# mit-acl/clipper

Hardware: AMD Instinct MI355X
Metric: affinity+solve ms and GEMV HBM GB/s, n=10k assoc, 95% outliers, 1/8 GPU (lower is better)
Workload: dtype f64 (M stored f32)

## Files before the change

clipper_amd/_abi.py:

```python
from __future__ import annotations

import ctypes as C
import os
from dataclasses import dataclass, field

import numpy as np

_HERE = os.path.dirname(os.path.abspath(__file__))
LIB_PATH = os.environ.get("CLIPPER_HIP_LIB") or os.path.join(_HERE, "lib", "libclipper_hip.so")

STORE_F32, STORE_F64, STORE_F32_CSC, STORE_F64_CSC = 0, 1, 2, 3
ROUNDING_NONZERO, ROUNDING_DSD, ROUNDING_DSD_HEU = 0, 1, 2
MC_EXACT, MC_HEU, MC_KCORE = 0, 1, 2
MC_SEED_ONLY = 3
SDP_MAX_N = 128
SDP_WIDE_MAX_N = 1024
SDP_ROUTE_WORKGROUP, SDP_ROUTE_AUTO, SDP_ROUTE_WIDE = 0, 1, 2
INVARIANT_MAX_D, INVARIANT_MAX_PARAMS = 32, 16

EXPORTED_SYMBOLS = [
    "clipper_hip_device_count", "clipper_hip_create", "clipper_hip_create_group",
    "clipper_hip_create_rank", "clipper_hip_comm_unique_id", "clipper_hip_comm_init",
    "clipper_hip_destroy", "clipper_hip_last_error", "clipper_hip_affinity_euclidean",
    "clipper_hip_affinity_pointnormal", "clipper_hip_num_associations",
    "clipper_hip_get_associations", "clipper_hip_set_matrix", "clipper_hip_set_sparse",
    "clipper_hip_get_matrix", "clipper_hip_solve", "clipper_hip_get_nodes",
    "clipper_hip_get_selected_associations", "clipper_hip_matvec", "clipper_hip_set_profiling",
    "clipper_hip_set_window", "clipper_hip_window", "clipper_hip_densest_subgraph",
    "clipper_hip_set_resident", "clipper_hip_last_solver",
    "clipper_hip_set_row_view", "clipper_hip_get_view_stats", "clipper_hip_view_matvec", "clipper_hip_set_subproblem",
    "clipper_hip_storage_in_use", "clipper_hip_knn", "clipper_hip_distance_based_correspondences",
    "clipper_hip_get_timings", "clipper_hip_bench_matvec", "clipper_hip_device_info",
    "clipper_hip_stage_inputs", "clipper_hip_affinity_euclidean_staged",
    "clipper_hip_affinity_pointnormal_staged", "clipper_hip_stage_u0",
    "clipper_hip_solve_staged", "clipper_hip_debug_stamps", "clipper_hip_comm_init_callback",
    "clipper_hip_read_ply_xyz", "clipper_hip_generate_synthetic_correspondences",
    "clipper_hip_precision_recall", "clipper_hip_estimate_rigid_transform", "clipper_hip_debug_occupy",
    "clipper_hip_max_clique", "clipper_hip_core_numbers", "clipper_hip_sdp", "clipper_hip_sdp_solve",
    "clipper_hip_batch_create", "clipper_hip_batch_destroy", "clipper_hip_batch_solve_euclidean",
    "clipper_hip_batch_solve_pointnormal", "clipper_hip_batch_get_solution", "clipper_hip_batch_get_nodes",
    "clipper_hip_batch_get_selected_associations", "clipper_hip_batch_route", "clipper_hip_batch_get_stats",
    "clipper_hip_batch_get_split", "clipper_hip_invariant_create", "clipper_hip_invariant_destroy",
    "clipper_hip_affinity_custom_staged", "clipper_hip_affinity_custom", "clipper_hip_batch_solve_custom",
    "clipper_hip_sdp_solve_batch", "clipper_hip_batch_sdp", "clipper_hip_batch_get_sdp",
    "clipper_hip_batch_max_clique", "clipper_hip_batch_max_clique_stats",
    "clipper_hip_max_clique_seeded", "clipper_hip_batch_max_clique_seeded",
    "clipper_hip_sdp_set_route", "clipper_hip_sdp_route", "clipper_hip_match_descriptors",
]


ALLGATHER_FN = C.CFUNCTYPE(C.c_int, C.c_void_p, C.c_void_p, C.c_void_p, C.c_size_t)


class ClipperError(RuntimeError):
    """a C ABI entry point returned a negative status (CLIPPER_HIP_E_*)"""


class Params(C.Structure):

    _fields_ = [
        ("tol_u", C.c_double), ("tol_F", C.c_double), ("tol_Fop", C.c_double),
        ("maxiniters", C.c_int32), ("maxoliters", C.c_int32), ("beta", C.c_double),
        ("maxlsiters", C.c_int32), ("eps", C.c_double), ("affinityeps", C.c_double),
        ("rescale_u0", C.c_int32), ("rounding", C.c_int32),
    ]

    def __init__(self, **kw):
        super().__init__()
        self.tol_u, self.tol_F, self.tol_Fop = 1e-8, 1e-9, 1e-10
        self.maxiniters, self.maxoliters = 200, 1000
        self.beta, self.maxlsiters = 0.25, 99
        self.eps, self.affinityeps = 1e-9, 1e-4
        self.rescale_u0, self.rounding = 1, ROUNDING_DSD_HEU
        for k, v in kw.items():
            setattr(self, k, v)


class SolveInfo(C.Structure):
    _fields_ = [
        ("score", C.c_double), ("seconds", C.c_double), ("d", C.c_double),
        ("ifinal", C.c_int32), ("num_nodes", C.c_int32),
        ("n_passes", C.c_int64), ("n_trials", C.c_int64),
    ]


class Timings(C.Structure):
    _fields_ = [
        ("affinity_kernel_ms", C.c_double), ("affinity_total_ms", C.c_double),
        ("solve_total_ms", C.c_double), ("gemv_avg_us", C.c_double),
        ("gemv_min_us", C.c_double), ("gemv_launches", C.c_int64), ("gemv_bytes", C.c_double),
        ("gemv_useful_bytes", C.c_double), ("affinity_bytes", C.c_double),
        ("exchange_avg_us", C.c_double), ("exchange_samples", C.c_int64), ("exchange_bytes", C.c_double),
    ]


class ViewStats(C.Structure):

    _fields_ = [
        ("builds", C.c_int64), ("rows", C.c_int64), ("bytes", C.c_int64),
        ("view_passes", C.c_int64), ("passes", C.c_int64), ("build_ms", C.c_double),
        ("view_pass_avg_us", C.c_double), ("view_pass_samples", C.c_int64),
        ("resident_launches", C.c_int64), ("resident_giveups", C.c_int64),
        ("resident_iterations", C.c_int64), ("resident_us", C.c_double), ("resident_event_us", C.c_double),
        ("resident_entries", C.c_int64), ("resident_units", C.c_int64),
        ("sub_entries", C.c_int64), ("sub_leaves", C.c_int64), ("sub_passes", C.c_int64),
        ("sub_rows", C.c_int64), ("sub_bytes", C.c_int64), ("sub_build_ms", C.c_double),
        ("sub_pass_avg_us", C.c_double), ("sub_pass_samples", C.c_int64), ("sub_dense", C.c_int64),
    ]


class MaxCliqueInfo(C.Structure):

    _fields_ = [
        ("num_nodes", C.c_int32), ("max_core", C.c_int32), ("heuristic_size", C.c_int32), ("timed_out", C.c_int32),
        ("edges", C.c_int64), ("roots_searched", C.c_int64), ("roots_pruned", C.c_int64), ("bb_nodes", C.c_int64),
        ("seconds", C.c_double),
    ]


class MaxCliqueSeedInfo(C.Structure):

    _fields_ = [("seed_given", C.c_int32), ("seed_kept", C.c_int32), ("seed_size", C.c_int32), ("winner", C.c_int32)]


class SdpParams(C.Structure):

    _fields_ = [
        ("verbose", C.c_int32), ("max_iters", C.c_int32), ("acceleration_interval", C.c_int32),
        ("acceleration_lookback", C.c_int32), ("eps_abs", C.c_float), ("eps_rel", C.c_float),
        ("eps_infeas", C.c_float), ("time_limit_secs", C.c_float),
    ]

    def __init__(self, **kw):
        base = dict(verbose=0, max_iters=2000, acceleration_interval=10, acceleration_lookback=10, eps_abs=1e-3,
                    eps_rel=1e-3, eps_infeas=1e-7, time_limit_secs=0.0)
        base.update(kw)
        super().__init__(**base)


class SdpInfo(C.Structure):

    _fields_ = [
        ("iters", C.c_int32), ("converged", C.c_int32), ("timed_out", C.c_int32), ("num_nodes", C.c_int32),
        ("sweeps", C.c_int32), ("route", C.c_int32),
        ("pobj", C.c_double), ("dobj", C.c_double), ("r_prim", C.c_double), ("r_dual", C.c_double),
        ("rho", C.c_double), ("thr", C.c_double), ("t_total", C.c_double), ("t_setup", C.c_double),
        ("t_solve", C.c_double), ("t_extract", C.c_double),
    ]


class SdpProblem(C.Structure):

    _fields_ = [
        ("M", C.POINTER(C.c_double)), ("C", C.POINTER(C.c_double)), ("n", C.c_int64),
        ("X_out", C.POINTER(C.c_double)), ("Y_out", C.POINTER(C.c_double)), ("lambdas_out", C.POINTER(C.c_double)),
        ("evec1_out", C.POINTER(C.c_double)), ("nodes_out", C.POINTER(C.c_int32)),
    ]


@dataclass
class SdpResult:

    X: np.ndarray
    Y: np.ndarray
    lambdas: np.ndarray
    evec1: np.ndarray
    thr: float
    nodes: np.ndarray
    iters: int
    pobj: float
    dobj: float
    info: SdpInfo


def _sdp_result(n, X, Y, lam, ev, nodes, info) -> SdpResult:
    return SdpResult(X=X, Y=Y, lambdas=lam, evec1=ev, thr=info.thr, nodes=nodes, iters=info.iters, pobj=info.pobj,
                     dobj=info.dobj, info=info)


class MatchParams(C.Structure):
    _fields_ = [("knn", C.c_int32), ("mutual", C.c_int32), ("ratio", C.c_double), ("max_sqdist", C.c_double)]


class BatchProblem(C.Structure):

    _fields_ = [
        ("D1", C.POINTER(C.c_double)), ("n1", C.c_int64),
        ("D2", C.POINTER(C.c_double)), ("n2", C.c_int64),
        ("A", C.POINTER(C.c_int32)), ("m", C.c_int64),
        ("u0", C.POINTER(C.c_double)),
    ]


@dataclass
class Solution:

    t: float = 0.0
    ifinal: int = 0
    nodes: np.ndarray = field(default_factory=lambda: np.zeros(0, np.int32))
    u0: np.ndarray = field(default_factory=lambda: np.zeros(0))
    u: np.ndarray = field(default_factory=lambda: np.zeros(0))
    score: float = 0.0
    d: float = 0.0
    n_passes: int = 0
    n_trials: int = 0


_lib = None


def load_library(path: str = LIB_PATH):
    global _lib
    if _lib is not None:
        return _lib
    if not os.path.exists(path):
        raise RuntimeError(
            f"{path} not found: build it with `python -c 'import __graft_entry__ as g; g.build()'`"
            " (hipcc --offload-arch=gfx950). There is no CPU fallback.")
    L = C.CDLL(path)
    dp, ip, i64, vp = C.POINTER(C.c_double), C.POINTER(C.c_int32), C.c_int64, C.c_void_p
    L.clipper_hip_device_count.restype = C.c_int
    L.clipper_hip_create.argtypes = [C.c_int, C.c_int]
    L.clipper_hip_create.restype = vp
    L.clipper_hip_create_group.argtypes = [C.POINTER(C.c_int), C.c_int, C.c_int]
    L.clipper_hip_create_group.restype = vp
    L.clipper_hip_create_rank.argtypes = [C.c_int, C.c_int, C.c_int, C.c_int]
    L.clipper_hip_create_rank.restype = vp
    L.clipper_hip_comm_unique_id.argtypes = [vp]
    L.clipper_hip_comm_init.argtypes = [vp, vp]
    L.clipper_hip_destroy.argtypes = [vp]
    L.clipper_hip_destroy.restype = None
    L.clipper_hip_last_error.restype = C.c_char_p
    L.clipper_hip_affinity_euclidean.argtypes = [
        vp, dp, C.c_int, i64, dp, i64, ip, i64, C.c_double, C.c_double, C.c_double, C.c_double]
    L.clipper_hip_affinity_pointnormal.argtypes = [
        vp, dp, C.c_int, i64, dp, i64, ip, i64, C.c_double, C.c_double, C.c_double, C.c_double,
        C.c_double]
    L.clipper_hip_stage_inputs.argtypes = [vp, dp, C.c_int, i64, dp, i64, ip, i64]
    L.clipper_hip_affinity_euclidean_staged.argtypes = [vp] + [C.c_double] * 4
    L.clipper_hip_affinity_pointnormal_staged.argtypes = [vp] + [C.c_double] * 5
    L.clipper_hip_stage_u0.argtypes = [vp, dp]
    L.clipper_hip_solve_staged.argtypes = [vp, C.POINTER(Params), dp, C.POINTER(SolveInfo)]
    L.clipper_hip_num_associations.argtypes = [vp]
    L.clipper_hip_num_associations.restype = i64
    L.clipper_hip_get_associations.argtypes = [vp, ip]
    L.clipper_hip_set_matrix.argtypes = [vp, dp, dp, i64]
    L.clipper_hip_set_sparse.argtypes = [vp, i64, C.POINTER(i64), ip, dp, C.POINTER(i64), ip, dp]
    L.clipper_hip_get_matrix.argtypes = [vp, dp, dp]
    L.clipper_hip_solve.argtypes = [vp, dp, C.POINTER(Params), dp, C.POINTER(SolveInfo)]
    L.clipper_hip_get_nodes.argtypes = [vp, ip, C.c_int32]
    L.clipper_hip_get_selected_associations.argtypes = [vp, ip, C.c_int32]
    L.clipper_hip_matvec.argtypes = [vp, dp, dp, dp]
    L.clipper_hip_densest_subgraph.argtypes = [vp, ip, C.c_int32, ip, C.c_int32]
    L.clipper_hip_set_window.argtypes = [vp, C.c_int]
    L.clipper_hip_window.argtypes = [vp]
    L.clipper_hip_set_resident.argtypes = [vp, C.c_int]
    L.clipper_hip_last_solver.argtypes = [vp]
    L.clipper_hip_storage_in_use.argtypes = [vp]
    L.clipper_hip_set_row_view.argtypes = [vp, C.c_int]
    L.clipper_hip_set_subproblem.argtypes = [vp, C.c_int]
    L.clipper_hip_get_view_stats.argtypes = [vp, C.POINTER(ViewStats)]
    L.clipper_hip_view_matvec.argtypes = [vp, ip, i64, dp, dp, dp]
    L.clipper_hip_knn.argtypes = [C.c_int, dp, C.c_int64, dp, C.c_int64, C.c_int, C.c_int, ip, dp]
    L.clipper_hip_distance_based_correspondences.argtypes = [
        C.c_int, dp, C.c_int64, dp, C.c_int64, C.c_int, C.c_int, C.c_double, C.c_int, ip, C.c_int64]
    L.clipper_hip_distance_based_correspondences.restype = C.c_int64
    L.clipper_hip_match_descriptors.argtypes = [C.c_int, dp, C.c_int64, dp, C.c_int64, C.c_int, C.POINTER(MatchParams),
                                                ip, dp, C.c_int64, ip, dp]
    L.clipper_hip_match_descriptors.restype = C.c_int64
    L.clipper_hip_set_profiling.argtypes = [vp, C.c_int]
    L.clipper_hip_get_timings.argtypes = [vp, C.POINTER(Timings)]
    L.clipper_hip_bench_matvec.argtypes = [vp, C.c_int, dp]
    L.clipper_hip_device_info.argtypes = [vp, C.c_char_p, C.POINTER(C.c_int), C.POINTER(i64)]
    L.clipper_hip_debug_stamps.argtypes = [vp, C.POINTER(i64), C.c_int]
    L.clipper_hip_comm_init_callback.argtypes = [vp, ALLGATHER_FN, vp]
    L.clipper_hip_read_ply_xyz.argtypes = [C.c_char_p, dp, i64]
    L.clipper_hip_read_ply_xyz.restype = i64
    L.clipper_hip_generate_synthetic_correspondences.argtypes = [i64, i64, ip, i64, i64, C.c_double, C.c_uint64,
                                                                 ip, ip, C.POINTER(i64)]
    L.clipper_hip_precision_recall.argtypes = [ip, i64, ip, i64, C.POINTER(C.c_double), C.POINTER(C.c_double)]
    L.clipper_hip_estimate_rigid_transform.argtypes = [dp, i64, dp, i64, ip, i64, dp]
    L.clipper_hip_debug_occupy.argtypes = [C.c_int, C.c_int, C.c_int, C.c_double]
    L.clipper_hip_max_clique.argtypes = [vp, C.c_int, C.c_double, C.POINTER(MaxCliqueInfo)]
    L.clipper_hip_core_numbers.argtypes = [vp, ip]
    L.clipper_hip_sdp.argtypes = [vp, C.POINTER(SdpParams), dp, dp, dp, dp, C.POINTER(SdpInfo)]
    L.clipper_hip_sdp_solve.argtypes = [C.c_int, dp, dp, C.c_int64, C.POINTER(SdpParams), dp, dp, dp, dp, ip,
                                        C.POINTER(SdpInfo)]
    L.clipper_hip_sdp_solve_batch.argtypes = [C.c_int, C.POINTER(SdpProblem), C.c_int32, C.POINTER(SdpParams),
                                              C.POINTER(SdpInfo)]
    L.clipper_hip_batch_sdp.argtypes = [vp, C.POINTER(SdpParams), C.POINTER(SdpInfo)]
    L.clipper_hip_batch_get_sdp.argtypes = [vp, C.c_int32, dp, dp, dp, dp]
    L.clipper_hip_sdp_set_route.argtypes = [C.c_int]
    L.clipper_hip_sdp_route.argtypes = []
    L.clipper_hip_batch_max_clique.argtypes = [vp, C.c_int, C.c_double, C.POINTER(MaxCliqueInfo)]
    L.clipper_hip_batch_max_clique_stats.argtypes = [vp, ip, ip, ip]
    L.clipper_hip_max_clique_seeded.argtypes = [vp, C.c_int, C.c_double, ip, C.c_int32, C.POINTER(MaxCliqueInfo),
                                                C.POINTER(MaxCliqueSeedInfo)]
    L.clipper_hip_batch_max_clique_seeded.argtypes = [vp, C.c_int, C.c_double, ip, C.POINTER(C.c_int64),
                                                      C.POINTER(MaxCliqueInfo), C.POINTER(MaxCliqueSeedInfo)]
    L.clipper_hip_batch_create.argtypes = [C.c_int, C.c_int, C.POINTER(vp)]
    L.clipper_hip_batch_destroy.argtypes = [vp]
    L.clipper_hip_batch_destroy.restype = None
    L.clipper_hip_batch_solve_euclidean.argtypes = [vp, C.POINTER(BatchProblem), C.c_int32, C.c_int] + \
        [C.c_double] * 3 + [C.POINTER(Params)]
    L.clipper_hip_batch_solve_pointnormal.argtypes = [vp, C.POINTER(BatchProblem), C.c_int32] + \
        [C.c_double] * 4 + [C.POINTER(Params)]
    L.clipper_hip_batch_solve_custom.argtypes = [vp, vp, C.POINTER(BatchProblem), C.c_int32, dp, C.c_int,
                                                 C.POINTER(Params)]
    L.clipper_hip_batch_get_solution.argtypes = [vp, C.c_int32, dp, C.POINTER(SolveInfo)]
    L.clipper_hip_batch_get_nodes.argtypes = [vp, C.c_int32, ip, C.c_int32]
    L.clipper_hip_batch_get_selected_associations.argtypes = [vp, C.c_int32, ip, C.c_int32]
    L.clipper_hip_batch_route.argtypes = [vp, C.c_int32]
    L.clipper_hip_batch_get_stats.argtypes = [vp, ip, ip, ip]
    L.clipper_hip_batch_get_split.argtypes = [vp, dp, dp, dp, dp]
    L.clipper_hip_invariant_create.argtypes = [C.c_char_p, C.c_int, C.POINTER(vp)]
    L.clipper_hip_invariant_destroy.argtypes = [vp]
    L.clipper_hip_affinity_custom_staged.argtypes = [vp, vp, dp, C.c_int, C.c_double]
    L.clipper_hip_affinity_custom.argtypes = [vp, vp, dp, C.c_int, i64, dp, i64, ip, i64, dp, C.c_int, C.c_double]
    _lib = L
    return L


def _dp(a):
    return a.ctypes.data_as(C.POINTER(C.c_double))


def _ip(a):
    return a.ctypes.data_as(C.POINTER(C.c_int32))


def _i64p(a):
    return a.ctypes.data_as(C.POINTER(C.c_int64))


def _f64_colmajor(D):
    return np.asfortranarray(np.asarray(D, dtype=np.float64))


def _assoc_colmajor(A):
    A = np.asarray(A)
    if A.size == 0:
        return None, 0
    A = np.asfortranarray(A.astype(np.int32, copy=False))
    if A.ndim != 2 or A.shape[1] != 2:
        raise ValueError("A must be m x 2")
    return A, A.shape[0]


def _params_array(params):
    p = np.ascontiguousarray(np.asarray(params, dtype=np.float64).reshape(-1))
    return p, (_dp(p) if p.size else None)


class HipInvariant:

    def __init__(self, source: str, d: int):
        self.L = load_library()
        self.source, self.d = source, int(d)
        h = C.c_void_p()
        rc = self.L.clipper_hip_invariant_create(source.encode(), self.d, C.byref(h))
        if rc < 0:
            raise ClipperError(f"clipper_hip error {rc}: {self.L.clipper_hip_last_error().decode()}")
        self.h = h

    def close(self):
        if getattr(self, "h", None):
            self.L.clipper_hip_invariant_destroy(self.h)
            self.h = None

    def __enter__(self):
        return self

    def __exit__(self, *exc):
        self.close()

    def __del__(self):
        try:
            self.close()
        except Exception:
            pass


class HipClipper:

    def __init__(self, params: Params | None = None, device: int = 0, storage: int = STORE_F32,
                 group: list[int] | None = None, rank: int | None = None, world: int = 1):
        self.L = load_library()
        self.params = params or Params()
        if group is not None:
            arr = (C.c_int * len(group))(*group)
            h = self.L.clipper_hip_create_group(arr, len(group), storage)
        elif rank is not None:
            h = self.L.clipper_hip_create_rank(device, storage, rank, world)
        else:
            h = self.L.clipper_hip_create(device, storage)
        if not h:
            raise RuntimeError("clipper_hip_create failed: " + self.last_error())
        self.h = C.c_void_p(h)
        self.storage = storage
        self.soln = Solution()

    def last_error(self) -> str:
        return self.L.clipper_hip_last_error().decode()

    def close(self):
        if getattr(self, "h", None):
            self.L.clipper_hip_destroy(self.h)
            self.h = None

    def __del__(self):
# ... 632 lines not shown
```

clipper_amd/csrc/host_rv_resident.hpp:

```cpp
#pragma once

namespace {

void rvr_free(Ctx* h) {
  ViewResident& r = h->vres;
  if (r.host_plan) hipHostFree(r.host_plan);
  if (r.xb) hipFree(r.xb);
  if (r.ctl) hipFree(r.ctl);
  if (r.giveup_host) hipHostFree(r.giveup_host);
  if (r.backup) hipFree(r.backup);
  for (hipEvent_t e : r.ev)
    if (e) hipEventDestroy(e);
  const unsigned long long ep = r.epoch;
  const int tu = r.target_units, cd = r.cooldown, cn = r.cooldown_next, mu = r.max_units_device;
  r = ViewResident{};
  r.epoch = ep;
  r.target_units = tu;
  r.cooldown = cd;
  r.cooldown_next = cn;
  r.max_units_device = mu;
}

void rvr_begin_solve(Ctx* h) {
  ViewResident& r = h->vres;
  r.launches_this_solve = 0;
  r.ev_n = 0;
  if (r.giveup_host) std::memset(r.giveup_host, 0, RVR_GIVEUP_SLOTS * 4 * sizeof(uint32_t));
  std::atomic_thread_fence(std::memory_order_seq_cst);
}

void rvr_end_solve(Ctx* h) {
  ViewResident& r = h->vres;
  if (r.cooldown > 0 && r.launches_this_solve == 0) --r.cooldown;
  if (r.launches_this_solve == 0 || !r.giveup_host) return;
  std::atomic_thread_fence(std::memory_order_acquire);
  int gave_up = 0;
  volatile const uint32_t* w = r.giveup_host;
  for (int k = 0; k < std::min(r.launches_this_solve, RVR_GIVEUP_SLOTS); ++k) {
    if (w[4 * k] != 0u) {
      ++gave_up;
    } else {
      h->rv_stats.resident_iterations += static_cast<int64_t>(w[4 * k + 1]);
      h->rv_stats.resident_us += static_cast<double>(static_cast<uint64_t>(w[4 * k + 2]) | (static_cast<uint64_t>(w[4 * k + 3]) << 32)) * 1e-2;
    }
  }
  for (int k = 0; k < r.ev_n; ++k) {
    float ms = 0.f;
    if (hipEventSynchronize(r.ev[2 * k + 1]) == hipSuccess && hipEventElapsedTime(&ms, r.ev[2 * k], r.ev[2 * k + 1]) == hipSuccess)
      h->rv_stats.resident_event_us += static_cast<double>(ms) * 1e3;
    else (void)hipGetLastError();
  }
  h->rv_stats.resident_entries = static_cast<int64_t>(r.plan_entries);
  h->rv_stats.resident_units = r.nunits;
  if (gave_up > 0) {
    h->rv_stats.resident_launches -= gave_up;
    h->rv_stats.resident_giveups += gave_up;
    r.cooldown = r.cooldown_next;
    r.cooldown_next = std::min(64, 2 * r.cooldown_next);
    if (rs_debug())
      std::fprintf(stderr, "[view-resident] %d launch(es) gave up (error %u): the next %d solve(s) stream their views\n", gave_up,
                   static_cast<unsigned>(w[0]), r.cooldown);
  } else {
    r.cooldown_next = 1;
  }
}

bool rvr_gate(const Ctx* h) { return h->rv_mode == 0 && csc_possible(h) && h->sh.size() == 1 && (h->V == 6 || h->V == 4); }
bool rvr_local_ok(const Ctx* h) {
  static const bool env_off = [] {
    const char* e = std::getenv("CLIPPER_HIP_VIEW_RESIDENT");
    return e && std::atoi(e) == 0;
  }();
  return !env_off && h->vres.cooldown == 0;
}
bool rvr_common(const Ctx* h) { return rvr_gate(h) && rvr_local_ok(h); }
bool rvr_enabled(const Ctx* h) { return rvr_common(h) && csc_single(h); }
bool rvr_replica_gate(const Ctx* h) { return rvr_gate(h) && h->multiproc && rect_fill_possible(h); }
bool rvr_replica_enabled(const Ctx* h) { return rvr_replica_gate(h) && rvr_local_ok(h); }

bool rvr_candidate(const Ctx* h, int64_t nrows) { return rvr_enabled(h) && nrows >= 1 && nrows <= RVR_MAXROWS; }

int rvr_plan(Ctx* h, Shard& s, bool replica = false) {
  ViewResident& r = h->vres;
  r.ready = false;
  r.on_replica = replica;
  if (!(replica ? rvr_replica_enabled(h) && s.rv.full_valid : rvr_enabled(h)) || !s.rv.valid) return 0;
  const RowView& v = s.rv;
  const SliceStore& vst = replica ? v.full : v.st;
  if (v.nrows < 1 || v.nrows > RVR_MAXROWS) return 0;
  static_assert(sizeof(clipper_plan::ViewUnit) == sizeof(RvrUnit), "the planner's unit is the kernel's");
  const clipper_plan::ResidentConsts K{RVR_NT, RVR_NWV, RVR_TMAX, RVR_PMAX, 2, RS_LDS_MAX,
                                       RVR_RED_BYTES, RVR_TAB_BYTES, RS_SLICE_PAD, SL_SO};
  static thread_local clipper_plan::ViewResidentPlan plan;
  if (r.target_units == 0) {
    const char* e = std::getenv("CLIPPER_HIP_VIEW_RESIDENT_WGS");
    r.target_units = e ? std::max(1, std::atoi(e)) : -1;
  }
  if (r.max_units_device < 0) {
    int per_cu = 0;
    hipError_t e = hipErrorUnknown;
    dispatch_vt(h, [&](auto tag) {
      using VT = decltype(tag);
      auto kern = (h->V == 6) ? k_solve_view_resident<VT, 6, false> : k_solve_view_resident<VT, 4, false>;
      if (raise_dynamic_lds(reinterpret_cast<const void*>(kern), s.device, static_cast<int>(RS_LDS_MAX)))
        e = hipOccupancyMaxActiveBlocksPerMultiprocessor(&per_cu, reinterpret_cast<const void*>(kern), RVR_NT, RS_LDS_MAX);
    });
    if (e != hipSuccess) (void)hipGetLastError();
    r.max_units_device = (e == hipSuccess) ? per_cu * h->cus : 0;
    if (rs_debug()) std::fprintf(stderr, "[view-resident] the device holds %d workgroups of the kernel at a time\n", r.max_units_device);
  }
  if (r.max_units_device < 16) return 0;
  const int max_units = std::min({RVR_MAXUNITS, h->cus - 8, r.max_units_device - 8});
  const int target = r.target_units > 0 ? r.target_units : std::max(8, (2 * h->cus) / 3);
  const uint32_t fixed = rvr_xt_bytes(h->V, static_cast<int>(v.nrows)) + RVR_RED_BYTES + RVR_TAB_BYTES;
  clipper_plan::plan_view_resident(h->csc_hLq, vst.s_ncg, vst.s_nchunks, static_cast<int>(h->esize()), target,
                                   max_units, fixed, K, plan);
  if (rs_debug())
    std::fprintf(stderr, "[view-resident] plan rows=%lld ncg=%d nchunks=%d entries=%llu -> units=%zu ok=%d\n",
                 static_cast<long long>(v.nrows), vst.s_ncg, vst.s_nchunks,
                 static_cast<unsigned long long>(plan.entries), plan.units.size(), plan.ok ? 1 : 0);
  if (!plan.ok) return 0;
  if (rs_debug() && std::atoi(std::getenv("CLIPPER_HIP_RESIDENT_DEBUG")) >= 2) {
    for (size_t ui = 0; ui < plan.units.size(); ++ui) {
      const clipper_plan::ViewUnit& U = plan.units[ui];
      uint64_t ent = 0;
      for (int c = 0; c < U.ncgs; ++c) ent += plan.ent[static_cast<size_t>(U.cg0 + c)];
      if (U.l1 - U.l0 < 64) ent = ent * static_cast<uint64_t>(U.l1 - U.l0) / 64;
      int wmax = 0, wsum = 0;
      for (int w = 0; w < RVR_NWV; ++w) {
        int st = 0;
        for (int j = 0; j < plan.npieces[ui * RVR_NWV + w]; ++j) {
          const uint32_t pc = plan.pieces[(ui * RVR_NWV + w) * RVR_PMAX + j];
          st += static_cast<int>((pc >> 16) & 255u) - static_cast<int>((pc >> 8) & 255u);
        }
        wmax = std::max(wmax, st);
        wsum += st;
      }
      std::fprintf(stderr, "[view-resident-unit] %zu cg0 %d ncgs %d lanes %d-%d pack %d entries %llu steps_max_wave %d steps_sum %d\n", ui, U.cg0, U.ncgs,
                   U.l0, U.l1, U.pack, static_cast<unsigned long long>(ent), wmax, wsum);
    }
  }
  HIPCHK(hipSetDevice(s.device));
  const size_t off_np = plan.units.size() * sizeof(RvrUnit);
  const size_t off_wc = off_np + static_cast<size_t>(round_up(static_cast<int64_t>(plan.npieces.size()), 16));
  const size_t off_pc = off_wc + static_cast<size_t>(round_up(static_cast<int64_t>(plan.wave_cg.size()), 16));
  const size_t bytes = off_pc + plan.pieces.size() * sizeof(uint32_t) + 64;
  if (bytes > r.host_plan_cap) {
    if (r.host_plan) hipHostFree(r.host_plan);
    r.host_plan = nullptr;
    r.host_plan_cap = 0;
    HIPCHK(hipHostMalloc(reinterpret_cast<void**>(&r.host_plan), bytes + 4096, hipHostMallocMapped | hipHostMallocCoherent));
    HIPCHK(hipHostGetDevicePointer(reinterpret_cast<void**>(&r.host_plan_dev), r.host_plan, 0));
    r.host_plan_cap = bytes + 4096;
  }
  std::memcpy(r.host_plan, plan.units.data(), plan.units.size() * sizeof(RvrUnit));
  std::memcpy(r.host_plan + off_np, plan.npieces.data(), plan.npieces.size());
  std::memcpy(r.host_plan + off_wc, plan.wave_cg.data(), plan.wave_cg.size());
  {
    uint32_t* dst = reinterpret_cast<uint32_t*>(r.host_plan + off_pc);
    const uint32_t* src = plan.pieces.data();
    for (size_t wv = 0; wv < plan.npieces.size(); ++wv)
      for (int j = 0; j < plan.npieces[wv]; ++j) dst[wv * RVR_PMAX + j] = src[wv * RVR_PMAX + j];
  }
  std::atomic_thread_fence(std::memory_order_seq_cst);
  r.off_np = off_np;
  r.off_wc = off_wc;
  r.off_pc = off_pc;
  const size_t xb_bytes = static_cast<size_t>(rvr_xb_granules(6)) * sizeof(unsigned long long);
  if (!r.xb) {
    HIPCHK(hipMalloc(&r.xb, xb_bytes));
    HIPCHK(hipMemsetAsync(r.xb, 0, xb_bytes, s.stream));
    r.xb_bytes = xb_bytes;
  }
  if (!r.ctl) {
    HIPCHK(hipMalloc(&r.ctl, RVR_GIVEUP_SLOTS * 64));
    HIPCHK(hipMemsetAsync(r.ctl, 0, RVR_GIVEUP_SLOTS * 64, s.stream));
  }
  if (!r.giveup_host) {
    HIPCHK(hipHostMalloc(reinterpret_cast<void**>(&r.giveup_host), RVR_GIVEUP_SLOTS * 4 * sizeof(uint32_t), hipHostMallocMapped | hipHostMallocCoherent));
    HIPCHK(hipHostGetDevicePointer(reinterpret_cast<void**>(&r.giveup_host_dev), r.giveup_host, 0));
    std::memset(r.giveup_host, 0, RVR_GIVEUP_SLOTS * 4 * sizeof(uint32_t));
  }
  r.nunits = static_cast<int>(plan.units.size());
  r.plan_entries = plan.entries;
  r.lds_slices = plan.lds_slices;
  r.ready = true;
  return 0;
}

template <typename VT, int V>
int rvr_launch_t(Ctx* h, Shard& s, const RvrArgs& a) {
  auto kern = a.stamps ? k_solve_view_resident<VT, V, true> : k_solve_view_resident<VT, V, false>;
  if (!raise_dynamic_lds(reinterpret_cast<const void*>(kern), s.device, static_cast<int>(RS_LDS_MAX))) return 1;
  hipLaunchKernelGGL(kern, dim3(static_cast<unsigned>(a.nunits)), dim3(RVR_NT), RS_LDS_MAX, s.stream, a);
  if (const hipError_t e = hipGetLastError(); e != hipSuccess) {
    if (rs_debug()) std::fprintf(stderr, "[view-resident] launch failed: %s\n", hipGetErrorString(e));
    return 1;
  }
  return 0;
}

int rvr_enqueue(Ctx* h, const SolverParams& prm, bool& launched) {
  launched = false;
  ViewResident& r = h->vres;
  if (!r.ready || !(r.on_replica ? rvr_replica_enabled(h) : rvr_enabled(h)) || prm.maxiniters < 1) return 0;
  Shard& s = h->sh[0];
  if (!s.rv.valid || (r.on_replica && !s.rv.full_valid)) return 0;
  static_assert(RV_MAX_BUILDS <= RVR_GIVEUP_SLOTS, "one give-up slot per view a solve can build");
  if (r.launches_this_solve >= RVR_GIVEUP_SLOTS) return 0;
  HIPCHK(hipSetDevice(s.device));
  RvrArgs a{};
  a.R = r.on_replica ? row_view_full(h, s) : row_view(h, s);
  a.units = reinterpret_cast<const RvrUnit*>(r.host_plan_dev);
  a.nunits = r.nunits;
  a.npieces = r.host_plan_dev + r.off_np;
  a.wave_cg = r.host_plan_dev + r.off_wc;
  a.pieces = reinterpret_cast<const uint32_t*>(r.host_plan_dev + r.off_pc);
  a.viewpos = s.rv.viewpos;
  a.st = s.st + h->par;
  a.shared = s.shared;
  a.host = h->mirror_dev;
  a.host_u = h->u_pinned_dev;
  a.marks = h->profiling ? s.marks : nullptr;
  a.kind = (a.marks && !h->multiproc) ? h->kind_dev : nullptr;
  a.marks_n = h->launch_counter;
  a.prm = prm;
  a.m = h->m;
  a.mp = h->mp;
  a.pt = s.pt;
  a.xb = r.xb;
  if (int rc = epoch_wrap(r.epoch, r.xb, r.xb_bytes, s.stream)) return rc;
  a.epoch0 = r.epoch;
  r.epoch += 1ull << 20;
  const bool own_ctl = r.launches_this_solve < RVR_GIVEUP_SLOTS;
  a.ctl = r.ctl + (own_ctl ? 16 * r.launches_this_solve : 0);
  a.giveup_host = (r.giveup_host_dev && r.launches_this_solve < RVR_GIVEUP_SLOTS) ? r.giveup_host_dev + 4 * r.launches_this_solve : nullptr;
  a.lds_slices = r.lds_slices;
  a.timeout_ticks = 200000ll;
  if (r.epoch == 0) a.timeout_ticks = 2000000ll;
  if (const char* e = std::getenv("CLIPPER_HIP_VIEW_RESIDENT_TIMEOUT_TICKS")) a.timeout_ticks = std::atoll(e);
  a.max_exchanges = 1 << 18;
  if (const char* e = std::getenv("CLIPPER_HIP_VIEW_RESIDENT_MAX_EXCHANGES"))
    a.max_exchanges = std::min((1 << 20) - 1, std::max(0, std::atoi(e)));
  a.rvp = h->rvp;
  a.rv_rows = static_cast<int>(s.rv.nrows);
  a.stamps = h->stamps_dev;
  if (!own_ctl) HIPCHK(hipMemsetAsync(r.ctl, 0, 64, s.stream));
  const bool timed = h->profiling_level >= 2 && r.ev_n < 16;
  if (timed) {
    for (int k = 0; k < 2; ++k)
      if (!r.ev[2 * r.ev_n + k]) HIPCHK(hipEventCreate(&r.ev[2 * r.ev_n + k]));
    HIPCHK(hipEventRecord(r.ev[2 * r.ev_n], s.stream));
  }
  int lr = 1;
  dispatch_vt(h, [&](auto tag) {
    using VT = decltype(tag);
    lr = (h->V == 6) ? rvr_launch_t<VT, 6>(h, s, a) : rvr_launch_t<VT, 4>(h, s, a);
  });
  if (lr != 0) {
    r.ready = false;
    return 0;
  }
  if (timed) {
    HIPCHK(hipEventRecord(r.ev[2 * r.ev_n + 1], s.stream));
    ++r.ev_n;
  }
  launched = true;
  r.launches_this_solve += 1;
  h->rv_stats.resident_launches += 1;
  return 0;
}

int rvr_agree(Ctx* h, bool mine, bool& all) {
  Shard& s = h->sh[0];
  HIPCHK(hipSetDevice(s.device));
  HIPCHK(hipStreamSynchronize(s.stream));
  const double v = mine ? 1.0 : 0.0;
  HIPCHK(hipMemcpy(s.ab + static_cast<int64_t>(s.slot) * h->W, &v, sizeof(double), hipMemcpyHostToDevice));
  if (int rc = exchange(h, 1)) return rc;
  if (int rc = sync_all(h)) return rc;
  all = true;
  std::vector<double> flags(static_cast<size_t>(h->world), 0.0);
  HIPCHK(hipMemcpy2D(flags.data(), sizeof(double), s.ab, static_cast<size_t>(h->W) * sizeof(double), sizeof(double),
                     static_cast<size_t>(h->world), hipMemcpyDeviceToHost));
  for (double x : flags) all = all && x == 1.0;
  return 0;
}

int rvr_build_replica(Ctx* h, Shard& s) {
  RowView& v = s.rv;
  v.full_valid = false;
  if (!v.valid) return 0;
  if (int rc = emit_rect(h, s, v.full, v.rowmap[v.cur], v.nrows, 0, round_up(h->m, 64), false, 4, "row view replica"))
    return rc;
  v.full_valid = true;
  return 0;
}

int rvr_replica_handover(Ctx* h, const SolverParams& prm) {
  ViewResident& r = h->vres;
  r.ready = false;
  if (!h->multiproc || h->sh.size() != 1) return 0;
  Shard& s = h->sh[0];
  if (!rvr_replica_gate(h) || !s.rv.valid || s.rv.nrows < 1 || s.rv.nrows > RVR_MAXROWS || prm.maxiniters < 1) return 0;
  int rc;
  const auto t0 = std::chrono::high_resolution_clock::now();
  bool mine = false;
  int local_rc = 0;
  if (rvr_local_ok(h) && r.launches_this_solve < RVR_GIVEUP_SLOTS) {
    local_rc = rvr_build_replica(h, s);
    if (!local_rc && s.rv.full_valid) {
      local_rc = rvr_plan(h, s, true);
      mine = !local_rc && r.ready;
    }
    if (mine && !r.backup && hipMalloc(reinterpret_cast<void**>(&r.backup), sizeof(SolverState) + sizeof(SolveShared)) != hipSuccess) {
      (void)hipGetLastError();
      r.backup = nullptr;
      local_rc = fail(CLIPPER_HIP_E_NOMEM, "resident solver on a view: no memory for the state's backup");
      mine = false;
    }
  }
  bool all = false;
  if ((rc = rvr_agree(h, mine, all))) return rc;
  if (local_rc) {
    r.ready = false;
    return local_rc;
  }
  if (rs_debug())
    std::fprintf(stderr, "[view-resident] replica: rows %lld, %.1f MB, this rank %s, all ranks %s\n", static_cast<long long>(s.rv.nrows),
                 static_cast<double>(s.rv.full.s_bytes) / 1e6, mine ? "ready" : "not ready", all ? "ready" : "not ready");
  if (!all) {
    r.ready = false;
    return 0;
  }
  if ((rc = enqueue_iteration(h, prm, true))) return rc;
  HIPCHK(hipSetDevice(s.device));
  HIPCHK(hipMemcpyAsync(r.backup, s.st + h->par, sizeof(SolverState), hipMemcpyDeviceToDevice, s.stream));
  HIPCHK(hipMemcpyAsync(r.backup + sizeof(SolverState), s.shared, sizeof(SolveShared), hipMemcpyDeviceToDevice, s.stream));
  bool launched = false;
  const int slot = r.launches_this_solve;
  if ((rc = rvr_enqueue(h, prm, launched))) return rc;
  if (!launched) {
    r.launches_this_solve += 1;
    h->rv_stats.resident_launches += 1;
    if (r.giveup_host && slot < RVR_GIVEUP_SLOTS) r.giveup_host[4 * slot] = RVR_ERR_STATE;
  }
  HIPCHK(hipStreamSynchronize(s.stream));
  std::atomic_thread_fence(std::memory_order_acquire);
  const bool ran = launched && !(r.giveup_host && slot < RVR_GIVEUP_SLOTS && static_cast<volatile uint32_t*>(r.giveup_host)[4 * slot] != 0u);
  bool all_ran = false;
  if ((rc = rvr_agree(h, ran, all_ran))) return rc;
  if (!all_ran) {
    if (ran) {
      HIPCHK(hipMemcpyAsync(s.st + h->par, r.backup, sizeof(SolverState), hipMemcpyDeviceToDevice, s.stream));
      HIPCHK(hipMemcpyAsync(s.shared, r.backup + sizeof(SolverState), sizeof(SolveShared), hipMemcpyDeviceToDevice, s.stream));
      if (r.giveup_host && slot < RVR_GIVEUP_SLOTS) r.giveup_host[4 * slot] = RVR_ERR_PEER;
    }
    r.ready = false;
  }
  h->rv_stats.build_ms += std::chrono::duration<double, std::milli>(std::chrono::high_resolution_clock::now() - t0).count();
  return 0;
}

}
```

clipper_amd/csrc/host_solve.hpp:

```cpp
#pragma once

namespace {

void destroy_ctx(Ctx* h) {
  if (!h) return;
  for (auto& s : h->sh) {
    hipSetDevice(s.device);
    if (s.stream) hipStreamSynchronize(s.stream);
  }
  if (h->comm && g_rccl.CommDestroy) g_rccl.CommDestroy(h->comm);
  sub_free(h);
  for (auto& s : h->sh) {
    free_shard_buffers(s);
    if (s.ev_reduced) hipEventDestroy(s.ev_reduced);
    if (s.ev_copied) hipEventDestroy(s.ev_copied);
    if (s.stream && !h->borrowed_stream) hipStreamDestroy(s.stream);
  }
  if (!h->sh.empty()) hipSetDevice(h->sh[0].device);
  for (hipEvent_t e : h->ev_pairs) hipEventDestroy(e);
  for (hipEvent_t e : h->ev_xchg) hipEventDestroy(e);
  for (hipEvent_t e : {h->ev_poll[0], h->ev_poll[1], h->ev_aff[0], h->ev_aff[1]})
    if (e) hipEventDestroy(e);
  for (void* p : std::initializer_list<void*>{h->host_state, h->mirror, h->kind, h->u_pinned, h->xchg_send, h->xchg_recv,
                                              h->csc_hLq, h->csc_hctl, h->csc_htotal, h->csc_hwork, h->rv_count, h->rv_desc_host,
                                              h->mc_stage.p})
    if (p) hipHostFree(p);
  if (h->stamps_dev) hipFree(h->stamps_dev);
  resident_free(h);
  rvr_free(h);
  delete h;
}

int ensure_u_pinned(Ctx* h) {
  const size_t vbytes = static_cast<size_t>(h->m) * sizeof(double);
  if (h->u_pinned_cap >= vbytes) return 0;
  if (h->u_pinned) hipHostFree(h->u_pinned);
  h->u_pinned = nullptr;
  h->u_pinned_dev = nullptr;
  h->u_pinned_cap = 0;
  HIPCHK(hipSetDevice(h->sh[0].device));
  HIPCHK(hipHostMalloc(reinterpret_cast<void**>(&h->u_pinned), vbytes,
                       hipHostMallocMapped | hipHostMallocCoherent));
  HIPCHK(hipHostGetDevicePointer(reinterpret_cast<void**>(&h->u_pinned_dev), h->u_pinned, 0));
  h->u_pinned_cap = vbytes;
  return 0;
}

void selected_associations(const Ctx* h, const std::vector<int32_t>& nodes, int32_t* out) {
  const size_t k = nodes.size();
  for (size_t r = 0; r < k; ++r) {
    const size_t a = static_cast<size_t>(nodes[r]);
    out[r] = h->A[a];
    out[k + r] = h->A[static_cast<size_t>(h->m) + a];
  }
}

int round_nodes(Ctx* h, int rounding, const std::vector<double>& u, double F, std::vector<int32_t>& nodes) {
  const int64_t m = static_cast<int64_t>(u.size());
  nodes.clear();
  if (rounding == CLIPPER_ROUNDING_NONZERO) {
    for (int64_t i = 0; i < m; ++i)
      if (u[static_cast<size_t>(i)] > 0.0) nodes.push_back(static_cast<int32_t>(i));
  } else if (rounding == CLIPPER_ROUNDING_DSD) {
    std::vector<int32_t> S;
    for (int64_t i = 0; i < m; ++i)
      if (u[static_cast<size_t>(i)] > 0.0) S.push_back(static_cast<int32_t>(i));
    if (S.empty())
      for (int64_t i = 0; i < m; ++i) S.push_back(static_cast<int32_t>(i));
    if (int rc = densest_subgraph_of(h, S, nodes)) return rc;
  } else {
    const int omega = static_cast<int>(std::round(F));
    nodes = indices_of_k_largest(u, omega);
  }
  return 0;
}

int solver_params(const clipper_params_t* P, SolverParams& prm) {
  if (!P) return fail(CLIPPER_HIP_E_INVALID, "params are required");
  if (P->rounding != CLIPPER_ROUNDING_NONZERO && P->rounding != CLIPPER_ROUNDING_DSD_HEU &&
      P->rounding != CLIPPER_ROUNDING_DSD)
    return fail(CLIPPER_HIP_E_INVALID, "unknown rounding mode %d", P->rounding);
  if (P->maxlsiters < 1) return fail(CLIPPER_HIP_E_INVALID, "maxlsiters must be >= 1");
  prm = SolverParams{P->tol_u, P->tol_F, P->beta, P->eps, P->maxiniters, P->maxoliters, P->maxlsiters};
  return 0;
}

void solve_info(clipper_solve_info_t& info, const SolveShared& fin) {
  info.score = fin.F;
  info.d = fin.d;
  info.ifinal = fin.ifinal;
  info.n_passes = fin.n_passes;
  info.n_trials = fin.n_trials;
}

struct SolveMarks {
  const std::chrono::high_resolution_clock::time_point t0 = std::chrono::high_resolution_clock::now();
  const bool on = [] { static const bool env = std::getenv("CLIPPER_HIP_HOST_TIMING") != nullptr; return env; }();
  std::vector<std::pair<const char*, double>> marks;
  void operator()(const char* what) {
    if (on) marks.emplace_back(what, std::chrono::duration<double, std::micro>(std::chrono::high_resolution_clock::now() - t0).count());
  }
};

int solve_begin(Ctx* h, bool rescale, SolverState& init) {
  h->rv_stats = clipper_hip_view_stats_t{};
  h->ev_used = 0;
  std::fill(h->ev_xchg_used.begin(), h->ev_xchg_used.end(), 0);
  if (h->profiling) {
    const size_t n = static_cast<size_t>(std::min<int64_t>(h->launch_counter + 1, KIND_CAP));
    std::memset(h->kind, 0, n);
    HIPCHK(hipSetDevice(h->sh[0].device));
    HIPCHK(hipMemsetAsync(h->sh[0].marks, 0, n, h->sh[0].stream));
  }
  h->launch_counter = 0;
  std::memset(&init, 0, sizeof(init));
  init.alpha = 1.0;
  for (int l = 0; l < VS; ++l) init.nrm[l] = 1.0;
  init.nlive = init.nout = static_cast<int32_t>(std::min<int64_t>(h->m, 0x7fffffff));
  init.rv_last = -100;
  init.zero_run = 2;
  init.phase = rescale ? PH_RESCALE : PH_NORMALIZE;
  init.stage = rescale ? ST_PASS : ST_RESULTS;
  rowview_drop(h);
  rvr_begin_solve(h);
  sub_begin_solve(h);
  h->rvp = rowview_policy(h);
  return ensure_u_pinned(h);
}

void hold_rewind(Ctx* h) {
  volatile HostMirror* hm = h->mirror;
  hm->hold = 0;
  h->launch_counter = hm->iters;
  while (h->ev_used > 0 && h->ev_launch_index[static_cast<size_t>(h->ev_used - 1)] >= hm->iters) --h->ev_used;
}

void sub_account(Ctx* h) {
  h->sub.sub_passes += std::max<int64_t>(0, h->mirror->n_passes - h->sub.passes_at_entry);
}

int solve_hold_view(Ctx* h, const SolverParams& prm, int64_t& queued, SolveMarks& mark) {
  int rc;
  bool built = false;
  if ((rc = rowview_build(h, built))) return rc;
  mark("view built");
  const bool early = h->early_decide_done;
  h->early_decide_done = false;
  if (early) ++queued;
  else h->rv_fresh = built;
  if (built && h->vres.ready) {
    if (!early) {
      if ((rc = enqueue_iteration(h, prm, true))) return rc;
      ++queued;
    }
    bool launched = false;
    if ((rc = rvr_enqueue(h, prm, launched))) return rc;
    mark("resident queued");
  }
  if ((rc = rowview_finish_plan(h))) return rc;
  if (built && !h->vres.ready && !early) {
    if (int r2 = sub_prepare(h)) {
      if (r2 != CLIPPER_HIP_E_NOMEM) return r2;
      (void)hipGetLastError();
      h->sub.ready = false;
    }
    mark("sub-problem prepared");
  }
  return 0;
}

int solve_hold(Ctx* h, const SolverParams& prm, int64_t& queued, SolveMarks& mark) {
  volatile HostMirror* hm = h->mirror;
  mark("hold seen");
  if (mark.on)
    std::fprintf(stderr, "[solve] hold: iters %lld passes %lld trials %lld view passes %lld live %d of which outside the view %d\n",
                 static_cast<long long>(hm->iters), static_cast<long long>(hm->n_passes), static_cast<long long>(hm->n_trials),
                 static_cast<long long>(hm->n_view_passes), static_cast<int>(hm->hold_nlive), static_cast<int>(hm->nout));
  int rc;
  if (h->sh.size() > 1 && (rc = sync_all(h))) return rc;
  std::atomic_thread_fence(std::memory_order_acquire);
  const int reason = hm->hold;
  hold_rewind(h);
  queued = hm->iters;
  switch (reason) {
    case HOLD_SUB_ENTER:
      if ((rc = sub_enter(h, prm))) return rc;
      ++queued;
      mark("sub-problem entered");
      return 0;
    case HOLD_SUB_LEAVE:
      sub_account(h);
      if ((rc = sub_leave(h))) return rc;
      mark("sub-problem left");
      return 0;
    default: return solve_hold_view(h, prm, queued, mark);
  }
}

int solve_in_process(Ctx* h, const SolverParams& prm, SolveShared& fin, SolveMarks& mark) {
  volatile HostMirror* hm = h->mirror;
  Shard& s0 = h->sh[0];
  int64_t queued = 0;
  uint64_t spins = 0;
  h->rv_fresh = false;
  int rc;
  while (!hm->done) {
    if (hm->hold) {
      if ((rc = solve_hold(h, prm, queued, mark))) return rc;
      continue;
    }
    if (hm->iters > queued) queued = hm->iters;
    if (queued - hm->iters < RUN_AHEAD) {
      if ((rc = enqueue_iteration(h->sub.active ? h->sub.use : h, prm, false))) return rc;
      ++queued;
      spins = 0;
    } else if ((++spins & 0xfffff) == 0) {
      hipError_t q = hipStreamQuery(s0.stream);
      if (q != hipSuccess && q != hipErrorNotReady)
        return fail(CLIPPER_HIP_E_HIP, "solver stream failed: %s", hipGetErrorString(q));
      if (q == hipSuccess && !hm->done && queued - hm->iters >= RUN_AHEAD)
        return fail(CLIPPER_HIP_E_HIP, "solver made no progress (iters %lld of %lld queued)",
                    static_cast<long long>(hm->iters), static_cast<long long>(queued));
    }
  }
  mark("done seen");
  std::atomic_thread_fence(std::memory_order_acquire);
  if (h->sub.active) {
    sub_account(h);
    h->sub.active = false;
  }
  fin = mirror_result(hm);
  h->rv_stats.view_passes = hm->n_view_passes;
  return 0;
}

int solve_multi_process(Ctx* h, const SolverParams& prm, SolveShared& fin) {
  Shard& s0 = h->sh[0];
  int batch = SOLVE_BATCH;
  if (const char* e = std::getenv("CLIPPER_HIP_SOLVE_BATCH")) batch = std::max(1, std::atoi(e));
  HIPCHK(hipSetDevice(s0.device));
  h->rv_fresh = false;
  int rc = run_batched_with_holds(
      batch, [&]() { return enqueue_iteration(h, prm, false); },
      [&](int slot) -> int {
        HIPCHK(hipSetDevice(s0.device));
        HIPCHK(hipMemcpyAsync(&h->host_state[slot], s0.shared, sizeof(SolveShared), hipMemcpyDeviceToHost, s0.stream));
        HIPCHK(hipEventRecord(h->ev_poll[slot], s0.stream));
        return 0;
      },
      [&](int slot, int& st) -> int {
        HIPCHK(hipEventSynchronize(h->ev_poll[slot]));
        st = h->host_state[slot].done != 0 ? 1 : (h->host_state[slot].hold != 0 ? 2 : 0);
        return 0;
      },
      [&]() -> int {
        if (int r2 = sync_all(h)) return r2;
        hold_rewind(h);
        bool built = false;
        if (int r2 = rowview_build(h, built)) return r2;
        h->rv_fresh = built;
        if (built)
          if (int r2 = rvr_replica_handover(h, prm)) return r2;
        return 0;
      },
      nullptr);
  if (rc) return rc;
  if ((rc = sync_all(h))) return rc;
  HIPCHK(hipSetDevice(s0.device));
  HIPCHK(hipMemcpy(&fin, s0.shared, sizeof(fin), hipMemcpyDeviceToHost));
  h->rv_stats.view_passes = h->mirror->n_view_passes;
  return 0;
}

int solve_streamed(Ctx* h, const SolverParams& prm, const SolverState& init, SolveShared& fin, SolveMarks& mark) {
  h->par = 0;
  std::memset(h->mirror, 0, sizeof(HostMirror));
  std::atomic_thread_fence(std::memory_order_seq_cst);
  for (auto& s : h->sh) {
    HIPCHK(hipSetDevice(s.device));
    const SolveArgs a = solve_args(h, s, prm, 0, false);
    hipLaunchKernelGGL(k_init, dim3(static_cast<unsigned>(ceil_div(h->m, 256))), dim3(256), 0, s.stream, a, init, s.st, s.X[0]);
  }
  mark("init queued");
  int rc;
  if (!h->multiproc) {
    h->solve_prm = &prm;
    rc = solve_in_process(h, prm, fin, mark);
    h->solve_prm = nullptr;
  } else {
    rc = solve_multi_process(h, prm, fin);
  }
  if (rc) return rc;
  rvr_end_solve(h);
  return 0;
}

int solve_finish(Ctx* h, int rounding, const SolveShared& fin, double* u_out, clipper_solve_info_t* info, SolveMarks& mark) {
  Shard& s0 = h->sh[0];
  const int64_t m = h->m;
  const size_t vbytes = static_cast<size_t>(m) * sizeof(double);
  int rc;
  HIPCHK(hipSetDevice(s0.device));
  if (h->multiproc) {
    const double* u_dev = s0.pt + ((static_cast<int64_t>(fin.ubp & 1) * h->V + fin.ubv) * 2 + 0) * h->mp;
    HIPCHK(hipMemcpyAsync(h->u_pinned, u_dev, vbytes, hipMemcpyDeviceToHost, s0.stream));
    if (h->profiling)
      HIPCHK(hipMemcpyAsync(h->kind, s0.marks, static_cast<size_t>(std::min<int64_t>(h->launch_counter, KIND_CAP)),
                            hipMemcpyDeviceToHost, s0.stream));
    if ((rc = sync_all(h))) return rc;
  } else {
    HIPCHK(hipGetLastError());
  }
  std::vector<double>& u = h->u_host;
  u.assign(h->u_pinned, h->u_pinned + m);
  std::vector<int32_t> nodes;
  if ((rc = round_nodes(h, rounding, u, fin.F, nodes))) return rc;
  h->nodes = nodes;
  if (u_out) std::memcpy(u_out, u.data(), vbytes);
  mark("rounded");
  if (mark.on) {
    std::fprintf(stderr, "[solve]");
    for (const auto& mk : mark.marks) std::fprintf(stderr, " %s %.1f |", mk.first, mk.second);
    std::fprintf(stderr, "\n");
  }
  const double secs = std::chrono::duration<double>(std::chrono::high_resolution_clock::now() - mark.t0).count();
  h->tm.solve_total_ms = secs * 1e3;
  if (info) {
    solve_info(*info, fin);
    info->seconds = secs;
    info->num_nodes = static_cast<int32_t>(nodes.size());
  }
  h->rv_stats.passes = fin.n_passes;
  h->rv_stats.sub_leaves = h->sub.leaves;
  h->rv_stats.sub_passes = h->sub.sub_passes;
  h->rv_stats.sub_build_ms = h->sub.build_ms;
  if (h->rv_stats.sub_entries > 0 && h->sub.use) {
    h->rv_stats.sub_rows = h->sub.nS;
    h->rv_stats.sub_bytes = h->sub.use->csc_valid ? static_cast<int64_t>(h->sub.use->sh[0].s_bytes)
                                                   : static_cast<int64_t>(algorithmic_gemv_bytes(h->sub.use));
    h->rv_stats.sub_dense = h->sub.use->csc_valid ? 0 : 1;
  }
  return 0;
}

int solve_timings(Ctx* h) {
  h->tm.gemv_avg_us = h->tm.gemv_min_us = 0.0;
  h->tm.gemv_launches = 0;
  h->tm.gemv_bytes = algorithmic_gemv_bytes(h);
  h->tm.gemv_useful_bytes = h->csc_valid ? static_cast<double>(h->sh[0].s_entries) * (h->esize() + 1.0) : h->tm.gemv_bytes;
  if (!h->profiling || h->ev_used <= 0) return 0;
  const uint8_t* kind = h->kind;
  const int64_t iters_run = std::min<int64_t>(h->launch_counter, KIND_CAP);
  double sum = 0.0, mn = 1e30, vsum = 0.0, ssum = 0.0, xs = 0.0;
  int64_t nreal = 0, nview = 0, nsub = 0, nx = 0;
  for (int k = 0; k < h->ev_used; ++k) {
    const int64_t li = h->ev_launch_index[static_cast<size_t>(k)];
    if (li >= iters_run || kind[static_cast<size_t>(li)] == MARK_NONE) continue;
    float ms = 0.f;
    if (h->ev_xchg_used[static_cast<size_t>(k)]) {
      HIPCHK(hipEventElapsedTime(&ms, h->ev_xchg[2 * k], h->ev_xchg[2 * k + 1]));
      xs += ms;
      ++nx;
    }
    HIPCHK(hipEventElapsedTime(&ms, h->ev_pairs[2 * k], h->ev_pairs[2 * k + 1]));
    const uint8_t mk = kind[static_cast<size_t>(li)];
    if (mk == MARK_VIEW) {
      vsum += ms;
      ++nview;
    } else if (mk == MARK_SUB_WINDOW) {
      ssum += ms;
      ++nsub;
    } else if (mk == MARK_WINDOW) {
      sum += ms;
      mn = std::min<double>(mn, ms);
      ++nreal;
    }
  }
  h->tm.exchange_avg_us = 0.0;
  h->tm.exchange_samples = 0;
  h->tm.exchange_bytes = static_cast<double>(nslot(h->V)) * static_cast<double>(h->W) * sizeof(double);
  if (nx > 0) {
    h->tm.exchange_avg_us = xs / static_cast<double>(nx) * 1e3;
    h->tm.exchange_samples = nx;
  }
  if (nview > 0) {
    h->rv_stats.view_pass_avg_us = vsum / static_cast<double>(nview) * 1e3;
    h->rv_stats.view_pass_samples = nview;
  }
  if (nsub > 0) {
    h->rv_stats.sub_pass_avg_us = ssum / static_cast<double>(nsub) * 1e3;
    h->rv_stats.sub_pass_samples = nsub;
  }
  if (nreal > 0) {
    h->tm.gemv_avg_us = sum / static_cast<double>(nreal) * 1e3;
    h->tm.gemv_min_us = mn * 1e3;
    h->tm.gemv_launches = nreal;
  }
  return 0;
}

int solve_staged(Ctx* h, const clipper_params_t* P, double* u_out, clipper_solve_info_t* info) {
  if (!h->has_matrix) return fail(CLIPPER_HIP_E_STATE, "no matrix has been built or set");
  if (!h->u0_staged) return fail(CLIPPER_HIP_E_STATE, "clipper_hip_stage_u0 not called");
  if (P && P->rounding == CLIPPER_ROUNDING_DSD && h->multiproc)
    return fail(CLIPPER_HIP_E_SCOPE, "Rounding::DSD needs the induced sub-matrix on one host: not available on a multi-process shard");
  SolverParams prm;
  int rc;
  if ((rc = solver_params(P, prm))) return rc;
  SolveMarks mark;
  SolverState init;
  if ((rc = solve_begin(h, P->rescale_u0 != 0, init))) return rc;
  SolveShared fin{};
  bool resident = false;
  if ((rc = resident_solve(h, prm, P->rescale_u0 != 0, fin, resident))) return rc;
  h->last_solver = resident ? 1 : 0;
  if (!resident && (rc = solve_streamed(h, prm, init, fin, mark))) return rc;
  if ((rc = solve_finish(h, P->rounding, fin, u_out, info, mark))) return rc;
  return solve_timings(h);
}

int stage_u0(Ctx* h, const double* u0) {
  if (!h->has_matrix) return fail(CLIPPER_HIP_E_STATE, "no matrix has been built or set");
  const size_t vbytes = static_cast<size_t>(h->m) * sizeof(double);
  for (auto& s : h->sh) {
    HIPCHK(hipSetDevice(s.device));
    HIPCHK(hipMemcpyAsync(s.u0, u0, vbytes, hipMemcpyHostToDevice, s.stream));
  }
  if (int rc = sync_all(h)) return rc;
  h->u0_staged = true;
  return 0;
}

int solve(Ctx* h, const double* u0, const clipper_params_t* P, double* u_out, clipper_solve_info_t* info) {
  const auto t0 = std::chrono::high_resolution_clock::now();
  if (int rc = stage_u0(h, u0); rc || (rc = solve_staged(h, P, u_out, info))) return rc;
  const double secs = std::chrono::duration<double>(std::chrono::high_resolution_clock::now() - t0).count();
  h->tm.solve_total_ms = secs * 1e3;
  if (info) info->seconds = secs;
  return 0;
}

}
```

clipper_amd/csrc/k_rv_resident.hip.h:

```cpp
#pragma once

#include <hip/hip_runtime.h>
#include <stdint.h>

#include "k_resident.hip.h"

namespace clipper_hip {

constexpr int RVR_NT = RS_NT;
constexpr int RVR_NWV = RS_NWV;
constexpr int RVR_TMAX = RS_TMAX;
constexpr int RVR_PMAX = RS_PMAX;
constexpr int RVR_MAXROWS = 2 * RVR_NT;
constexpr int RVR_MAXUNITS = 256;
constexpr int RVR_NRED = 40;

struct RvrUnit {
  int cg0, ncgs;
  int l0, l1;
  int pack;
  int pad1, pad2, pad3;
};

struct RvrArgs {
  SliceView R;
  const RvrUnit* units;
  int nunits;
  const uint32_t* pieces;
  const uint8_t* npieces;
  const uint8_t* wave_cg;
  const int32_t* viewpos;
  SolverState* st;
  SolveShared* shared;
  HostMirror* host;
  double* host_u;
  SolverParams prm;
  int64_t m, mp;
  double* pt;
  unsigned long long* xb;
  unsigned long long epoch0;
  uint32_t* ctl;
  uint32_t* giveup_host;
  uint32_t lds_slices;
  long long timeout_ticks;
  int max_exchanges;
  ViewPolicy rvp;
  int rv_rows;
  long long* stamps;
  const uint8_t* marks;
  uint8_t* kind;
  int64_t marks_n;
};
constexpr int RVR_FINE0 = 5120, RVR_FINE_TURNS = 96;
enum : int {
  RVR_F_KIND = 0, RVR_F_ROUNDS = 1, RVR_F_XT = 2 , RVR_F_NORMS = 3 ,
  RVR_F_SUMS = 4 , RVR_F_TAIL = 5 ,
  RVR_F_ROUND = 8 ,
  RVR_F_DECIDED = 14 , RVR_F_WAVE = 16
};
enum : uint32_t { RVR_ERR_LDS = 1, RVR_ERR_TIMEOUT = 2, RVR_ERR_STATE = 3, RVR_ERR_PEER = 4  };

__host__ __device__ constexpr uint32_t rvr_xt_bytes(int V, int nrows) {
  const uint32_t xt = static_cast<uint32_t>((nrows + 127) / 128 * 128) * V * 8u;
  const uint32_t sc = RVR_NWV * (V + 1) * 64u * 8u;
  return xt > sc ? xt : sc;
}
constexpr uint32_t RVR_RED_BYTES = RVR_NWV * RVR_NRED * 8 + 64 * 8;
constexpr uint32_t RVR_TAB_BYTES = RVR_TMAX * 4 + 64 + RVR_TMAX * 4;
__host__ __device__ constexpr int64_t rvr_xb_granules(int V) {
  return 2 * (static_cast<int64_t>(V + 2) * RVR_MAXROWS + RVR_MAXUNITS) * 2;
}

template <int N>
__device__ __forceinline__ void rvr_reduce(double (&v)[N], double* part , double* tot ) {
  static_assert(N <= RVR_NRED, "scratch");
#pragma unroll
  for (int q = 0; q < N; ++q) v[q] = wave_sum_to_lane63(v[q]);
  const int wave = threadIdx.x >> 6;
  __syncthreads();
  if ((threadIdx.x & 63) == 63) {
#pragma unroll
    for (int q = 0; q < N; ++q) part[wave * N + q] = v[q];
  }
  __syncthreads();
  if (threadIdx.x < N) {
    double acc = part[threadIdx.x];
#pragma unroll
    for (int w = 1; w < RVR_NWV; ++w) acc += part[w * N + threadIdx.x];
    tot[threadIdx.x] = acc;
  }
  __syncthreads();
}
__device__ __forceinline__ double rvr_uni(const double* p) {
  const double x = *p;
  return __hiloint2double(__builtin_amdgcn_readfirstlane(__double2hiint(x)),
                          __builtin_amdgcn_readfirstlane(__double2loint(x)));
}

__device__ __forceinline__ void rvr_publish(unsigned long long* gq, unsigned long long tag, double x) {
  const unsigned long long bits = static_cast<unsigned long long>(__double_as_longlong(x));
  __hip_atomic_store(gq, tag | (bits >> 32), __ATOMIC_RELAXED, __HIP_MEMORY_SCOPE_AGENT);
  __hip_atomic_store(gq + 1, tag | (bits & 0xffffffffull), __ATOMIC_RELAXED, __HIP_MEMORY_SCOPE_AGENT);
}
__device__ __forceinline__ bool rvr_poll(const unsigned long long* gq, unsigned long long tag, double& x) {
  const unsigned long long g0 = rs_ld_granule(gq), g1 = rs_ld_granule(gq + 1);
  x = __longlong_as_double(static_cast<long long>((g0 << 32) | (g1 & 0xffffffffull)));
  return ((g0 ^ tag) >> 32) == 0 && ((g1 ^ tag) >> 32) == 0;
}

typedef uint32_t rvr_u4 __attribute__((ext_vector_type(4)));
__device__ __forceinline__ rvr_u4 rvr_ld16(const unsigned long long* gq) {
  rvr_u4 v;
  asm volatile("global_load_dwordx4 %0, %1, off sc1" : "=v"(v) : "v"(gq) : "memory");
  return v;
}
__device__ __forceinline__ void rvr_wait_loads() { asm volatile("s_waitcnt vmcnt(0)" ::: "memory"); }
__device__ __forceinline__ void rvr_tie(rvr_u4& v) { asm volatile("" : "+v"(v)); }
__device__ __forceinline__ bool rvr_take(const rvr_u4& v, uint32_t tag32, double& x) {
  x = __hiloint2double(static_cast<int>(v.x), static_cast<int>(v.z));
  return v.y == tag32 && v.w == tag32;
}
__device__ __forceinline__ int wave_isum_to_lane63(int v) {
  v += __builtin_amdgcn_update_dpp(0, v, 0xB1, 0xf, 0xf, false);
  v += __builtin_amdgcn_update_dpp(0, v, 0x4E, 0xf, 0xf, false);
  v += __builtin_amdgcn_update_dpp(0, v, 0x141, 0xf, 0xf, false);
  v += __builtin_amdgcn_update_dpp(0, v, 0x140, 0xf, 0xf, false);
  v += __builtin_amdgcn_update_dpp(0, v, 0x142, 0xa, 0xf, false);
  v += __builtin_amdgcn_update_dpp(0, v, 0x143, 0xc, 0xf, false);
  return v;
}

template <typename VT, int V, bool FINE>
__global__ __launch_bounds__(RVR_NT) void k_solve_view_resident(RvrArgs A) {
  extern __shared__ __attribute__((aligned(16))) uint8_t rvr_lds[];
  constexpr int NS = V + 1;
  constexpr int QB = 4 * static_cast<int>(sizeof(VT));
  typedef uint32_t u32x4 __attribute__((ext_vector_type(4)));
  static_assert(V >= 2 && V <= 6 && (V % 2) == 0, "window of the streaming solver on slices");
  const int tid = threadIdx.x, lane = tid & 63;
  const int wave = __builtin_amdgcn_readfirstlane(tid >> 6);
  const int64_t m = A.m, mp = A.mp;
  const int nrows = static_cast<int>(A.R.nrows);
  const SolverParams P = A.prm;
  const int unit = blockIdx.x;
  const bool two = nrows > RVR_NT;

  uint32_t off = 0;
  double* Xt = reinterpret_cast<double*>(rvr_lds + off);
  double* scr = Xt;
  off += rvr_xt_bytes(V, nrows);
  double* red = reinterpret_cast<double*>(rvr_lds + off);
  double* tot = red + RVR_NWV * RVR_NRED;
  double* nrmL = tot + 32;
  double* sxL = tot + 40;
  off += RVR_RED_BYTES;
  uint32_t* tab = reinterpret_cast<uint32_t*>(rvr_lds + off);
  uint32_t* words = tab + RVR_TMAX;
  uint32_t* sizes = words + 16;
  off += RVR_TAB_BYTES;
  uint8_t* sl = rvr_lds + off;

  const long long ts0 = wall_clock64();
  if (unit == 0 && tid == 0)
    __hip_atomic_store(reinterpret_cast<unsigned long long*>(A.ctl + 4), static_cast<unsigned long long>(ts0), __ATOMIC_RELAXED, __HIP_MEMORY_SCOPE_AGENT);
  const SolverState* st = A.st;
  const int e_done = A.shared->done, e_hold = st->hold, e_stage = st->stage, e_resume = st->resume;
  if (e_done || e_hold || e_stage != ST_PASS || (e_resume != 1 && e_resume != 2) || st->nout != 0 ||
      nrows > RVR_MAXROWS || nrows < 1 || P.maxiniters < 1)
    return;

  const RvrUnit U = A.units[unit];
  const unsigned long long wcg = *reinterpret_cast<const unsigned long long*>(A.wave_cg + static_cast<int64_t>(unit) * RVR_NWV);
  const int cgl = static_cast<int>((wcg >> (8 * wave)) & 255ull);
  const bool has_cg = cgl < U.ncgs && U.cg0 + cgl < A.R.ncg;
  const int G = U.pack > 1 ? U.pack : 1;
  const int Wd = U.l1 - U.l0;
  const int S = (A.R.nchunks + G - 1) / G;
  const int nslices = U.ncgs * S;
  const bool whole = U.l0 <= 0 && U.l1 >= 64;
  const bool packed = G > 1;
  const int lgrp = packed ? lane / Wd : 0;
  const int lsrc = packed ? U.l0 + (lane - lgrp * Wd) : lane;
  const bool in_lanes = packed ? true : (lane >= U.l0 && lane < U.l1);
  const gbytes_t rdata = (gbytes_t)A.R.data;
  const CLIPPER_GLOBAL uint64_t* rpre = (const CLIPPER_GLOBAL uint64_t*)A.R.Pre;
  auto src_of = [&](int t) -> gbytes_t {
    const int tc = t / S, tk = t - tc * S;
    return rdata + 16 * rpre[static_cast<int64_t>(U.cg0 + tc) * A.R.nchunks + tk];
  };
  auto src_chunk = [&](int k) -> gbytes_t {
    return rdata + 16 * rpre[static_cast<int64_t>(U.cg0) * A.R.nchunks + k];
  };
  if (nslices <= RVR_TMAX) {
    for (int t = wave; t < nslices; t += RVR_NWV) {
      uint32_t bytes = 0;
      if (packed) {
        const int k = t * G + lgrp;
        const bool have = k < A.R.nchunks;
        const gbytes_t sp = src_chunk(have ? k : 0);
        int mq = have ? static_cast<int>(reinterpret_cast<const CLIPPER_GLOBAL uint32_t*>(sp)[1]) : 0;
        const int tq = have ? static_cast<int>(sp[16 + lsrc]) : 0;
        mq = sl_wave_max(mq);
        bytes = 16 + 64 + sl_so_bytes(mq) + sl_steps_bytes(tq, mq, QB);
        if (lane == 0) sizes[t] = bytes;
        continue;
      }
      const gbytes_t sp = src_of(t);
      const uint32_t nb = reinterpret_cast<const CLIPPER_GLOBAL uint32_t*>(sp)[2];
      bytes = nb;
      if (!whole) {
        const int maxq = __builtin_amdgcn_readfirstlane(static_cast<int>(reinterpret_cast<const CLIPPER_GLOBAL uint32_t*>(sp)[1]));
        const int tq = in_lanes ? static_cast<int>(sp[16 + lane]) : 0;
        bytes = 16 + 64 + sl_so_bytes(maxq) + sl_steps_bytes(tq, maxq, QB);
      }
      if (lane == 0) sizes[t] = bytes;
    }
  }
  __syncthreads();
  if (wave == 0) {
    const uint32_t bytes_t = (lane < nslices && nslices <= RVR_TMAX) ? sizes[lane] : 0u;
    uint32_t inc = bytes_t;
#pragma unroll
    for (int o = 1; o < 64; o <<= 1) {
      const uint32_t t2 = __shfl_up(inc, o);
      if (lane >= o) inc += t2;
    }
    tab[lane] = inc - bytes_t;
    if (lane == 63) words[0] = inc;
  }
  __syncthreads();
  const uint32_t total = words[0];
  const bool bad_plan = total + RS_SLICE_PAD > A.lds_slices || nslices > RVR_TMAX || U.ncgs > RVR_NWV;
  if (__syncthreads_or(bad_plan ? 1 : 0)) {
    if (tid == 0) {
      __hip_atomic_store(A.ctl, static_cast<uint32_t>(RVR_ERR_LDS), __ATOMIC_RELAXED, __HIP_MEMORY_SCOPE_AGENT);
      if (A.giveup_host) __hip_atomic_store(A.giveup_host, static_cast<uint32_t>(RVR_ERR_LDS), __ATOMIC_RELAXED, __HIP_MEMORY_SCOPE_SYSTEM);
    }
    return;
  }
  for (int t = wave; t < nslices; t += RVR_NWV) {
    const uint32_t o = tab[t];
    if (packed) {
      const int k = t * G + lgrp;
      const bool have = k < A.R.nchunks;
      const gbytes_t src = src_chunk(have ? k : 0);
      const int mq_own = have ? static_cast<int>(reinterpret_cast<const CLIPPER_GLOBAL uint32_t*>(src)[1]) : 0;
      const int tot_dst = have ? static_cast<int>(src[16 + lsrc]) : 0;
      const int maxq = __builtin_amdgcn_readfirstlane(sl_wave_max(mq_own));
      uint8_t* dp = sl + o;
      if (lane < 4) reinterpret_cast<uint32_t*>(dp)[lane] = (lane == 1) ? static_cast<uint32_t>(maxq) : 0u;
      dp[16 + lane] = static_cast<uint8_t>(tot_dst);
      for (int b = lane * 4; b < sl_so_bytes(maxq); b += 256) *reinterpret_cast<uint32_t*>(dp + 16 + 64 + b) = 0u;
      uint8_t* dfb = dp + 16 + 64 + sl_so_bytes(maxq);
      gbytes_t sfb = src + 16 + 64 + sl_so_bytes(mq_own);
      int tgs[8];
#pragma unroll
      for (int g = 0; g < 8; ++g) {
        const int kg = t * G + g;
        tgs[g] = (g < G && kg < A.R.nchunks) ? static_cast<int>(src_chunk(kg)[16 + lane]) : 0;
      }
      for (int q = 0; q < maxq; ++q) {
        uint64_t ms_own = 0;
#pragma unroll
        for (int g = 0; g < 8; ++g) {
          const uint64_t mg = __ballot(q < tgs[g]);
          if (g == lgrp) ms_own = mg;
        }
        const bool ad = q < tot_dst;
        const uint64_t md = __ballot(ad);
        const int cd = __builtin_amdgcn_readfirstlane(__popcll(md));
        const int cs = __popcll(ms_own);
        if (ad) {
          const uint32_t rs_ = static_cast<uint32_t>(__popcll(ms_own & ((1ull << lsrc) - 1ull)));
          const uint32_t rd_ = sl_lane_rank(md);
          SliceQuad<VT> vq;
          vq.load(sfb + rs_ * QB);
          const uint32_t rq = *reinterpret_cast<const CLIPPER_GLOBAL uint32_t*>(sfb + cs * QB + rs_ * 4);
          vq.store(dfb + rd_ * QB);
          *reinterpret_cast<uint32_t*>(dfb + cd * QB + rd_ * 4) = rq;
        }
        sfb += cs * QB + ((cs * 4 + 15) & ~15);
        dfb += cd * QB + ((cd * 4 + 15) & ~15);
      }
      continue;
    }
    const gbytes_t src = src_of(t);
    if (whole) {
      const uint32_t nb = reinterpret_cast<const CLIPPER_GLOBAL uint32_t*>(src)[2];
      for (uint32_t b = lane * 16; b < nb; b += 64 * 16)
        *reinterpret_cast<u32x4*>(sl + o + b) = *reinterpret_cast<const CLIPPER_GLOBAL u32x4*>(src + b);
    } else {
      const int maxq = __builtin_amdgcn_readfirstlane(static_cast<int>(reinterpret_cast<const CLIPPER_GLOBAL uint32_t*>(src)[1]));
      const int tot_src = static_cast<int>(src[16 + lane]);
      const int tot_dst = in_lanes ? tot_src : 0;
      uint8_t* dp = sl + o;
      if (lane < 4) reinterpret_cast<uint32_t*>(dp)[lane] = (lane == 1) ? static_cast<uint32_t>(maxq) : 0u;
      dp[16 + lane] = static_cast<uint8_t>(tot_dst);
      for (int b = lane * 4; b < sl_so_bytes(maxq); b += 256) *reinterpret_cast<uint32_t*>(dp + 16 + 64 + b) = 0u;
      gbytes_t sfb = src + 16 + 64 + sl_so_bytes(maxq);
      uint8_t* dfb = dp + 16 + 64 + sl_so_bytes(maxq);
      for (int q = 0; q < maxq; ++q) {
        const bool as = q < tot_src, ad = q < tot_dst;
        const uint64_t ms = __ballot(as), md = __ballot(ad);
        const int cs = __builtin_amdgcn_readfirstlane(__popcll(ms)), cd = __builtin_amdgcn_readfirstlane(__popcll(md));
        if (ad) {
          const uint32_t rs_ = sl_lane_rank(ms), rd_ = sl_lane_rank(md);
          SliceQuad<VT> vq;
          vq.load(sfb + rs_ * QB);
          const uint32_t rq = *reinterpret_cast<const CLIPPER_GLOBAL uint32_t*>(sfb + cs * QB + rs_ * 4);
          vq.store(dfb + rd_ * QB);
          *reinterpret_cast<uint32_t*>(dfb + cd * QB + rd_ * 4) = rq;
        }
        sfb += cs * QB + ((cs * 4 + 15) & ~15);
        dfb += cd * QB + ((cd * 4 + 15) & ~15);
      }
    }
  }
  const uint32_t* toff = tab + (has_cg ? cgl * S : 0);
  const int np = has_cg ? A.npieces[unit * RVR_NWV + wave] : 0;
  const uint32_t pc = (lane < RVR_PMAX) ? A.pieces[(static_cast<int64_t>(unit) * RVR_NWV + wave) * RVR_PMAX + lane] : 0u;

  double d = st->d, F = st->F, alpha = st->alpha, s = st->s;
  int i_ = st->i, j_ = st->j, k_ = st->k;
  const int e_ubp = st->ubp, e_ubv = st->ubv;
  int64_t n_passes = st->n_passes, n_trials = st->n_trials, n_iters = st->n_iters, n_view_passes = st->n_view_passes;
  int nlive = st->nlive, nout = 0;
  const int rv_builds = st->rv_builds, rv_last = st->rv_last, rv_backoff = st->rv_backoff;
  const int n_redo = st->n_redo;

  const double* Ue = A.pt + ((static_cast<int64_t>(e_ubp) * V + e_ubv) * 2 + 0) * mp;
  const double* Ge = A.pt + ((static_cast<int64_t>(e_ubp) * V + e_ubv) * 2 + 1) * mp;
  double UR[2], GR[2], aR[2] = {0.0, 0.0}, bR[2] = {0.0, 0.0};
  bool rok[2];
#pragma unroll
  for (int e = 0; e < 2; ++e) {
    const int r = tid + e * RVR_NT;
    rok[e] = r < nrows;
    const int64_t i = rok[e] ? A.R.rowmap[r] : 0;
    UR[e] = rok[e] ? Ue[i] : 0.0;
    GR[e] = rok[e] ? Ge[i] : 0.0;
  }
  const int64_t col = static_cast<int64_t>(U.cg0 + wave) * 64 + (packed ? U.l0 + lane : lane);
  const bool cown = wave < U.ncgs && (packed ? lane < Wd : in_lanes) && col < m;
  const int rpos = cown ? A.viewpos[col] : -1;
  double u_c = cown ? Ue[col] : 0.0, g_c = cown ? Ge[col] : 0.0, a_c = 0.0, b_c = 0.0;
  __syncthreads();

  unsigned long long epoch = A.epoch0;
  int exchanges = 0;
  int stamp_row = 0;
  const long long ts1 = A.stamps ? wall_clock64() : 0;
  auto stamp_end = [&]() {
    if (A.stamps && unit == 0 && tid == 0) {
      long long* row = A.stamps + 500 * 8;
      row[0] = ts0;
      row[1] = ts1;
      row[2] = wall_clock64();
      row[3] = stamp_row;
    }
  };
  int trow = 0;
  auto stamp = [&](int c) {
    if (A.stamps && tid == 0) {
      if (unit == 0 && trow < 500) A.stamps[trow * 8 + c] = wall_clock64();
      if (trow == 6 && c < 4 && unit < RVR_MAXUNITS) A.stamps[4096 + unit * 4 + c] = wall_clock64();
    }
  };
  auto fstamp = [&](int c, double dep = 0.0) {
    if constexpr (FINE) {
      if (A.stamps && unit == 0 && tid == 0 && trow < RVR_FINE_TURNS)
        A.stamps[RVR_FINE0 + trow * 32 + c] = wall_clock64() + (dep > 1e300 ? 1 : 0);
    }
  };
  auto fstamp_value = [&](int c, long long v) {
    if constexpr (FINE) {
      if (A.stamps && unit == 0 && tid == 0 && trow < RVR_FINE_TURNS) A.stamps[RVR_FINE0 + trow * 32 + c] = v;
    }
  };
  unsigned long long* const xb0 = A.xb;
  const int64_t par_stride = rvr_xb_granules(V) / 2;
  auto sec_g = [&](int par, int v, int r) { return xb0 + par * par_stride + ((static_cast<int64_t>(v) * RVR_MAXROWS + r) << 1); };
  auto sec_c = [&](int par, int p) { return xb0 + par * par_stride + ((static_cast<int64_t>(V + 2) * RVR_MAXROWS + p) << 1); };

  auto arrive_last = [&]() __attribute__((always_inline)) -> bool {
    __threadfence_system();
    __syncthreads();
    if (tid == 0) {
      const uint32_t k = __hip_atomic_fetch_add(A.ctl + 1, 1u, __ATOMIC_RELAXED, __HIP_MEMORY_SCOPE_AGENT) + 1u;
      words[1] = (k == static_cast<uint32_t>(A.nunits)) ? 1u : 0u;
    }
    __syncthreads();
    return words[1] != 0u;
  };
  auto report_run = [&]() __attribute__((always_inline)) {
    if (A.giveup_host) {
      const unsigned long long t_begin = __hip_atomic_load(reinterpret_cast<unsigned long long*>(A.ctl + 4), __ATOMIC_RELAXED, __HIP_MEMORY_SCOPE_AGENT);
      const unsigned long long dt = static_cast<unsigned long long>(wall_clock64()) - t_begin;
      __hip_atomic_store(A.giveup_host + 1, static_cast<uint32_t>(exchanges), __ATOMIC_RELAXED, __HIP_MEMORY_SCOPE_SYSTEM);
      __hip_atomic_store(A.giveup_host + 2, static_cast<uint32_t>(dt & 0xffffffffull), __ATOMIC_RELAXED, __HIP_MEMORY_SCOPE_SYSTEM);
      __hip_atomic_store(A.giveup_host + 3, static_cast<uint32_t>(dt >> 32), __ATOMIC_RELAXED, __HIP_MEMORY_SCOPE_SYSTEM);
    }
  };
  auto write_point = [&](bool to_host) __attribute__((always_inline)) {
    double* Ux = A.pt + ((static_cast<int64_t>(e_ubp ^ 1) * V + 0) * 2 + 0) * mp;
    double* Gx = A.pt + ((static_cast<int64_t>(e_ubp ^ 1) * V + 0) * 2 + 1) * mp;
    if (cown) {
      Ux[col] = u_c;
      Gx[col] = g_c;
      if (to_host && A.host_u) __hip_atomic_store(A.host_u + col, u_c, __ATOMIC_RELAXED, __HIP_MEMORY_SCOPE_SYSTEM);
    }
  };

  enum { K_TRIAL = 0, K_PAIR = 1, K_BUILD = 2 };
  int kind = (e_resume == 2) ? K_PAIR : K_TRIAL;
  bool want_out = false;
  for (;;) {
    trow = stamp_row;
    stamp(0);
    const bool out_now = kind != K_BUILD && (exchanges >= A.max_exchanges || (kind == K_TRIAL ? want_out : nout != 0));
    if (out_now) {
      const int resume = (kind == K_TRIAL) ? (nout != 0 ? 3 : 1) : 2;
      const bool window = kind == K_TRIAL;
      if (window) {
        double r2[2 * V];
#pragma unroll
        for (int q = 0; q < 2 * V; ++q) r2[q] = 0.0;
#pragma unroll
        for (int e = 0; e < 2; ++e) {
          double al = alpha;
#pragma unroll
          for (int l = 0; l < V; ++l) {
            const double t = cl_project(UR[e], al, GR[e]);
            r2[2 * l] += t * t;
            r2[2 * l + 1] += t;
            al = al * P.beta;
          }
        }
        rvr_reduce<2 * V>(r2, red, tot);
      }
      write_point(false);
      if (arrive_last() && tid == 0) {
        SolverState* o = A.st;
        o->d = d;
        o->F = F;
        o->alpha = alpha;
        o->s = s;
#pragma unroll
        for (int l = 0; l < V; ++l) {
          const double nl = (window && tot[2 * l] > 0.0) ? sqrt(tot[2 * l]) : 1.0;
          o->nrm[l] = (resume == 3) ? tot[2 * l] : nl;
          o->sx[l] = (resume == 3) ? tot[2 * l + 1] : (window ? tot[2 * l + 1] / nl : 0.0);
        }
        o->sel = 0;
        o->ubp = e_ubp ^ 1;
        o->ubv = 0;
        o->phase = window ? static_cast<int>(PH_TRIAL) : static_cast<int>(PH_PENALTY);
        o->stage = ST_PASS;
        o->i = i_;
        o->j = j_;
        o->k = k_;
        o->n_passes = n_passes;
        o->n_trials = n_trials;
        o->n_iters = n_iters;
        o->nlive = nlive;
        o->nout = nout;
        o->view = 0;
        o->hold = 0;
        o->n_view_passes = n_view_passes;
        o->rv_builds = rv_builds;
        o->rv_last = rv_last;
        o->rv_backoff = rv_backoff;
        o->hold_slot = 0;
        o->hold_nlive = 0;
        o->resume = resume;
        o->weff = V;
        o->zero_run = 0;
        report_run();
        if (A.host) {
          HostMirror* hm = A.host;
          __hip_atomic_store(&hm->nlive, nlive, __ATOMIC_RELAXED, __HIP_MEMORY_SCOPE_SYSTEM);
          __hip_atomic_store(&hm->nout, nout, __ATOMIC_RELAXED, __HIP_MEMORY_SCOPE_SYSTEM);
          __hip_atomic_store(&hm->n_view_passes, n_view_passes, __ATOMIC_RELAXED, __HIP_MEMORY_SCOPE_SYSTEM);
          __hip_atomic_store(&hm->iters, n_iters, __ATOMIC_RELEASE, __HIP_MEMORY_SCOPE_SYSTEM);
        }
      }
      stamp_end();
      return;
    }

    fstamp_value(RVR_F_KIND, kind);
    double y[NS];
#pragma unroll
    for (int v = 0; v < NS; ++v) y[v] = 0.0;
    if (kind != K_BUILD) {
#pragma unroll
      for (int e = 0; e < 2; ++e) {
        const int r = tid + e * RVR_NT;
        if (r < nrows) {
          double al = alpha;
#pragma unroll
          for (int l = 0; l < V; ++l) {
            double t = cl_project(UR[e], al, GR[e]);
            if (kind == K_PAIR) t = (l == 0) ? UR[e] : 0.0;
            Xt[r * V + l] = t;
            al = al * P.beta;
          }
        }
      }
      __syncthreads();
      fstamp(RVR_F_XT);
      double acc[NS];
      rs_wave_pass<VT, V>(sl, toff, pc, np, 0, Xt, (kind == K_TRIAL) ? d : 0.0, acc, G, lgrp * SL_SUB);
      if constexpr (FINE) {
        if (A.stamps && unit == 0 && lane == 0 && trow < RVR_FINE_TURNS)
          A.stamps[RVR_FINE0 + trow * 32 + RVR_F_WAVE + wave] = wall_clock64() + (acc[0] > 1e300 ? 1 : 0);
      }
      if (wave < V) {
        double z = 0.0, t1 = 0.0;
        if (kind == K_TRIAL) {
          for (int r = lane; r < nrows; r += 64) {
            const double c = Xt[r * V + wave];
            z += c * c;
            t1 += c;
          }
          z = wave_sum_to_lane63(z);
          t1 = wave_sum_to_lane63(t1);
        }
        if (lane == 63) {
          const double nl = cl_norm(z, kind == K_TRIAL);
          nrmL[wave] = nl;
          sxL[wave] = (kind == K_TRIAL) ? t1 / nl : 0.0;
        }
      }
      __syncthreads();
      fstamp(RVR_F_NORMS);
      if (packed) {
        for (int o = Wd; o < 64; o <<= 1) {
#pragma unroll
          for (int v = 0; v < NS; ++v) acc[v] += __shfl_xor(acc[v], o);
        }
      }
#pragma unroll
      for (int v = 0; v < NS; ++v) scr[(wave * NS + v) * 64 + lane] = acc[v];
      __syncthreads();
      if (wave < U.ncgs) {
        uint32_t mine = 0;
#pragma unroll
        for (int w = 0; w < RVR_NWV; ++w) mine |= (static_cast<int>((wcg >> (8 * w)) & 255ull) == wave) ? (1u << w) : 0u;
#pragma unroll
        for (int v = 0; v < NS; ++v) {
          double sum = 0.0;
#pragma unroll
          for (int w = 0; w < RVR_NWV; ++w) {
            const double t = scr[(w * NS + v) * 64 + lane];
            sum += ((mine >> w) & 1u) ? t : 0.0;
          }
          y[v] = sum;
        }
      }
      fstamp(RVR_F_SUMS, y[0]);
    }
    stamp(1);
    ++epoch;
    ++exchanges;
    const int par = static_cast<int>(epoch & 1ull);
    const unsigned long long tag = (epoch & 0xffffffffull) << 32;
    double gn_c[V], an_c = a_c, bn_c = b_c;
    uint32_t cbits = 0;
    if (kind == K_TRIAL) {
      double al = alpha;
#pragma unroll
      for (int v = 0; v < V; ++v) {
        const double t = cl_project(u_c, al, g_c);
        const double nv = rvr_uni(nrmL + v), sv = rvr_uni(sxL + v);
        const double xi = t / nv;
        double gn;
        if (v == 0) {
          an_c = y[0] / nv;
          bn_c = y[V] / nv;
          gn = cl_grad(d, xi, sv, an_c, bn_c);
        } else {
          const double gs = y[v] / nv;
          gn = cl_grad_fused(d, xi, sv, gs);
        }
        gn_c[v] = gn;
        if (cown && rpos < 0 && (xi > 0.0 || gn > 0.0)) cbits |= 1u << v;
        if (cown && rpos >= 0) rvr_publish(sec_g(par, v, rpos), tag, gn);
        al = al * P.beta;
      }
    } else {
#pragma unroll
      for (int v = 0; v < V; ++v) gn_c[v] = 0.0;
      if (kind == K_PAIR) {
        an_c = y[0];
        bn_c = y[V];
      } else if (cown) {
        gn_c[0] = cl_grad(d, u_c, s, a_c, b_c);
        if (rpos < 0 && (u_c > 0.0 || gn_c[0] > 0.0)) cbits = 1u;
      }
    }
    if (kind != K_BUILD && cown && rpos >= 0) {
      rvr_publish(sec_g(par, V, rpos), tag, an_c);
      rvr_publish(sec_g(par, V + 1, rpos), tag, bn_c);
    }
    a_c = an_c;
    b_c = bn_c;
    fstamp(RVR_F_TAIL, a_c + gn_c[V - 1]);
    if (U.ncgs == 1) {
      if (wave == 0) {
        unsigned long long pk = 0;
#pragma unroll
        for (int v = 0; v < V; ++v) pk |= static_cast<unsigned long long>(__popcll(__ballot((cbits >> v) & 1u))) << (10 * v);
        if (lane == 0) rvr_publish(sec_c(par, unit), tag, __longlong_as_double(static_cast<long long>(pk)));
      }
      __syncthreads();
    } else {
      unsigned long long w = 0;
#pragma unroll
      for (int v = 0; v < V; ++v) w |= static_cast<unsigned long long>(__popcll(__ballot((cbits >> v) & 1u))) << (7 * v);
      if (lane == 0) reinterpret_cast<unsigned long long*>(tot)[wave] = w;
      __syncthreads();
      if (tid == 0) {
        unsigned long long pk = 0;
#pragma unroll
        for (int v = 0; v < V; ++v) {
          unsigned long long tsum = 0;
          for (int w2 = 0; w2 < RVR_NWV; ++w2) tsum += (reinterpret_cast<unsigned long long*>(tot)[w2] >> (7 * v)) & 127ull;
          pk |= tsum << (10 * v);
        }
        rvr_publish(sec_c(par, unit), tag, __longlong_as_double(static_cast<long long>(pk)));
      }
      __syncthreads();
    }
    stamp(2);

    double gR[2][V], anR[2], bnR[2];
    unsigned long long cpk = 0;
#pragma unroll
    for (int e = 0; e < 2; ++e) {
      anR[e] = aR[e];
      bnR[e] = bR[e];
#pragma unroll
      for (int v = 0; v < V; ++v) gR[e][v] = 0.0;
    }
    {
      const uint32_t tag32 = static_cast<uint32_t>(epoch & 0xffffffffull);
      int fail = 0;
      const long long t_poll = wall_clock64();
      for (unsigned spins = 0;; ++spins) {
        bool ok = true;
#pragma unroll
        for (int e = 0; e < 2; ++e) {
          const int r = tid + e * RVR_NT;
          if ((e == 0 || two) && rok[e] && kind != K_BUILD) {
            rvr_u4 w[V + 2];
            if (kind == K_TRIAL) {
#pragma unroll
              for (int v = 0; v < V; ++v) w[v] = rvr_ld16(sec_g(par, v, r));
            }
            w[V] = rvr_ld16(sec_g(par, V, r));
            w[V + 1] = rvr_ld16(sec_g(par, V + 1, r));
            rvr_wait_loads();
            if (kind == K_TRIAL) {
#pragma unroll
              for (int v = 0; v < V; ++v) {
                rvr_tie(w[v]);
                ok = rvr_take(w[v], tag32, gR[e][v]) && ok;
              }
            }
            rvr_tie(w[V]);
            rvr_tie(w[V + 1]);
            ok = rvr_take(w[V], tag32, anR[e]) && ok;
            ok = rvr_take(w[V + 1], tag32, bnR[e]) && ok;
          }
        }
        if (tid < A.nunits) {
          rvr_u4 w = rvr_ld16(sec_c(par, tid));
          rvr_wait_loads();
          rvr_tie(w);
          double cd;
          ok = rvr_take(w, tag32, cd) && ok;
          cpk = static_cast<unsigned long long>(__double_as_longlong(cd));
        }
        if (__all(ok)) break;
        if ((spins & 63u) == 63u || A.timeout_ticks < 0) {
          const bool late = wall_clock64() - t_poll > A.timeout_ticks;
          const uint32_t e2 = __hip_atomic_load(A.ctl, __ATOMIC_RELAXED, __HIP_MEMORY_SCOPE_AGENT);
          if (late || e2 != 0) {
            fail = 1;
            break;
          }
        }
      }
      if (__syncthreads_or(fail)) {
        if (tid == 0) {
          uint32_t expect = 0;
          if (__hip_atomic_compare_exchange_strong(A.ctl, &expect, static_cast<uint32_t>(RVR_ERR_TIMEOUT), __ATOMIC_RELAXED,
                                                   __ATOMIC_RELAXED, __HIP_MEMORY_SCOPE_AGENT) &&
              A.giveup_host)
            __hip_atomic_store(A.giveup_host, static_cast<uint32_t>(RVR_ERR_TIMEOUT), __ATOMIC_RELAXED, __HIP_MEMORY_SCOPE_SYSTEM);
        }
        return;
      }
    }
    stamp(3);
#pragma unroll
    for (int e = 0; e < 2; ++e) {
      aR[e] = anR[e];
      bR[e] = bnR[e];
    }

    double* rbuf = red;
    int* ibuf = reinterpret_cast<int*>(red + V * RVR_NWV * 4);
    int nrounds = 0;
    auto round_sums = [&](int rd, double (&dv)[3], int (&iv)[3]) __attribute__((always_inline)) {
#pragma unroll
      for (int q = 0; q < 3; ++q) dv[q] = wave_sum_to_lane63(dv[q]);
      if (wave * 64 < A.nunits) iv[2] = wave_isum_to_lane63(iv[2]);
      if (lane == 63) {
#pragma unroll
        for (int q = 0; q < 3; ++q) rbuf[(rd * RVR_NWV + wave) * 4 + q] = dv[q];
#pragma unroll
        for (int q = 0; q < 3; ++q) ibuf[(rd * RVR_NWV + wave) * 4 + q] = iv[q];
      }
      __syncthreads();
#pragma unroll
      for (int q = 0; q < 3; ++q) {
        double acc = rbuf[(rd * RVR_NWV) * 4 + q];
        int iacc = ibuf[(rd * RVR_NWV) * 4 + q];
#pragma unroll
        for (int w = 1; w < RVR_NWV; ++w) {
          acc += rbuf[(rd * RVR_NWV + w) * 4 + q];
          iacc += ibuf[(rd * RVR_NWV + w) * 4 + q];
        }
        dv[q] = __hiloint2double(__builtin_amdgcn_readfirstlane(__double2hiint(acc)),
                                 __builtin_amdgcn_readfirstlane(__double2loint(acc)));
        iv[q] = __builtin_amdgcn_readfirstlane(iacc);
      }
      fstamp(RVR_F_ROUND + rd);
      ++nrounds;
    };
    auto stamp_decided = [&]() {
      stamp(4);
      fstamp(RVR_F_DECIDED);
      fstamp_value(RVR_F_ROUNDS, nrounds);
    };
    ++n_iters;
    if (kind != K_BUILD) {
      ++n_passes;
      ++n_view_passes;
    }
    ++stamp_row;
    bool penalty = false;
    int pen_cnt = 0;
    double pen_rs = 0.0;
    if (kind == K_TRIAL) {
      int jstar = -1;
      double Fnew = 0.0, deltaF = 0.0, du2 = 0.0;
      int lr = 0, no = 0;
      const double alpha_w = alpha;
      double al = alpha_w;
#pragma unroll
      for (int v = 0; v < V; ++v) {
        if (jstar < 0) {
          double dv[3] = {0.0, 0.0, 0.0};
          int iv[3] = {0, 0, 0};
          const double nv = rvr_uni(nrmL + v);
#pragma unroll
          for (int e = 0; e < 2; ++e) {
            if (e == 0 || two) {
              const double xi = cl_project(UR[e], al, GR[e]) / nv;
              const double gv = gR[e][v];
              bool live = false, pen = false;
              if (rok[e]) {
                dv[0] += xi * gv;
                const double du = xi - UR[e];
                dv[1] += du * du;
                live = xi > 0.0 || gv > 0.0;
                if (v == 0) {
                  const double cbu = cl_pen_cbu(rvr_uni(sxL), bnR[e], xi);
                  if (cl_pen_in(cbu, xi, P.eps)) {
                    pen = true;
                    dv[2] += cl_pen_ratio(anR[e], xi, cbu);
                  }
                }
              }
              iv[0] += __popcll(__ballot(live));
              if (v == 0) iv[1] += __popcll(__ballot(pen));
            }
          }
          iv[2] = (tid < A.nunits) ? static_cast<int>((cpk >> (10 * v)) & 1023ull) : 0;
          round_sums(v, dv, iv);
          if (v == 0) {
            pen_rs = dv[2];
            pen_cnt = iv[1];
          }
          ++n_trials;
          Fnew = dv[0];
          deltaF = Fnew - F;
          bool accept = true;
          if (deltaF < -P.eps) {
            alpha = alpha * P.beta;
            ++k_;
            if (k_ < P.maxlsiters) accept = false;
          }
          if (accept) {
            jstar = v;
            du2 = dv[1];
            lr = iv[0];
            no = iv[2];
            s = rvr_uni(sxL + v);
            u_c = cl_project(u_c, al, g_c) / nv;
            g_c = gn_c[v];
#pragma unroll
            for (int e = 0; e < 2; ++e) {
              UR[e] = rok[e] ? cl_project(UR[e], al, GR[e]) / nv : 0.0;
              GR[e] = rok[e] ? gR[e][v] : 0.0;
            }
          }
        }
        al = al * P.beta;
      }
      stamp_decided();
      if (jstar < 0) continue;
      const double deltau = sqrt(du2);
      F = Fnew;
      ++j_;
      nout = no;
      nlive = lr + nout;
      if (deltau < P.tol_u || fabs(deltaF) < P.tol_F || j_ >= P.maxiniters) {
        if (jstar == 0) {
          penalty = true;
        } else {
          kind = K_PAIR;
          continue;
        }
      } else {
        alpha = 1.0;
        k_ = 0;
        want_out = nout != 0 || view_wanted_v(A.rvp, m, true, A.rv_rows, nlive, nout, n_iters + 1 - n_redo, rv_builds, rv_last, rv_backoff);
        continue;
      }
    } else if (kind == K_PAIR) {
      double dv[3] = {0.0, 0.0, 0.0};
      int iv[3] = {0, 0, 0};
#pragma unroll
      for (int e = 0; e < 2; ++e) {
        const double cbu = s - bR[e] - UR[e];
        bool pen = false;
        if (rok[e] && cbu > P.eps && UR[e] > P.eps) {
          pen = true;
          dv[2] += fabs((aR[e] + UR[e]) / cbu);
        }
        iv[1] += __popcll(__ballot(pen));
      }
      round_sums(0, dv, iv);
      pen_rs = dv[2];
      pen_cnt = iv[1];
      penalty = true;
      stamp_decided();
    } else {
      double dv[3] = {0.0, 0.0, 0.0};
      int iv[3] = {0, 0, 0};
#pragma unroll
      for (int e = 0; e < 2; ++e) {
        bool live = false;
        if (rok[e]) {
          const double gi = cl_grad(d, UR[e], s, aR[e], bR[e]);
          GR[e] = gi;
          dv[0] += UR[e] * gi;
          live = UR[e] > 0.0 || gi > 0.0;
        }
        iv[0] += __popcll(__ballot(live));
      }
      iv[2] = (tid < A.nunits) ? static_cast<int>(cpk & 1023ull) : 0;
      round_sums(0, dv, iv);
      stamp_decided();
      if (cown) g_c = gn_c[0];
      F = dv[0];
      nout = iv[2];
      nlive = iv[0] + nout;
      j_ = 0;
      alpha = 1.0;
      k_ = 0;
      kind = K_TRIAL;
      want_out = nout != 0 || view_wanted_v(A.rvp, m, true, A.rv_rows, nlive, nout, n_iters + 1 - n_redo, rv_builds, rv_last, rv_backoff);
      continue;
    }
    if (penalty) {
      bool done = true;
      if (pen_cnt > 0) {
        d += pen_rs / static_cast<double>(pen_cnt);
        ++i_;
        done = i_ >= P.maxoliters;
      }
      if (!done) {
        kind = K_BUILD;
        continue;
      }
      write_point(true);
      if (blockIdx.x == 0 && A.kind != nullptr && A.marks != nullptr) {
        const int64_t n = (A.marks_n < KIND_CAP) ? A.marks_n : KIND_CAP;
        for (int64_t i = tid; i < n; i += RVR_NT)
          __hip_atomic_store(A.kind + i, A.marks[i], __ATOMIC_RELAXED, __HIP_MEMORY_SCOPE_SYSTEM);
      }
      if (arrive_last() && tid == 0) {
        SolverState* o = A.st;
        o->ubp = e_ubp ^ 1;
        o->ubv = 0;
        SolveShared* sh = A.shared;
        sh->F = F;
        sh->d = d;
        sh->n_passes = n_passes;
        sh->n_trials = n_trials;
        sh->ifinal = i_;
        sh->ubp = e_ubp ^ 1;
        sh->ubv = 0;
        sh->done = 1;
        report_run();
        if (A.host) {
          HostMirror* hm = A.host;
          __hip_atomic_store(&hm->F, F, __ATOMIC_RELAXED, __HIP_MEMORY_SCOPE_SYSTEM);
          __hip_atomic_store(&hm->d, d, __ATOMIC_RELAXED, __HIP_MEMORY_SCOPE_SYSTEM);
          __hip_atomic_store(&hm->n_passes, n_passes, __ATOMIC_RELAXED, __HIP_MEMORY_SCOPE_SYSTEM);
          __hip_atomic_store(&hm->n_trials, n_trials, __ATOMIC_RELAXED, __HIP_MEMORY_SCOPE_SYSTEM);
          __hip_atomic_store(&hm->n_view_passes, n_view_passes, __ATOMIC_RELAXED, __HIP_MEMORY_SCOPE_SYSTEM);
          __hip_atomic_store(&hm->nlive, nlive, __ATOMIC_RELAXED, __HIP_MEMORY_SCOPE_SYSTEM);
          __hip_atomic_store(&hm->nout, nout, __ATOMIC_RELAXED, __HIP_MEMORY_SCOPE_SYSTEM);
          __hip_atomic_store(&hm->iters, n_iters, __ATOMIC_RELAXED, __HIP_MEMORY_SCOPE_SYSTEM);
          __hip_atomic_store(&hm->ifinal, i_, __ATOMIC_RELAXED, __HIP_MEMORY_SCOPE_SYSTEM);
          __hip_atomic_store(&hm->ubp, e_ubp ^ 1, __ATOMIC_RELAXED, __HIP_MEMORY_SCOPE_SYSTEM);
          __hip_atomic_store(&hm->ubv, 0, __ATOMIC_RELAXED, __HIP_MEMORY_SCOPE_SYSTEM);
          __hip_atomic_store(&hm->done, 1, __ATOMIC_RELEASE, __HIP_MEMORY_SCOPE_SYSTEM);
        }
      }
      stamp_end();
      return;
    }
  }
}

}
```

clipper_amd/csrc/k_solver.hip.h:

```cpp
#pragma once

#include <hip/hip_runtime.h>
#include <stdint.h>
#include <type_traits>


namespace clipper_hip {


constexpr int VS = 8;
constexpr int nslot(int V) { return V + 1; }
constexpr int tail_nr(int V) { return 3 + 2 * V; }
constexpr int tail_q(int V) { return V * tail_nr(V) + 2 * V + 2; }

constexpr double LIVE_OUT = 67108864.0;
constexpr double RV_GAIN_MARGIN = 1.3;
constexpr double RV_ROWS_RATIO = 0.8;

struct ViewPolicy {
  int32_t on;
  int32_t max_builds;
  double pass_fixed, pass_per_row;
  double build_fixed, build_per_row;
};

enum Phase : int32_t {
  PH_NORMALIZE = 0,
  PH_RESCALE = 1,
  PH_INIT = 2,
  PH_TRIAL = 3,
  PH_PENALTY = 4,
  PH_BUILD = 5
};

enum Stage : int32_t {
  ST_PASS = 0,
  ST_RESULTS = 1
};

struct SolverState {
  double d;
  double F;
  double alpha;
  double s;
  double nrm[VS];
  double sx[VS];
  int32_t sel;
  int32_t ubp, ubv;
  int32_t phase;
  int32_t stage;
  int32_t i, j, k;
  int64_t n_passes;
  int64_t n_trials;
  int64_t n_iters;
  int32_t nlive;
  int32_t nout;
  int32_t view;
  int32_t hold;
  int64_t n_view_passes;
  int32_t rv_builds;
  int32_t rv_last;
  int32_t rv_backoff;
  int32_t hold_slot;
  int32_t hold_nlive;
  int32_t resume;
  int32_t weff;
  int32_t zero_run;
  int32_t n_redo;
  int32_t pad_;
};

struct SolveShared {
  double F, d;
  int64_t n_passes, n_trials;
  int32_t ifinal, ubp, ubv;
  int32_t done;
  int32_t hold;
  int32_t pad;
};

struct HostMirror {
  double F, d;
  int64_t n_passes, n_trials;
  int64_t iters;
  int32_t ifinal, ubp, ubv;
  int32_t done;
  int32_t nlive, nout;
  int64_t n_view_passes;
  int32_t hold;
  int32_t hold_nlive;
};

enum HoldReason : int32_t { HOLD_ROW_VIEW = 1, HOLD_SUB_ENTER = 2, HOLD_SUB_LEAVE = 3 };
enum PassMark : uint8_t { MARK_NONE = 0, MARK_WINDOW = 1, MARK_VIEW = 2, MARK_PAIR = 3, MARK_SUB_WINDOW = 4, MARK_SUB_PAIR = 5 };

struct SolverParams {
  double tol_u, tol_F, beta, eps;
  int32_t maxiniters, maxoliters, maxlsiters;
};


__device__ __forceinline__ double cl_project(double u, double al, double g) {
  const double t = u + al * g;
  return (t > 0.0) ? t : 0.0;
}

__device__ __forceinline__ double cl_norm(double z, bool use = true) { return (use && z > 0.0) ? sqrt(z) : 1.0; }

__device__ __forceinline__ double cl_grad(double d, double x, double s, double a, double b) {
  return (1 + d) * x - d * s + a + b * d;
}
__device__ __forceinline__ double cl_grad_fused(double d, double x, double s, double gs) {
  return (1 + d) * x - d * s + gs;
}

__device__ __forceinline__ double cl_pen_cbu(double s, double b, double u) { return s - b - u; }
__device__ __forceinline__ bool cl_pen_in(double cbu, double u, double eps) { return cbu > eps && u > eps; }
__device__ __forceinline__ double cl_pen_ratio(double a, double u, double cbu) { return fabs((a + u) / cbu); }
__device__ __forceinline__ double cl_pen_ratio_init(double a, double u, double cbu) { return (a + u) / cbu; }

constexpr double SUB_ENTER_MARGIN = 1.10;
constexpr double SUB_STAY_MARGIN = 1.01;

constexpr int TAIL_THREADS = 256;
constexpr int TAIL_WAVES = TAIL_THREADS / 64;
constexpr int TAIL_SPLIT = 1;

struct SolveArgs {
  const SolverState* st_cur;
  SolverState* st_next;
  SolveShared* shared;
  HostMirror* host;
  SolverParams prm;
  int64_t m;
  int64_t W;
  int64_t mp;
  const double* u0;
  double* pt;
  double* cab;
  const double* Xin;
  double* Xout;
  double* ab;
  double* part;
  int ntiles;
  int slot;
  double* scal;
  int nwg;
  const double* scal_in;
  int nwg_in;
  uint8_t* marks;
  uint8_t* kind;
  double* host_u;
  long long* stamps;
  int stamps_wide;
  const uint8_t* in_view;
  int rv_nslots;
  int rv_nwork;
  int rv_fresh;
  int rv_rows;
  ViewPolicy rvp;
  int decide_only;
  int adaptive_window;
  int sub_state;
  double sub_ncol;
  const int32_t* colmap;
};
constexpr int KIND_CAP = 1 << 16;


__device__ __forceinline__ double* pt_arr(const SolveArgs& A, int V, int p, int v, int k) {
  return A.pt + ((static_cast<int64_t>(p) * V + v) * 2 + k) * A.mp;
}

template <int CTRL, int ROW_MASK>
__device__ __forceinline__ double dpp_f64(double v) {
  const int lo = __builtin_amdgcn_update_dpp(0, __double2loint(v), CTRL, ROW_MASK, 0xf, false);
  const int hi = __builtin_amdgcn_update_dpp(0, __double2hiint(v), CTRL, ROW_MASK, 0xf, false);
  return __hiloint2double(hi, lo);
}

__device__ __forceinline__ double wave_sum_to_lane63(double v) {
  v += dpp_f64<0xB1, 0xf>(v);
  v += dpp_f64<0x4E, 0xf>(v);
  v += dpp_f64<0x141, 0xf>(v);
  v += dpp_f64<0x140, 0xf>(v);
  v += dpp_f64<0x142, 0xa>(v);
  v += dpp_f64<0x143, 0xc>(v);
  return v;
}

template <int N, int NWAVES>
__device__ __forceinline__ void block_reduce(double (&v)[N], double* lds ) {
#pragma unroll
  for (int q = 0; q < N; ++q) v[q] = wave_sum_to_lane63(v[q]);
  const int wave = threadIdx.x >> 6;
  __syncthreads();
  if ((threadIdx.x & 63) == 63) {
#pragma unroll
    for (int q = 0; q < N; ++q) lds[wave * N + q] = v[q];
  }
  __syncthreads();
#pragma unroll
  for (int q = 0; q < N; ++q) {
    double acc = lds[q];
#pragma unroll
    for (int w = 1; w < NWAVES; ++w) acc += lds[w * N + q];
    v[q] = acc;
  }
}

template <int N, int NWAVES>
__device__ __forceinline__ double block_reduce_pick(double (&v)[N], double* lds) {
#pragma unroll
  for (int q = 0; q < N; ++q) v[q] = wave_sum_to_lane63(v[q]);
  const int wave = threadIdx.x >> 6;
  __syncthreads();
  if ((threadIdx.x & 63) == 63) {
#pragma unroll
    for (int q = 0; q < N; ++q) lds[wave * N + q] = v[q];
  }
  __syncthreads();
  double acc = 0.0;
  if (threadIdx.x < N) {
    acc = lds[threadIdx.x];
#pragma unroll
    for (int w = 1; w < NWAVES; ++w) acc += lds[w * N + threadIdx.x];
  }
  return acc;
}

__device__ __forceinline__ void store_row(double* row, const double (&c)[VS]) {
  double4* q = reinterpret_cast<double4*>(row);
  q[0] = make_double4(c[0], c[1], c[2], c[3]);
  q[1] = make_double4(c[4], c[5], c[6], c[7]);
}

constexpr int pow2_at_least(int x) {
  int p = 1;
  while (p < x) p *= 2;
  return p;
}


__device__ __forceinline__ bool is_writer_block() {
  return blockIdx.x == gridDim.x - 1 && blockIdx.y == gridDim.y - 1;
}

__device__ __forceinline__ bool view_wanted_v(const ViewPolicy& rvp, int64_t m, bool have_view, int rv_rows,
                                              int nlive, int nout, int64_t n_iters, int builds, int last,
                                              int backoff) {
  if (builds >= rvp.max_builds || n_iters < 2 || n_iters - last < 3) return false;
  if (nlive <= 0 || nlive >= m) return false;
  const double rows_now = (have_view && nout == 0) ? static_cast<double>(rv_rows) : static_cast<double>(m);
  const double r = static_cast<double>(nlive);
  if (r > RV_ROWS_RATIO * rows_now) return false;
  if (backoff > 0 && r > RV_ROWS_RATIO * static_cast<double>(backoff)) return false;
  const double horizon = n_iters > 12 ? static_cast<double>(n_iters) : 12.0;
  const double gain = horizon * ((rows_now - r) * rvp.pass_per_row);
  return gain > RV_GAIN_MARGIN * (rvp.build_fixed + r * rvp.build_per_row);
}
__device__ __forceinline__ bool view_wanted(const SolveArgs& A, int nlive, int nout, int64_t n_iters,
                                            int builds, int last, int backoff) {
  return view_wanted_v(A.rvp, A.m, A.in_view != nullptr, A.rv_rows, nlive, nout, n_iters, builds, last, backoff);
}

__device__ __forceinline__ void copy_state(SolverState* dst, const SolverState* src, int tid, int nt) {
  static_assert(sizeof(SolverState) % 8 == 0, "copied in 8-byte words");
  const unsigned long long* s8 = reinterpret_cast<const unsigned long long*>(src);
  unsigned long long* d8 = reinterpret_cast<unsigned long long*>(dst);
  for (int k = tid; k < static_cast<int>(sizeof(SolverState) / 8); k += nt) d8[k] = s8[k];
}

struct PassPlan {
  int view;
  int phase;
  int sel;
  int from_u;
  double d;
  int src;
  double alpha0;
  int weff;
};

constexpr int VU = 4;
#define VEC_CHUNKS(base) for (int64_t base = tid; base < m; base += NT * VU)
#define VEC_EACH(k, i, base)            \
  _Pragma("unroll") for (int k = 0; k < VU; ++k) \
    if (const int64_t i = base + static_cast<int64_t>(k) * NT; i < m)

struct HeadLoads {
  int done, stage, phase;
  double d, F, alpha, s;
  int i, j, k, ubp, ubv, sel;
  int64_t n_passes, n_trials, n_iters, n_view_passes;
  int nlive, nout, hold, rv_builds, rv_last, rv_backoff, weff, zero_run, n_redo;
  double chain;
};

template <int V, int NT>
__device__ __forceinline__ void head_loads(const SolveArgs& A, HeadLoads& L) {
  constexpr int Q = tail_q(V);
  constexpr int QPAD = pow2_at_least(Q);
  constexpr int NCH = NT / QPAD;
  const SolverState* st = A.st_cur;
  L.done = A.shared->done;
  L.stage = st->stage;
  L.phase = st->phase;
  L.d = st->d;
  L.F = st->F;
  L.alpha = st->alpha;
  L.s = st->s;
  L.i = st->i;
  L.j = st->j;
  L.k = st->k;
  L.ubp = st->ubp;
  L.ubv = st->ubv;
  L.sel = st->sel;
  L.n_passes = st->n_passes;
  L.n_trials = st->n_trials;
  L.n_iters = st->n_iters;
  L.n_view_passes = st->n_view_passes;
  L.nlive = st->nlive;
  L.nout = st->nout;
  L.hold = st->hold;
  L.rv_builds = st->rv_builds;
  L.rv_last = st->rv_last;
  L.rv_backoff = st->rv_backoff;
  L.weff = st->weff;
  L.zero_run = st->zero_run;
  L.n_redo = st->n_redo;
  const int tid = threadIdx.x;
  const int q = tid & (QPAD - 1), c = tid / QPAD;
  double acc = 0.0;
  if (q < Q) {
    constexpr int U = 20;
    const double* p = A.scal_in + q;
    int w = c;
    for (; w + NCH * (U - 1) < A.nwg_in; w += NCH * U) {
      double x[U];
#pragma unroll
      for (int k = 0; k < U; ++k) x[k] = p[static_cast<int64_t>(w + NCH * k) * Q];
#pragma unroll
      for (int k = 0; k < U; ++k) acc += x[k];
    }
    if (w < A.nwg_in) {
      auto rest = [&](auto un) __attribute__((always_inline)) {
        constexpr int R = decltype(un)::value;
        double x[R];
#pragma unroll
        for (int k = 0; k < R; ++k) {
          const int ww = w + NCH * k;
          x[k] = p[static_cast<int64_t>(ww < A.nwg_in ? ww : w) * Q];
        }
#pragma unroll
        for (int k = 0; k < R; ++k)
          if (w + NCH * k < A.nwg_in) acc += x[k];
      };
      if (w + NCH * 4 >= A.nwg_in) rest(std::integral_constant<int, 4>{});
      else if (w + NCH * 10 >= A.nwg_in) rest(std::integral_constant<int, 10>{});
      else rest(std::integral_constant<int, U>{});
    }
  }
  L.chain = acc;
}

template <int V, int NT>
__device__ __forceinline__ bool decide(const SolveArgs& A, const HeadLoads& L, double* red,
                                       SolverState* stash, PassPlan& plan) {
  constexpr int NR = tail_nr(V);
  constexpr int PEN = V * NR + 2 * V;
  constexpr int Q = tail_q(V);
  constexpr int QPAD = pow2_at_least(Q);
  constexpr int NCH = NT / QPAD;
  constexpr int NWV = NT / 64;
  static_assert(QPAD <= NT && V <= VS, "window too large");
  double* scratch = red + NT;
  const SolverState* st = A.st_cur;
  const int tid = threadIdx.x;
  const int64_t m = A.m;
  const SolverParams P = A.prm;
  const bool writer = is_writer_block();

  const int phase = L.phase;
  double d = L.d, F = L.F, alpha = L.alpha, s = L.s;
  int i_ = L.i, j_ = L.j, k_ = L.k, ubp = L.ubp, ubv = L.ubv, sel = L.sel;
  const int wprev = (L.weff >= 1 && L.weff <= V) ? L.weff : V;
  int zero_run = L.zero_run;
  int64_t n_passes = L.n_passes, n_trials = L.n_trials;
  const int64_t n_iters = L.n_iters + 1;
  int nlive = L.nlive, nout = L.nout;
  auto live_code = [&](double code) {
    const double o = floor(code * (1.0 / LIVE_OUT));
    nout = static_cast<int>(o);
    nlive = static_cast<int>(code - o * LIVE_OUT);
  };
  if (writer && tid == 0) {
#pragma unroll
    for (int l = 0; l < V; ++l) {
      stash->nrm[l] = 1.0;
      stash->sx[l] = 0.0;
    }
  }
  enum { ACT_PASS, ACT_BUILD, ACT_SLOW, ACT_DONE };
  int action = ACT_SLOW;
  int next_phase = PH_TRIAL;
  bool need_pair = false;
  bool redo = false;
  bool sub_ok = true;
  auto sub_bound = [&](const double* sums, int nb) {
    if (A.sub_state == 0) return;
    const double kap = (A.sub_state == 1 ? SUB_ENTER_MARGIN : SUB_STAY_MARGIN) * A.sub_ncol;
    const double lhs = d * d, rhs = (1.0 + d) * (1.0 + d) * kap;
#pragma unroll
    for (int l = 0; l < V; ++l) {
      const double z = sums[nb + 2 * l], sl = sums[nb + 2 * l + 1];
      sub_ok = sub_ok && (lhs * sl * sl >= rhs * z);
    }
  };

  if (phase == PH_TRIAL || phase == PH_BUILD) {
    {
      red[tid] = L.chain;
      __syncthreads();
      double tot = 0.0;
      if (tid < QPAD) {
        tot = red[tid];
#pragma unroll
        for (int c2 = 1; c2 < NCH; ++c2) tot += red[c2 * QPAD + tid];
      }
      __syncthreads();
      if (tid < QPAD) red[tid] = tot;
      __syncthreads();
    }
    const double* sums = red;
    if (phase == PH_TRIAL) {
      int jstar = -1;
      double Fnew = 0.0, deltaF = 0.0;
#pragma unroll
      for (int v = 0; v < V; ++v) {
        if (jstar < 0 && v < wprev) {
          ++n_trials;
          Fnew = sums[v * NR + 0];
          deltaF = Fnew - F;
          bool accept = true;
          if (deltaF < -P.eps) {
            alpha = alpha * P.beta;
            ++k_;
            if (k_ < P.maxlsiters) accept = false;
          }
          if (accept) jstar = v;
        }
      }
      if (jstar < 0 && wprev < V) {
        alpha = L.alpha;
        k_ = L.k;
        n_trials = L.n_trials;
        zero_run = 0;
        redo = true;
        action = ACT_PASS;
        if (A.sub_state != 0) {
          const double kap = (A.sub_state == 1 ? SUB_ENTER_MARGIN : SUB_STAY_MARGIN) * A.sub_ncol;
          const double rhs = (1.0 + d) * (1.0 + d) * kap;
#pragma unroll
          for (int l = 0; l < V; ++l) {
            const double dsx = d * st->sx[l];
            sub_ok = sub_ok && (dsx * dsx >= rhs);
          }
        }
        if (writer && tid == 0) {
#pragma unroll
          for (int l = 0; l < V; ++l) {
            stash->nrm[l] = st->nrm[l];
            stash->sx[l] = st->sx[l];
          }
        }
      } else if (jstar < 0) {
        sel = V;
        action = ACT_PASS;
        sub_bound(sums, V * NR);
        if (writer && tid == 0) {
#pragma unroll
          for (int l = 0; l < V; ++l) {
            const double nl = cl_norm(sums[V * NR + 2 * l]);
            stash->nrm[l] = nl;
            stash->sx[l] = sums[V * NR + 2 * l + 1] / nl;
          }
        }
      } else {
        zero_run = (k_ == 0) ? (zero_run < 1000000 ? zero_run + 1 : zero_run) : 0;
        const double deltau = sqrt(sums[jstar * NR + 1]);
        live_code(sums[jstar * NR + NR - 1]);
        s = st->sx[jstar];
        F = Fnew;
        ubp ^= 1;
        ubv = jstar;
        ++j_;
        if (deltau < P.tol_u || fabs(deltaF) < P.tol_F || j_ >= P.maxiniters) {
          if (jstar == 0) {
            const double cnt = sums[PEN], rs = sums[PEN + 1];
            if (cnt > 0.0) {
              d += rs / cnt;
              ++i_;
              action = (i_ >= P.maxoliters) ? ACT_DONE : ACT_BUILD;
            } else {
              action = ACT_DONE;
            }
          } else {
            need_pair = true;
            action = ACT_PASS;
            next_phase = PH_PENALTY;
          }
        } else {
          alpha = 1.0;
          k_ = 0;
          sel = jstar;
          action = ACT_PASS;
          sub_bound(sums, jstar * NR + 2);
          if (writer && tid == 0) {
#pragma unroll
            for (int l = 0; l < V; ++l) {
              const double nl = cl_norm(sums[jstar * NR + 2 + 2 * l]);
              stash->nrm[l] = nl;
              stash->sx[l] = sums[jstar * NR + 3 + 2 * l] / nl;
            }
          }
        }
      }
    } else {
      F = sums[0];
      live_code(sums[NR - 1]);
      j_ = 0;
      if (P.maxiniters <= 0) {
        action = ACT_SLOW;
      } else {
        alpha = 1.0;
        k_ = 0;
        sel = 0;
        action = ACT_PASS;
        sub_bound(sums, 2);
        if (writer && tid == 0) {
#pragma unroll
          for (int l = 0; l < V; ++l) {
            const double nl = cl_norm(sums[2 + 2 * l]);
            stash->nrm[l] = nl;
            stash->sx[l] = sums[3 + 2 * l] / nl;
          }
        }
      }
    }
  }

  if (action == ACT_SLOW) {
    if (!writer) return false;
    nlive = nout = static_cast<int>(m < 0x7fffffff ? m : 0x7fffffff);
    const double* ca_ = A.cab;
    const double* cb_ = A.cab + A.mp;
    if (phase == PH_NORMALIZE || phase == PH_RESCALE) {
      double* u = pt_arr(A, V, ubp, ubv, 0);
      double z[1] = {0.0};
      VEC_CHUNKS(base) {
        double uv[VU], av[VU];
        VEC_EACH(k, i, base) {
          uv[k] = A.u0[i];
          if (phase == PH_RESCALE) av[k] = ca_[i];
        }
        VEC_EACH(k, i, base) {
          const double ui = (phase == PH_RESCALE) ? av[k] + uv[k] : uv[k];
          u[i] = ui;
          z[0] += ui * ui;
        }
      }
      block_reduce<1, NWV>(z, scratch);
      const double n0 = sqrt(z[0]);
      VEC_CHUNKS(base) {
        double uv[VU];
        VEC_EACH(k, i, base) uv[k] = u[i];
        VEC_EACH(k, i, base) {
          const double ui = uv[k] / n0;
          u[i] = ui;
          const double row[VS] = {ui, 0.0, 0.0, 0.0, 0.0, 0.0, 0.0, 0.0};
          store_row(A.Xout + i * VS, row);
        }
      }
      sel = 0;
      next_phase = PH_INIT;
    } else {
      if (phase == PH_INIT) {
        const double* u = pt_arr(A, V, ubp, ubv, 0);
        double sv[1] = {0.0};
        VEC_CHUNKS(base) {
          double uv[VU];
          VEC_EACH(k, i, base) uv[k] = u[i];
          VEC_EACH(k, i, base) sv[0] += uv[k];
        }
        block_reduce<1, NWV>(sv, scratch);
        s = sv[0];
        double ca[2] = {0.0, 0.0};
        VEC_CHUNKS(base) {
          double uv[VU], av[VU], bv[VU];
          VEC_EACH(k, i, base) {
            uv[k] = u[i];
            av[k] = ca_[i];
            bv[k] = cb_[i];
          }
          VEC_EACH(k, i, base) {
            const double cbu = cl_pen_cbu(s, bv[k], uv[k]);
            if (cl_pen_in(cbu, uv[k], P.eps)) {
              ca[0] += 1.0;
              ca[1] += cl_pen_ratio_init(av[k], uv[k], cbu);
            }
          }
        }
        block_reduce<2, NWV>(ca, scratch);
        d = (ca[0] > 0.0) ? ca[1] / ca[0] : 0.0;
        i_ = 0;
        action = (i_ >= P.maxoliters) ? ACT_DONE : ACT_BUILD;
      } else {
        const double* u = pt_arr(A, V, ubp, ubv, 0);
        double ca[2] = {0.0, 0.0};
        VEC_CHUNKS(base) {
          double uv[VU], av[VU], bv[VU];
          VEC_EACH(k, i, base) {
            uv[k] = u[i];
            av[k] = ca_[i];
            bv[k] = cb_[i];
          }
          VEC_EACH(k, i, base) {
            const double cbu = cl_pen_cbu(s, bv[k], uv[k]);
            if (cl_pen_in(cbu, uv[k], P.eps)) {
              ca[0] += 1.0;
              ca[1] += cl_pen_ratio(av[k], uv[k], cbu);
            }
          }
        }
        block_reduce<2, NWV>(ca, scratch);
        if (ca[0] > 0.0) {
          d += ca[1] / ca[0];
          ++i_;
          action = (i_ >= P.maxoliters) ? ACT_DONE : ACT_BUILD;
        } else {
          action = ACT_DONE;
        }
      }
    }
  }

  if (writer && action == ACT_DONE && A.host_u != nullptr) {
    const double* u = pt_arr(A, V, ubp, ubv, 0);
    for (int64_t i = tid; i < m; i += NT)
      __hip_atomic_store(A.host_u + (A.colmap != nullptr ? static_cast<int64_t>(A.colmap[i]) : i), u[i], __ATOMIC_RELAXED,
                         __HIP_MEMORY_SCOPE_SYSTEM);
    if (A.kind != nullptr && A.marks != nullptr) {
      const int64_t n = (n_iters < KIND_CAP) ? n_iters : KIND_CAP;
      for (int64_t i = tid; i < n; i += NT)
        __hip_atomic_store(A.kind + i, A.marks[i], __ATOMIC_RELAXED, __HIP_MEMORY_SCOPE_SYSTEM);
    }
    __threadfence_system();
    __syncthreads();
  }

  if (A.rv_fresh != 0 && action != ACT_SLOW) nout = 0;
  auto put_on_hold = [&](int reason) {
    if (writer) {
      copy_state(A.st_next, st, tid, NT);
      __syncthreads();
      if (tid == 0) {
        A.st_next->hold = reason;
        A.st_next->hold_slot = ubp * V + ubv;
        A.st_next->hold_nlive = nlive;
        A.shared->hold = reason;
        if (A.host != nullptr) {
          __hip_atomic_store(&A.host->hold_nlive, nlive, __ATOMIC_RELAXED, __HIP_MEMORY_SCOPE_SYSTEM);
          __hip_atomic_store(&A.host->hold, reason, __ATOMIC_RELEASE, __HIP_MEMORY_SCOPE_SYSTEM);
        }
      }
    }
  };
  if (action == ACT_PASS && next_phase == PH_TRIAL && A.rvp.on != 0 && A.rv_fresh == 0 && A.sub_state != 2 &&
      view_wanted(A, nlive, nout, n_iters - (L.n_redo + (redo ? 1 : 0)), L.rv_builds, L.rv_last, L.rv_backoff)) {
    put_on_hold(HOLD_ROW_VIEW);
    return false;
  }
  const bool on_view = A.in_view != nullptr && nout == 0 && action == ACT_PASS &&
                       (next_phase == PH_TRIAL || need_pair);
  if (A.sub_state == 1 && A.decide_only == 0 && on_view && next_phase == PH_TRIAL && !need_pair && sub_ok) {
    put_on_hold(HOLD_SUB_ENTER);
    return false;
  }
  const bool sub_leave = A.sub_state == 2 && action == ACT_PASS && !sub_ok;
  const int wnext = (A.adaptive_window != 0 && !redo && k_ == 0 && zero_run >= 2) ? 1 : V;
  if (writer && tid == 0) {
    auto record = [&](SolverState* o, bool norms_in_place) {
      o->d = d;
      o->F = F;
      o->alpha = alpha;
      o->s = s;
      if (!norms_in_place) {
#pragma unroll
        for (int l = 0; l < V; ++l) {
          o->nrm[l] = 1.0;
          o->sx[l] = 0.0;
        }
      }
      o->sel = sel;
      o->ubp = ubp;
      o->ubv = ubv;
      o->phase = (action == ACT_BUILD) ? static_cast<int>(PH_BUILD) : next_phase;
      o->stage = (action == ACT_SLOW) ? ST_PASS : ST_RESULTS;
      o->i = i_;
      o->j = j_;
      o->k = k_;
      o->n_passes = n_passes + (action == ACT_PASS ? 1 : 0);
      o->n_trials = n_trials;
      o->n_iters = n_iters;
      o->nlive = nlive;
      o->nout = nout;
      o->view = (action == ACT_PASS && on_view) ? 1 : 0;
      o->hold = 0;
      o->n_view_passes = L.n_view_passes + ((action == ACT_PASS && on_view) ? 1 : 0);
      o->rv_builds = L.rv_builds;
      o->rv_last = L.rv_last;
      o->rv_backoff = L.rv_backoff;
      o->hold_slot = 0;
      o->hold_nlive = 0;
      o->resume = 0;
      o->weff = wnext;
      o->zero_run = zero_run;
      o->n_redo = L.n_redo + (redo ? 1 : 0);
      o->pad_ = 0;
    };
    if (action == ACT_PASS) record(stash, true);
    else record(A.st_next, false);
    if ((A.decide_only != 0 || sub_leave) && action == ACT_PASS) {
      stash->stage = ST_PASS;
      stash->resume = need_pair ? 2 : 1;
      stash->n_passes = n_passes;
      stash->view = 0;
      stash->n_view_passes = L.n_view_passes;
      if (sub_leave) {
        stash->hold = HOLD_SUB_LEAVE;
        A.shared->hold = HOLD_SUB_LEAVE;
      }
    }
    if (action == ACT_DONE) {
      SolveShared* sh = A.shared;
      sh->F = F;
      sh->d = d;
      sh->n_passes = n_passes;
      sh->n_trials = n_trials;
      sh->ifinal = i_;
      sh->ubp = ubp;
      sh->ubv = ubv;
      sh->done = 1;
    }
    if (A.host != nullptr) {
      HostMirror* hm = A.host;
      if (action == ACT_DONE) {
        __hip_atomic_store(&hm->F, F, __ATOMIC_RELAXED, __HIP_MEMORY_SCOPE_SYSTEM);
        __hip_atomic_store(&hm->d, d, __ATOMIC_RELAXED, __HIP_MEMORY_SCOPE_SYSTEM);
        __hip_atomic_store(&hm->n_passes, n_passes, __ATOMIC_RELAXED, __HIP_MEMORY_SCOPE_SYSTEM);
        __hip_atomic_store(&hm->n_trials, n_trials, __ATOMIC_RELAXED, __HIP_MEMORY_SCOPE_SYSTEM);
        __hip_atomic_store(&hm->ifinal, i_, __ATOMIC_RELAXED, __HIP_MEMORY_SCOPE_SYSTEM);
        __hip_atomic_store(&hm->ubp, ubp, __ATOMIC_RELAXED, __HIP_MEMORY_SCOPE_SYSTEM);
        __hip_atomic_store(&hm->ubv, ubv, __ATOMIC_RELAXED, __HIP_MEMORY_SCOPE_SYSTEM);
        __hip_atomic_store(&hm->done, 1, __ATOMIC_RELEASE, __HIP_MEMORY_SCOPE_SYSTEM);
      }
      if (action != ACT_PASS || A.decide_only != 0 || sub_leave) {
        __hip_atomic_store(&hm->n_passes, n_passes, __ATOMIC_RELAXED, __HIP_MEMORY_SCOPE_SYSTEM);
        __hip_atomic_store(&hm->nlive, nlive, __ATOMIC_RELAXED, __HIP_MEMORY_SCOPE_SYSTEM);
        __hip_atomic_store(&hm->nout, nout, __ATOMIC_RELAXED, __HIP_MEMORY_SCOPE_SYSTEM);
        __hip_atomic_store(&hm->iters, n_iters, __ATOMIC_RELEASE, __HIP_MEMORY_SCOPE_SYSTEM);
        if (sub_leave) __hip_atomic_store(&hm->hold, HOLD_SUB_LEAVE, __ATOMIC_RELEASE, __HIP_MEMORY_SCOPE_SYSTEM);
      }
    }
  }
  if ((A.decide_only != 0 || sub_leave) && action == ACT_PASS) {
    if (writer) {
      __syncthreads();
      copy_state(A.st_next, stash, tid, NT);
    }
    return false;
  }
  plan.view = __builtin_amdgcn_readfirstlane(on_view ? 1 : 0);
  plan.phase = __builtin_amdgcn_readfirstlane(next_phase);
  plan.sel = __builtin_amdgcn_readfirstlane(sel);
  plan.from_u = __builtin_amdgcn_readfirstlane(need_pair ? ubp * V + ubv : -1);
  plan.d = __hiloint2double(__builtin_amdgcn_readfirstlane(__double2hiint(d)),
                            __builtin_amdgcn_readfirstlane(__double2loint(d)));
  plan.src = __builtin_amdgcn_readfirstlane(ubp * V + ubv);
  plan.alpha0 = __hiloint2double(__builtin_amdgcn_readfirstlane(__double2hiint(alpha)),
                                 __builtin_amdgcn_readfirstlane(__double2loint(alpha)));
  plan.weff = __builtin_amdgcn_readfirstlane(wnext);
  return action == ACT_PASS;
}
#undef VEC_CHUNKS
#undef VEC_EACH

template <int V, int NT>
__device__ __forceinline__ bool iteration_head(const SolveArgs& A, double* lds,
                                               SolverState* stash, PassPlan& plan) {
  const SolverState* st = A.st_cur;
  HeadLoads L;
  head_loads<V, NT>(A, L);
  if (L.done) return false;
  if (L.hold) {
    if (is_writer_block()) copy_state(A.st_next, st, threadIdx.x, NT);
    return false;
  }
  if (L.stage == ST_RESULTS) return decide<V, NT>(A, L, lds, stash, plan);
  const int resume = st->resume;
  const int slot = L.ubp * V + L.ubv;
  const int on_view = (resume != 0 && A.in_view != nullptr && L.nout == 0) ? 1 : 0;
  if (A.decide_only != 0) {
    if (is_writer_block()) copy_state(A.st_next, st, threadIdx.x, NT);
    return false;
  }
  plan.view = __builtin_amdgcn_readfirstlane(on_view);
  plan.phase = st->phase;
  plan.sel = st->sel;
  plan.from_u = __builtin_amdgcn_readfirstlane(resume == 2 ? slot : -1);
  plan.d = st->d;
  plan.src = __builtin_amdgcn_readfirstlane(slot);
  plan.alpha0 = L.alpha;
  plan.weff = __builtin_amdgcn_readfirstlane((A.adaptive_window != 0 && L.weff == 1) ? 1 : V);
  if (is_writer_block()) {
    copy_state(stash, st, threadIdx.x, NT);
    __syncthreads();
    if (resume == 3) {
      const bool all_rows = A.in_view == nullptr;
      double r[2 * V];
#pragma unroll
      for (int q = 0; q < 2 * V; ++q) r[q] = 0.0;
      const double* u = pt_arr(A, V, L.ubp, L.ubv, 0);
      const double* g = pt_arr(A, V, L.ubp, L.ubv, 1);
      const double beta = A.prm.beta;
      for (int64_t i = threadIdx.x; i < A.m; i += NT) {
        if (all_rows || A.in_view[i] == 0) {
          const double ui = u[i], gi = g[i];
          double al = L.alpha;
#pragma unroll
          for (int l = 0; l < V; ++l) {
            const double t = cl_project(ui, al, gi);
            r[2 * l] += t * t;
            r[2 * l + 1] += t;
            al = al * beta;
          }
        }
      }
      block_reduce<2 * V, NT / 64>(r, lds);
      if (threadIdx.x == 0) {
#pragma unroll
        for (int l = 0; l < V; ++l) {
          const double z = (all_rows ? 0.0 : stash->nrm[l]) + r[2 * l], sm = (all_rows ? 0.0 : stash->sx[l]) + r[2 * l + 1];
          const double nl = cl_norm(z);
          stash->nrm[l] = nl;
          stash->sx[l] = sm / nl;
        }
      }
      __syncthreads();
    }
    if (threadIdx.x == 0) {
      stash->stage = ST_RESULTS;
      stash->n_passes = L.n_passes + 1;
      stash->n_iters = L.n_iters + 1;
      stash->view = on_view;
      stash->n_view_passes = L.n_view_passes + on_view;
      stash->resume = 0;
      stash->weff = plan.weff;
    }
  }
  return true;
}

__device__ __forceinline__ void flush_state(const SolveArgs& A, const SolverState* stash) {
  if (!is_writer_block()) return;
  copy_state(A.st_next, stash, threadIdx.x, blockDim.x);
  if (threadIdx.x == 0) {
    const int64_t n_iters = stash->n_iters;
    if (A.marks != nullptr && n_iters <= KIND_CAP)
      A.marks[n_iters - 1] = A.sub_state == 2 ? (stash->phase == PH_TRIAL ? MARK_SUB_WINDOW : MARK_SUB_PAIR)
                             : stash->view   ? MARK_VIEW
                                             : (stash->phase == PH_TRIAL ? MARK_WINDOW : MARK_PAIR);
    if (A.host != nullptr) {
      __hip_atomic_store(&A.host->nlive, stash->nlive, __ATOMIC_RELAXED, __HIP_MEMORY_SCOPE_SYSTEM);
      __hip_atomic_store(&A.host->nout, stash->nout, __ATOMIC_RELAXED, __HIP_MEMORY_SCOPE_SYSTEM);
      __hip_atomic_store(&A.host->n_view_passes, stash->n_view_passes, __ATOMIC_RELAXED, __HIP_MEMORY_SCOPE_SYSTEM);
      __hip_atomic_store(&A.host->n_passes, stash->n_passes, __ATOMIC_RELAXED, __HIP_MEMORY_SCOPE_SYSTEM);
      __hip_atomic_store(&A.host->iters, n_iters, __ATOMIC_RELEASE, __HIP_MEMORY_SCOPE_SYSTEM);
    }
  }
}

__global__ __launch_bounds__(256) void k_init(SolveArgs A, SolverState init, SolverState* st0,
                                               double* X0) {
  const int64_t i = static_cast<int64_t>(blockIdx.x) * 256 + threadIdx.x;
  if (i < A.m) {
    const double row[VS] = {A.u0[i], 0.0, 0.0, 0.0, 0.0, 0.0, 0.0, 0.0};
    store_row(X0 + i * VS, row);
  }
  if (blockIdx.x == 0) {
    if (threadIdx.x == 0) {
      *st0 = init;
      A.shared->done = 0;
      A.shared->hold = 0;
    }
  }
}

constexpr int SCAL_FOLD = 32;
constexpr int SCAL_FOLD_MIN = 64;
__global__ __launch_bounds__(128) void k_scal_fold(const double* __restrict__ scal, int nwg, int Q,
                                                    double* __restrict__ out,
                                                    const SolveShared* __restrict__ shared) {
  if (shared->done) return;
  const int w0 = blockIdx.x * SCAL_FOLD;
  const int w1 = (w0 + SCAL_FOLD < nwg) ? w0 + SCAL_FOLD : nwg;
  for (int q = threadIdx.x; q < Q; q += 128) {
    double x[SCAL_FOLD];
#pragma unroll
    for (int k = 0; k < SCAL_FOLD; ++k) {
      const int w = (w0 + k < w1) ? w0 + k : w1 - 1;
      x[k] = scal[static_cast<int64_t>(w) * Q + q];
    }
    double acc = 0.0;
#pragma unroll
    for (int k = 0; k < SCAL_FOLD; ++k)
      if (w0 + k < w1) acc += x[k];
    out[static_cast<int64_t>(blockIdx.x) * Q + q] = acc;
  }
}

template <int V, bool FUSED_REDUCE, bool TABLES = true>
__global__ __launch_bounds__(TAIL_THREADS * (FUSED_REDUCE ? TAIL_SPLIT : 1)) void k_tail(SolveArgs A) {
  constexpr int NR = tail_nr(V);
  constexpr int Q = tail_q(V);
  constexpr int NRED = NR + 2 * V + 2;
  constexpr int NSLOT = nslot(V);
  constexpr int NTW = TAIL_WAVES * (FUSED_REDUCE ? TAIL_SPLIT : 1);
  __shared__ double red[NTW * NRED > 2 * TAIL_SPLIT * TAIL_THREADS ? NTW * NRED : 2 * TAIL_SPLIT * TAIL_THREADS];
  const int v = blockIdx.y;
  const long long c0 = A.stamps ? wall_clock64() : 0;
  const SolverState* st = A.st_next;
  const int te = threadIdx.x & (TAIL_THREADS - 1);
  const int grp = threadIdx.x / TAIL_THREADS;
  const int64_t i = static_cast<int64_t>(blockIdx.x) * TAIL_THREADS + te;
  const bool valid = i < A.m && grp == 0;
  const int done = A.shared->done;
  const int stage = st->stage, phase = st->phase;
  const int ubp = st->ubp, ubv = st->ubv, sel = st->sel;
  const double d = st->d, alpha = st->alpha, s_cur = st->s;
  const double nrmv = st->nrm[v], sxv = st->sx[v];
  const int weff = (st->weff >= 1 && st->weff <= V) ? st->weff : V;
  const int nslots_pass = st->view ? A.rv_nslots : A.ntiles;
  const double live_w = (valid && A.in_view != nullptr && A.in_view[i] == 0) ? 1.0 + LIVE_OUT : 1.0;

  double p0 = 0.0, p1 = 0.0;
  if (FUSED_REDUCE) {
    const int64_t o1 = (v == 0) ? static_cast<int64_t>(V) * A.W : 0;
    const int per = (nslots_pass + TAIL_SPLIT - 1) / TAIL_SPLIT;
    const int t0 = grp * per, t1 = (t0 + per < nslots_pass) ? t0 + per : nslots_pass;
    if (i < A.m) {
      const double* p = A.part + static_cast<int64_t>(v) * A.W + i;
      const int64_t ts = static_cast<int64_t>(NSLOT) * A.W;
      for (int t = t0; t < t1; t += 16) {
        double va[16], vb[16];
#pragma unroll
        for (int q = 0; q < 16; ++q) {
          const int tt = (t + q < t1) ? t + q : t1 - 1;
          va[q] = p[static_cast<int64_t>(tt) * ts];
          vb[q] = p[static_cast<int64_t>(tt) * ts + o1];
        }
#pragma unroll
        for (int q = 0; q < 16; ++q) {
          if (t + q < t1) {
            p0 += va[q];
            p1 += vb[q];
          }
        }
      }
    }
    if constexpr (TAIL_SPLIT > 1) {
      red[(grp * 2 + 0) * TAIL_THREADS + te] = p0;
      red[(grp * 2 + 1) * TAIL_THREADS + te] = p1;
      __syncthreads();
      p0 = red[te];
      p1 = red[TAIL_THREADS + te];
#pragma unroll
      for (int g = 1; g < TAIL_SPLIT; ++g) {
        p0 += red[(g * 2 + 0) * TAIL_THREADS + te];
        p1 += red[(g * 2 + 1) * TAIL_THREADS + te];
      }
      __syncthreads();
    }
  } else if (valid) {
    const int64_t o1 = (v == 0) ? static_cast<int64_t>(V) * A.W : 0;
    const uint32_t pb = static_cast<uint32_t>(i) / static_cast<uint32_t>(A.W);
    const int64_t off = i - static_cast<int64_t>(pb) * A.W;
    const double* blk = A.ab + (static_cast<int64_t>(pb) * NSLOT) * A.W;
    p0 = blk[static_cast<int64_t>(v) * A.W + off];
    p1 = blk[o1 + off];
  }
  if (done) return;
  if (st->hold) return;
  if (stage != ST_RESULTS) return;
  if (phase == PH_TRIAL && v >= weff) return;
  const long long c1 = A.stamps ? wall_clock64() + (p0 > 1e300 ? 1 : 0) : 0;

  if (phase != PH_TRIAL && phase != PH_BUILD) {
    if (v == 0 && valid) {
      A.cab[i] = p0;
      A.cab[A.mp + i] = p1;
    }
    return;
  }
  const double beta = A.prm.beta;
  double r[NRED];
#pragma unroll
  for (int q = 0; q < NRED; ++q) r[q] = 0.0;

  if (phase == PH_BUILD) {
    if (v != 0) return;
    if (valid) {
      const double ui = pt_arr(A, V, ubp, ubv, 0)[i];
      const double gi = (1 + d) * ui - d * s_cur + A.cab[i] + A.cab[A.mp + i] * d;
      pt_arr(A, V, ubp, ubv, 1)[i] = gi;
      r[0] = ui * gi;
      r[NR - 1] = (ui > 0.0 || gi > 0.0) ? live_w : 0.0;
      double row[VS] = {0.0, 0.0, 0.0, 0.0, 0.0, 0.0, 0.0, 0.0};
      double al = 1.0;
#pragma unroll
      for (int l = 0; l < V; ++l) {
        const double t = cl_project(ui, al, gi);
        row[l] = t;
        r[2 + 2 * l] = t * t;
        r[3 + 2 * l] = t;
        al = al * beta;
      }
      if constexpr (TABLES) store_row(A.Xout + i * VS, row);
    }
  } else {
    if (valid) {
      const double ui = pt_arr(A, V, ubp, ubv, 0)[i];
      double xraw;
      if constexpr (TABLES) {
        xraw = A.Xin[(static_cast<int64_t>(sel) * A.mp + i) * VS + v];
      } else {
        double al = alpha;
        for (int l = 0; l < v; ++l) al = al * beta;
        xraw = cl_project(ui, al, pt_arr(A, V, ubp, ubv, 1)[i]);
      }
      const double xi = xraw / nrmv;
      double gn;
      if (v == 0) {
        const double an = p0 / nrmv, bn = p1 / nrmv;
        gn = cl_grad(d, xi, sxv, an, bn);
        A.cab[i] = an;
        A.cab[A.mp + i] = bn;
        const double cbu = cl_pen_cbu(sxv, bn, xi);
        if (cl_pen_in(cbu, xi, A.prm.eps)) {
          r[NR + 2 * V] = 1.0;
          r[NR + 2 * V + 1] = cl_pen_ratio(an, xi, cbu);
        }
      } else {
        const double gs = p0 / nrmv;
        gn = cl_grad_fused(d, xi, sxv, gs);
      }
      pt_arr(A, V, ubp ^ 1, v, 0)[i] = xi;
// ... 52 lines not shown
```

include/clipper_hip.h:

```cpp
#ifndef CLIPPER_HIP_H
#define CLIPPER_HIP_H

#include <stddef.h>

#include "clipper_abi.h"

#ifdef __cplusplus
extern "C" {
#endif

typedef struct clipper_hip_ctx clipper_hip_t;

enum {
  CLIPPER_HIP_STORE_F32 = 0,
  CLIPPER_HIP_STORE_F64 = 1,
  CLIPPER_HIP_STORE_F32_CSC = 2,
  CLIPPER_HIP_STORE_F64_CSC = 3
};

enum {
  CLIPPER_HIP_OK = 0,
  CLIPPER_HIP_E_INVALID = -1,
  CLIPPER_HIP_E_NOMEM = -2,
  CLIPPER_HIP_E_HIP = -3,
  CLIPPER_HIP_E_NODEVICE = -4,
  CLIPPER_HIP_E_STATE = -5,
  CLIPPER_HIP_E_COMM = -6,
  CLIPPER_HIP_E_SCOPE = -7,
  CLIPPER_HIP_E_INTERNAL = -8
};

typedef struct clipper_hip_timings_t {
  double affinity_kernel_ms;
  double affinity_total_ms;
  double solve_total_ms;
  double gemv_avg_us;
  double gemv_min_us;
  int64_t gemv_launches;
  double gemv_bytes;
  double gemv_useful_bytes;
  double affinity_bytes;
  double exchange_avg_us;
  int64_t exchange_samples;
  double exchange_bytes;
} clipper_hip_timings_t;

typedef struct clipper_hip_view_stats_t {
  int64_t builds;
  int64_t rows;
  int64_t bytes;
  int64_t view_passes;
  int64_t passes;
  double build_ms;
  double view_pass_avg_us;
  int64_t view_pass_samples;
  int64_t resident_launches;
  int64_t resident_giveups;
  int64_t resident_iterations;
  double resident_us;
  double resident_event_us;
  int64_t resident_entries;
  int64_t resident_units;
  int64_t sub_entries;
  int64_t sub_leaves;
  int64_t sub_passes;
  int64_t sub_rows;
  int64_t sub_bytes;
  double sub_build_ms;
  double sub_pass_avg_us;
  int64_t sub_pass_samples;
  int64_t sub_dense;
} clipper_hip_view_stats_t;


int clipper_hip_device_count(void);

clipper_hip_t* clipper_hip_create(int device, int storage);

clipper_hip_t* clipper_hip_create_group(const int* devices, int nshards, int storage);

clipper_hip_t* clipper_hip_create_rank(int device, int storage, int rank, int world);
int clipper_hip_comm_unique_id(void* id128);
int clipper_hip_comm_init(clipper_hip_t* h, const void* id128);
typedef int (*clipper_hip_allgather_fn)(void* user, const void* sendbuf, void* recvbuf, size_t bytes);
int clipper_hip_comm_init_callback(clipper_hip_t* h, clipper_hip_allgather_fn fn, void* user);

void clipper_hip_destroy(clipper_hip_t* h);
const char* clipper_hip_last_error(void);


int clipper_hip_affinity_euclidean(clipper_hip_t* h, const double* D1, int d, int64_t n1,
                                   const double* D2, int64_t n2, const int32_t* A, int64_t m,
                                   double sigma, double epsilon, double mindist,
                                   double affinityeps);

int clipper_hip_affinity_pointnormal(clipper_hip_t* h, const double* D1, int d, int64_t n1,
                                     const double* D2, int64_t n2, const int32_t* A, int64_t m,
                                     double sigp, double epsp, double sign, double epsn,
                                     double affinityeps);

int clipper_hip_stage_inputs(clipper_hip_t* h, const double* D1, int d, int64_t n1,
                             const double* D2, int64_t n2, const int32_t* A, int64_t m);
int clipper_hip_affinity_euclidean_staged(clipper_hip_t* h, double sigma, double epsilon,
                                          double mindist, double affinityeps);
int clipper_hip_affinity_pointnormal_staged(clipper_hip_t* h, double sigp, double epsp,
                                            double sign, double epsn, double affinityeps);


#define CLIPPER_HIP_INVARIANT_MAX_D 32
#define CLIPPER_HIP_INVARIANT_MAX_PARAMS 16
typedef struct clipper_hip_invariant clipper_hip_invariant_t;

int clipper_hip_invariant_create(const char* source, int d, clipper_hip_invariant_t** out);
int clipper_hip_invariant_destroy(clipper_hip_invariant_t* inv);

int clipper_hip_affinity_custom_staged(clipper_hip_t* h, const clipper_hip_invariant_t* inv,
                                       const double* params, int nparams, double affinityeps);
int clipper_hip_affinity_custom(clipper_hip_t* h, const clipper_hip_invariant_t* inv, const double* D1, int d,
                                int64_t n1, const double* D2, int64_t n2, const int32_t* A, int64_t m,
                                const double* params, int nparams, double affinityeps);

int64_t clipper_hip_num_associations(const clipper_hip_t* h);
int clipper_hip_get_associations(const clipper_hip_t* h, int32_t* A_out );


int clipper_hip_set_matrix(clipper_hip_t* h, const double* M, const double* C, int64_t m);

int clipper_hip_set_sparse(clipper_hip_t* h, int64_t m, const int64_t* Mcolptr,
                           const int32_t* Mrow, const double* Mval, const int64_t* Ccolptr,
                           const int32_t* Crow, const double* Cval);

int clipper_hip_get_matrix(clipper_hip_t* h, double* M_out, double* C_out);


int clipper_hip_solve(clipper_hip_t* h, const double* u0, const clipper_params_t* params,
                      double* u_out, clipper_solve_info_t* info);

int clipper_hip_stage_u0(clipper_hip_t* h, const double* u0);
int clipper_hip_solve_staged(clipper_hip_t* h, const clipper_params_t* params, double* u_out,
                             clipper_solve_info_t* info);

int clipper_hip_get_nodes(const clipper_hip_t* h, int32_t* nodes_out, int32_t capacity);
int clipper_hip_get_selected_associations(const clipper_hip_t* h, int32_t* A_out,
                                          int32_t capacity);

int clipper_hip_densest_subgraph(clipper_hip_t* h, const int32_t* S, int32_t k,
                                 int32_t* nodes_out, int32_t capacity);


enum { CLIPPER_HIP_MC_EXACT = 0, CLIPPER_HIP_MC_HEU = 1, CLIPPER_HIP_MC_KCORE = 2 };
typedef struct clipper_maxclique_info_t {
  int32_t num_nodes;
  int32_t max_core;
  int32_t heuristic_size;
  int32_t timed_out;
  int64_t edges;
  int64_t roots_searched;
  int64_t roots_pruned;
  int64_t bb_nodes;
  double seconds;
} clipper_maxclique_info_t;
int clipper_hip_max_clique(clipper_hip_t* h, int method, double time_limit_s, clipper_maxclique_info_t* info);
typedef struct clipper_maxclique_seed_info_t {
  int32_t seed_given;
  int32_t seed_kept;
  int32_t seed_size;
  int32_t winner;
} clipper_maxclique_seed_info_t;
enum { CLIPPER_HIP_MC_SEED_ONLY = 3 };
int clipper_hip_max_clique_seeded(clipper_hip_t* h, int method, double time_limit_s, const int32_t* seed, int32_t nseed,
                                  clipper_maxclique_info_t* info, clipper_maxclique_seed_info_t* seed_info);
int clipper_hip_core_numbers(clipper_hip_t* h, int32_t* core_out );


#define CLIPPER_HIP_SDP_MAX_N 128
#define CLIPPER_HIP_SDP_WIDE_MAX_N 1024
enum { CLIPPER_HIP_SDP_ROUTE_WORKGROUP = 0,
       CLIPPER_HIP_SDP_ROUTE_AUTO      = 1,
       CLIPPER_HIP_SDP_ROUTE_WIDE      = 2 };
int clipper_hip_sdp_set_route(int route);
int clipper_hip_sdp_route(void);
typedef struct clipper_sdp_params_t {
  int32_t verbose;
  int32_t max_iters;
  int32_t acceleration_interval;
  int32_t acceleration_lookback;
  float eps_abs;
  float eps_rel;
  float eps_infeas;
  float time_limit_secs;
} clipper_sdp_params_t;
typedef struct clipper_sdp_info_t {
  int32_t iters;
  int32_t converged;
  int32_t timed_out;
  int32_t num_nodes;
  int32_t sweeps;
  int32_t route;
  double pobj;
  double dobj;
  double r_prim;
  double r_dual;
  double rho;
  double thr;
  double t_total;
  double t_setup;
  double t_solve;
  double t_extract;
} clipper_sdp_info_t;
int clipper_hip_sdp(clipper_hip_t* h, const clipper_sdp_params_t* params, double* X_out, double* Y_out,
                    double* lambdas_out, double* evec1_out, clipper_sdp_info_t* info);
int clipper_hip_sdp_solve(int device, const double* M, const double* C, int64_t n, const clipper_sdp_params_t* params,
                          double* X_out, double* Y_out, double* lambdas_out, double* evec1_out, int32_t* nodes_out,
                          clipper_sdp_info_t* info);
typedef struct clipper_sdp_problem_t {
  const double* M;
  const double* C;
  int64_t n;
  double* X_out;
  double* Y_out;
  double* lambdas_out;
  double* evec1_out;
  int32_t* nodes_out;
} clipper_sdp_problem_t;
int clipper_hip_sdp_solve_batch(int device, const clipper_sdp_problem_t* problems, int32_t count,
                                const clipper_sdp_params_t* params, clipper_sdp_info_t* infos);


int clipper_hip_knn(int device, const double* P0, int64_t n0, const double* P1, int64_t n1, int d,
                    int knn, int32_t* idx_out, double* sqd_out);

int64_t clipper_hip_distance_based_correspondences(int device, const double* P0, int64_t n0,
                                                   const double* P1, int64_t n1, int d, int knn,
                                                   double radius, int enforce_1to1,
                                                   int32_t* A_out, int64_t capacity);

typedef struct {
  int32_t knn;
  int32_t mutual;
  double  ratio;
  double  max_sqdist;
} clipper_match_params_t;

int64_t clipper_hip_match_descriptors(int device, const double* F0, int64_t n0, const double* F1, int64_t n1, int d,
                                      const clipper_match_params_t* params,
                                      int32_t* A_out, double* sqd_out, int64_t capacity,
                                      int32_t* nn_idx_out, double* nn_sqd_out);

int clipper_hip_set_window(clipper_hip_t* h, int window);
int clipper_hip_window(const clipper_hip_t* h);

int clipper_hip_set_resident(clipper_hip_t* h, int mode);
int clipper_hip_last_solver(const clipper_hip_t* h);

int clipper_hip_set_row_view(clipper_hip_t* h, int mode);
int clipper_hip_get_view_stats(const clipper_hip_t* h, clipper_hip_view_stats_t* out);

int clipper_hip_set_subproblem(clipper_hip_t* h, int mode);

int clipper_hip_view_matvec(clipper_hip_t* h, const int32_t* rows, int64_t nrows, const double* x,
                            double* yM, double* yC);

int clipper_hip_storage_in_use(const clipper_hip_t* h);

int clipper_hip_matvec(clipper_hip_t* h, const double* x, double* yM, double* yC);


int clipper_hip_set_profiling(clipper_hip_t* h, int on);
int clipper_hip_get_timings(const clipper_hip_t* h, clipper_hip_timings_t* out);
int clipper_hip_bench_matvec(clipper_hip_t* h, int reps, double* avg_us);
int64_t clipper_hip_read_ply_xyz(const char* path, double* pts_out, int64_t capacity);
int clipper_hip_generate_synthetic_correspondences(int64_t n0, int64_t n1, const int32_t* Agood,
                                                   int64_t p, int64_t m, double rho, uint64_t seed,
                                                   int32_t* A_out, int32_t* Agt_out,
                                                   int64_t* ni_out);
int clipper_hip_precision_recall(const int32_t* A, int64_t na, const int32_t* Agt, int64_t ngt,
                                 double* precision, double* recall);
int clipper_hip_estimate_rigid_transform(const double* D1, int64_t n1, const double* D2, int64_t n2,
                                         const int32_t* A, int64_t k, double* T_out);

int clipper_hip_debug_stamps(clipper_hip_t* h, int64_t* out, int capacity);

int clipper_hip_debug_occupy(int device, int workgroups, int lds_bytes, double milliseconds);

int clipper_hip_device_info(const clipper_hip_t* h, char* name64, int* cus, int64_t* hbm_bytes);

typedef struct clipper_hip_batch clipper_hip_batch_t;
typedef struct {
  const double* D1; int64_t n1;
  const double* D2; int64_t n2;
  const int32_t* A; int64_t m;
  const double* u0;
} clipper_batch_problem_t;
int clipper_hip_batch_create(int device, int storage, clipper_hip_batch_t** out);
void clipper_hip_batch_destroy(clipper_hip_batch_t* b);
int clipper_hip_batch_solve_euclidean(clipper_hip_batch_t* b, const clipper_batch_problem_t* p, int32_t n,
                                      int d, double sigma, double epsilon, double mindist, const clipper_params_t* prm);
int clipper_hip_batch_solve_pointnormal(clipper_hip_batch_t* b, const clipper_batch_problem_t* p, int32_t n,
                                        double sigp, double epsp, double sign, double epsn, const clipper_params_t* prm);
int clipper_hip_batch_solve_custom(clipper_hip_batch_t* b, const clipper_hip_invariant_t* inv,
                                   const clipper_batch_problem_t* p, int32_t n, const double* params, int nparams,
                                   const clipper_params_t* prm);
int clipper_hip_batch_get_solution(const clipper_hip_batch_t* b, int32_t i, double* u_out, clipper_solve_info_t* info);
int clipper_hip_batch_get_nodes(const clipper_hip_batch_t* b, int32_t i, int32_t* nodes_out, int32_t capacity);
int clipper_hip_batch_get_selected_associations(const clipper_hip_batch_t* b, int32_t i, int32_t* A_out, int32_t capacity);
int clipper_hip_batch_route(const clipper_hip_batch_t* b, int32_t i);
int clipper_hip_batch_get_stats(const clipper_hip_batch_t* b, int32_t* launches, int32_t* n_batched, int32_t* n_alone);
int clipper_hip_batch_get_split(const clipper_hip_batch_t* b, double* fill_ms, double* launch_ms, double* alone_ms,
                                double* round_ms);
int clipper_hip_batch_sdp(clipper_hip_batch_t* b, const clipper_sdp_params_t* params, clipper_sdp_info_t* infos);
int clipper_hip_batch_max_clique(clipper_hip_batch_t* b, int method, double time_limit_s,
                                 clipper_maxclique_info_t* infos );
int clipper_hip_batch_max_clique_seeded(clipper_hip_batch_t* b, int method, double time_limit_s, const int32_t* seeds,
                                        const int64_t* offsets, clipper_maxclique_info_t* infos,
                                        clipper_maxclique_seed_info_t* seed_infos);
int clipper_hip_batch_max_clique_stats(const clipper_hip_batch_t* b, int32_t* launches, int32_t* n_batched,
                                       int32_t* n_alone);
int clipper_hip_batch_get_sdp(const clipper_hip_batch_t* b, int32_t i, double* X_out, double* Y_out,
                              double* lambdas_out, double* evec1_out);

#ifdef __cplusplus
}
#endif
#endif
```

Measured before the change: 1.299.

## Add adaptive single-column window turns to the resident view solver kernel

The persistent view-resident solver kernel now templates each turn on window width. When the adaptive window heuristic predicts the line search will accept alpha=1 (zero_run >= 2, k == 0), it runs a width-1 pass instead of the full V-wide window, and redoes the turn at full width if the guess fails. This is meant to cut GEMV traffic and reduction work per turn. The cost is extra turns on mispredicted guesses, plus new redo and single-turn counters in the stats and host mirror.

Result: slower. 1.349 (+3.9%).

```diff
diff --git a/clipper_amd/_abi.py b/clipper_amd/_abi.py
--- a/clipper_amd/_abi.py
+++ b/clipper_amd/_abi.py
@@ -106,6 +106,7 @@
         ("sub_entries", C.c_int64), ("sub_leaves", C.c_int64), ("sub_passes", C.c_int64),
         ("sub_rows", C.c_int64), ("sub_bytes", C.c_int64), ("sub_build_ms", C.c_double),
         ("sub_pass_avg_us", C.c_double), ("sub_pass_samples", C.c_int64), ("sub_dense", C.c_int64),
+        ("resident_single_turns", C.c_int64), ("resident_redos", C.c_int64), ("window_redos", C.c_int64),
     ]
 
 
diff --git a/clipper_amd/csrc/host_rv_resident.hpp b/clipper_amd/csrc/host_rv_resident.hpp
--- a/clipper_amd/csrc/host_rv_resident.hpp
+++ b/clipper_amd/csrc/host_rv_resident.hpp
@@ -25,7 +25,7 @@
   ViewResident& r = h->vres;
   r.launches_this_solve = 0;
   r.ev_n = 0;
-  if (r.giveup_host) std::memset(r.giveup_host, 0, RVR_GIVEUP_SLOTS * 4 * sizeof(uint32_t));
+  if (r.giveup_host) std::memset(r.giveup_host, 0, RVR_GIVEUP_SLOTS * RVR_REPORT_WORDS * sizeof(uint32_t));
   std::atomic_thread_fence(std::memory_order_seq_cst);
 }
 
@@ -37,11 +37,14 @@
   int gave_up = 0;
   volatile const uint32_t* w = r.giveup_host;
   for (int k = 0; k < std::min(r.launches_this_solve, RVR_GIVEUP_SLOTS); ++k) {
-    if (w[4 * k] != 0u) {
+    const volatile uint32_t* wk = w + RVR_REPORT_WORDS * k;
+    if (wk[0] != 0u) {
       ++gave_up;
     } else {
-      h->rv_stats.resident_iterations += static_cast<int64_t>(w[4 * k + 1]);
-      h->rv_stats.resident_us += static_cast<double>(static_cast<uint64_t>(w[4 * k + 2]) | (static_cast<uint64_t>(w[4 * k + 3]) << 32)) * 1e-2;
+      h->rv_stats.resident_iterations += static_cast<int64_t>(wk[1]);
+      h->rv_stats.resident_us += static_cast<double>(static_cast<uint64_t>(wk[2]) | (static_cast<uint64_t>(wk[3]) << 32)) * 1e-2;
+      h->rv_stats.resident_single_turns += static_cast<int64_t>(wk[4]);
+      h->rv_stats.resident_redos += static_cast<int64_t>(wk[5]);
     }
   }
   for (int k = 0; k < r.ev_n; ++k) {
@@ -177,9 +180,9 @@
     HIPCHK(hipMemsetAsync(r.ctl, 0, RVR_GIVEUP_SLOTS * 64, s.stream));
   }
   if (!r.giveup_host) {
-    HIPCHK(hipHostMalloc(reinterpret_cast<void**>(&r.giveup_host), RVR_GIVEUP_SLOTS * 4 * sizeof(uint32_t), hipHostMallocMapped | hipHostMallocCoherent));
+    HIPCHK(hipHostMalloc(reinterpret_cast<void**>(&r.giveup_host), RVR_GIVEUP_SLOTS * RVR_REPORT_WORDS * sizeof(uint32_t), hipHostMallocMapped | hipHostMallocCoherent));
     HIPCHK(hipHostGetDevicePointer(reinterpret_cast<void**>(&r.giveup_host_dev), r.giveup_host, 0));
-    std::memset(r.giveup_host, 0, RVR_GIVEUP_SLOTS * 4 * sizeof(uint32_t));
+    std::memset(r.giveup_host, 0, RVR_GIVEUP_SLOTS * RVR_REPORT_WORDS * sizeof(uint32_t));
   }
   r.nunits = static_cast<int>(plan.units.size());
   r.plan_entries = plan.entries;
@@ -234,14 +237,18 @@
   r.epoch += 1ull << 20;
   const bool own_ctl = r.launches_this_solve < RVR_GIVEUP_SLOTS;
   a.ctl = r.ctl + (own_ctl ? 16 * r.launches_this_solve : 0);
-  a.giveup_host = (r.giveup_host_dev && r.launches_this_solve < RVR_GIVEUP_SLOTS) ? r.giveup_host_dev + 4 * r.launches_this_solve : nullptr;
+  a.giveup_host = (r.giveup_host_dev && r.launches_this_solve < RVR_GIVEUP_SLOTS) ? r.giveup_host_dev + RVR_REPORT_WORDS * r.launches_this_solve : nullptr;
   a.lds_slices = r.lds_slices;
   a.timeout_ticks = 200000ll;
   if (r.epoch == 0) a.timeout_ticks = 2000000ll;
   if (const char* e = std::getenv("CLIPPER_HIP_VIEW_RESIDENT_TIMEOUT_TICKS")) a.timeout_ticks = std::atoll(e);
   a.max_exchanges = 1 << 18;
   if (const char* e = std::getenv("CLIPPER_HIP_VIEW_RESIDENT_MAX_EXCHANGES"))
-    a.max_exchanges = std::min((1 << 20) - 1, std::max(0, std::atoi(e)));
+    a.max_exchanges = std::min((1 << 19) - 1, std::max(0, std::atoi(e)));
+  a.window_in_use = (!r.on_replica && h->csc_valid && h->world == 1 && !h->multiproc && h->sh.size() == 1 && h->adaptive_window) ? 1 : 0;
+  if (a.window_in_use != 0)
+    if (const char* e = std::getenv("CLIPPER_HIP_VIEW_RESIDENT_FORCE_SINGLE"))
+      if (std::atoi(e) != 0) a.window_in_use = 2;
   a.rvp = h->rvp;
   a.rv_rows = static_cast<int>(s.rv.nrows);
   a.stamps = h->stamps_dev;
@@ -343,18 +350,18 @@
   if (!launched) {
     r.launches_this_solve += 1;
     h->rv_stats.resident_launches += 1;
-    if (r.giveup_host && slot < RVR_GIVEUP_SLOTS) r.giveup_host[4 * slot] = RVR_ERR_STATE;
+    if (r.giveup_host && slot < RVR_GIVEUP_SLOTS) r.giveup_host[RVR_REPORT_WORDS * slot] = RVR_ERR_STATE;
   }
   HIPCHK(hipStreamSynchronize(s.stream));
   std::atomic_thread_fence(std::memory_order_acquire);
-  const bool ran = launched && !(r.giveup_host && slot < RVR_GIVEUP_SLOTS && static_cast<volatile uint32_t*>(r.giveup_host)[4 * slot] != 0u);
+  const bool ran = launched && !(r.giveup_host && slot < RVR_GIVEUP_SLOTS && static_cast<volatile uint32_t*>(r.giveup_host)[RVR_REPORT_WORDS * slot] != 0u);
   bool all_ran = false;
   if ((rc = rvr_agree(h, ran, all_ran))) return rc;
   if (!all_ran) {
     if (ran) {
       HIPCHK(hipMemcpyAsync(s.st + h->par, r.backup, sizeof(SolverState), hipMemcpyDeviceToDevice, s.stream));
       HIPCHK(hipMemcpyAsync(s.shared, r.backup + sizeof(SolverState), sizeof(SolveShared), hipMemcpyDeviceToDevice, s.stream));
-      if (r.giveup_host && slot < RVR_GIVEUP_SLOTS) r.giveup_host[4 * slot] = RVR_ERR_PEER;
+      if (r.giveup_host && slot < RVR_GIVEUP_SLOTS) r.giveup_host[RVR_REPORT_WORDS * slot] = RVR_ERR_PEER;
     }
     r.ready = false;
   }
diff --git a/clipper_amd/csrc/host_solve.hpp b/clipper_amd/csrc/host_solve.hpp
--- a/clipper_amd/csrc/host_solve.hpp
+++ b/clipper_amd/csrc/host_solve.hpp
@@ -231,6 +231,7 @@
   }
   fin = mirror_result(hm);
   h->rv_stats.view_passes = hm->n_view_passes;
+  h->rv_stats.window_redos = hm->n_redo;
   return 0;
 }
 
diff --git a/clipper_amd/csrc/k_rv_resident.hip.h b/clipper_amd/csrc/k_rv_resident.hip.h
--- a/clipper_amd/csrc/k_rv_resident.hip.h
+++ b/clipper_amd/csrc/k_rv_resident.hip.h
@@ -50,11 +50,14 @@
   const uint8_t* marks;
   uint8_t* kind;
   int64_t marks_n;
+  int window_in_use;
 };
+constexpr int RVR_REPORT_WORDS = 8;
 constexpr int RVR_FINE0 = 5120, RVR_FINE_TURNS = 96;
 enum : int {
   RVR_F_KIND = 0, RVR_F_ROUNDS = 1, RVR_F_XT = 2 , RVR_F_NORMS = 3 ,
   RVR_F_SUMS = 4 , RVR_F_TAIL = 5 ,
+  RVR_F_WIDTH = 6 ,
   RVR_F_ROUND = 8 ,
   RVR_F_DECIDED = 14 , RVR_F_WAVE = 16
 };
@@ -133,7 +136,6 @@
 template <typename VT, int V, bool FINE>
 __global__ __launch_bounds__(RVR_NT) void k_solve_view_resident(RvrArgs A) {
   extern __shared__ __attribute__((aligned(16))) uint8_t rvr_lds[];
-  constexpr int NS = V + 1;
   constexpr int QB = 4 * static_cast<int>(sizeof(VT));
   typedef uint32_t u32x4 __attribute__((ext_vector_type(4)));
   static_assert(V >= 2 && V <= 6 && (V % 2) == 0, "window of the streaming solver on slices");
@@ -326,7 +328,9 @@
   int64_t n_passes = st->n_passes, n_trials = st->n_trials, n_iters = st->n_iters, n_view_passes = st->n_view_passes;
   int nlive = st->nlive, nout = 0;
   const int rv_builds = st->rv_builds, rv_last = st->rv_last, rv_backoff = st->rv_backoff;
-  const int n_redo = st->n_redo;
+  int n_redo = st->n_redo;
+  int zero_run = st->zero_run;
+  int n_single = 0, n_redo_here = 0;
 
   const double* Ue = A.pt + ((static_cast<int64_t>(e_ubp) * V + e_ubv) * 2 + 0) * mp;
   const double* Ge = A.pt + ((static_cast<int64_t>(e_ubp) * V + e_ubv) * 2 + 1) * mp;
@@ -399,6 +403,8 @@
       __hip_atomic_store(A.giveup_host + 1, static_cast<uint32_t>(exchanges), __ATOMIC_RELAXED, __HIP_MEMORY_SCOPE_SYSTEM);
       __hip_atomic_store(A.giveup_host + 2, static_cast<uint32_t>(dt & 0xffffffffull), __ATOMIC_RELAXED, __HIP_MEMORY_SCOPE_SYSTEM);
       __hip_atomic_store(A.giveup_host + 3, static_cast<uint32_t>(dt >> 32), __ATOMIC_RELAXED, __HIP_MEMORY_SCOPE_SYSTEM);
+      __hip_atomic_store(A.giveup_host + 4, static_cast<uint32_t>(n_single), __ATOMIC_RELAXED, __HIP_MEMORY_SCOPE_SYSTEM);
+      __hip_atomic_store(A.giveup_host + 5, static_cast<uint32_t>(n_redo_here), __ATOMIC_RELAXED, __HIP_MEMORY_SCOPE_SYSTEM);
     }
   };
   auto write_point = [&](bool to_host) __attribute__((always_inline)) {
@@ -414,10 +420,11 @@
   enum { K_TRIAL = 0, K_PAIR = 1, K_BUILD = 2 };
   int kind = (e_resume == 2) ? K_PAIR : K_TRIAL;
   bool want_out = false;
+  bool redo = false;
   for (;;) {
     trow = stamp_row;
     stamp(0);
-    const bool out_now = kind != K_BUILD && (exchanges >= A.max_exchanges || (kind == K_TRIAL ? want_out : nout != 0));
+    const bool out_now = kind != K_BUILD && (exchanges - n_redo_here >= A.max_exchanges || (kind == K_TRIAL ? want_out : nout != 0));
     if (out_now) {
       const int resume = (kind == K_TRIAL) ? (nout != 0 ? 3 : 1) : 2;
       const bool window = kind == K_TRIAL;
@@ -474,7 +481,8 @@
         o->hold_nlive = 0;
         o->resume = resume;
         o->weff = V;
-        o->zero_run = 0;
+        o->zero_run = zero_run;
+        o->n_redo = n_redo;
         report_run();
         if (A.host) {
           HostMirror* hm = A.host;
@@ -488,455 +496,481 @@
       return;
     }
 
-    fstamp_value(RVR_F_KIND, kind);
-    double y[NS];
-#pragma unroll
-    for (int v = 0; v < NS; ++v) y[v] = 0.0;
-    if (kind != K_BUILD) {
-#pragma unroll
-      for (int e = 0; e < 2; ++e) {
-        const int r = tid + e * RVR_NT;
-        if (r < nrows) {
-          double al = alpha;
-#pragma unroll
-          for (int l = 0; l < V; ++l) {
-            double t = cl_project(UR[e], al, GR[e]);
-            if (kind == K_PAIR) t = (l == 0) ? UR[e] : 0.0;
-            Xt[r * V + l] = t;
-            al = al * P.beta;
-          }
-        }
-      }
-      __syncthreads();
-      fstamp(RVR_F_XT);
-      double acc[NS];
-      rs_wave_pass<VT, V>(sl, toff, pc, np, 0, Xt, (kind == K_TRIAL) ? d : 0.0, acc, G, lgrp * SL_SUB);
-      if constexpr (FINE) {
-        if (A.stamps && unit == 0 && lane == 0 && trow < RVR_FINE_TURNS)
-          A.stamps[RVR_FINE0 + trow * 32 + RVR_F_WAVE + wave] = wall_clock64() + (acc[0] > 1e300 ? 1 : 0);
-      }
-      if (wave < V) {
-        double z = 0.0, t1 = 0.0;
-        if (kind == K_TRIAL) {
-          for (int r = lane; r < nrows; r += 64) {
-            const double c = Xt[r * V + wave];
-            z += c * c;
-            t1 += c;
-          }
-          z = wave_sum_to_lane63(z);
-          t1 = wave_sum_to_lane63(t1);
-        }
-        if (lane == 63) {
-          const double nl = cl_norm(z, kind == K_TRIAL);
-          nrmL[wave] = nl;
-          sxL[wave] = (kind == K_TRIAL) ? t1 / nl : 0.0;
-        }
-      }
-      __syncthreads();
-      fstamp(RVR_F_NORMS);
-      if (packed) {
-        for (int o = Wd; o < 64; o <<= 1) {
-#pragma unroll
-          for (int v = 0; v < NS; ++v) acc[v] += __shfl_xor(acc[v], o);
-        }
-      }
-#pragma unroll
-      for (int v = 0; v < NS; ++v) scr[(wave * NS + v) * 64 + lane] = acc[v];
-      __syncthreads();
-      if (wave < U.ncgs) {
-        uint32_t mine = 0;
-#pragma unroll
-        for (int w = 0; w < RVR_NWV; ++w) mine |= (static_cast<int>((wcg >> (8 * w)) & 255ull) == wave) ? (1u << w) : 0u;
-#pragma unroll
-        for (int v = 0; v < NS; ++v) {
-          double sum = 0.0;
-#pragma unroll
-          for (int w = 0; w < RVR_NWV; ++w) {
-            const double t = scr[(w * NS + v) * 64 + lane];
-            sum += ((mine >> w) & 1u) ? t : 0.0;
-          }
-          y[v] = sum;
-        }
-      }
-      fstamp(RVR_F_SUMS, y[0]);
-    }
-    stamp(1);
-    ++epoch;
-    ++exchanges;
-    const int par = static_cast<int>(epoch & 1ull);
-    const unsigned long long tag = (epoch & 0xffffffffull) << 32;
-    double gn_c[V], an_c = a_c, bn_c = b_c;
-    uint32_t cbits = 0;
-    if (kind == K_TRIAL) {
-      double al = alpha;
-#pragma unroll
-      for (int v = 0; v < V; ++v) {
-        const double t = cl_project(u_c, al, g_c);
-        const double nv = rvr_uni(nrmL + v), sv = rvr_uni(sxL + v);
-        const double xi = t / nv;
-        double gn;
-        if (v == 0) {
-          an_c = y[0] / nv;
-          bn_c = y[V] / nv;
-          gn = cl_grad(d, xi, sv, an_c, bn_c);
-        } else {
-          const double gs = y[v] / nv;
-          gn = cl_grad_fused(d, xi, sv, gs);
-        }
-        gn_c[v] = gn;
-        if (cown && rpos < 0 && (xi > 0.0 || gn > 0.0)) cbits |= 1u << v;
-        if (cown && rpos >= 0) rvr_publish(sec_g(par, v, rpos), tag, gn);
-        al = al * P.beta;
-      }
-    } else {
-#pragma unroll
-      for (int v = 0; v < V; ++v) gn_c[v] = 0.0;
-      if (kind == K_PAIR) {
-        an_c = y[0];
-        bn_c = y[V];
-      } else if (cown) {
-        gn_c[0] = cl_grad(d, u_c, s, a_c, b_c);
-        if (rpos < 0 && (u_c > 0.0 || gn_c[0] > 0.0)) cbits = 1u;
-      }
-    }
-    if (kind != K_BUILD && cown && rpos >= 0) {
-      rvr_publish(sec_g(par, V, rpos), tag, an_c);
-      rvr_publish(sec_g(par, V + 1, rpos), tag, bn_c);
-    }
-    a_c = an_c;
-    b_c = bn_c;
-    fstamp(RVR_F_TAIL, a_c + gn_c[V - 1]);
-    if (U.ncgs == 1) {
-      if (wave == 0) {
-        unsigned long long pk = 0;
-#pragma unroll
-        for (int v = 0; v < V; ++v) pk |= static_cast<unsigned long long>(__popcll(__ballot((cbits >> v) & 1u))) << (10 * v);
-        if (lane == 0) rvr_publish(sec_c(par, unit), tag, __longlong_as_double(static_cast<long long>(pk)));
-      }
-      __syncthreads();
-    } else {
-      unsigned long long w = 0;
-#pragma unroll
-      for (int v = 0; v < V; ++v) w |= static_cast<unsigned long long>(__popcll(__ballot((cbits >> v) & 1u))) << (7 * v);
-      if (lane == 0) reinterpret_cast<unsigned long long*>(tot)[wave] = w;
-      __syncthreads();
-      if (tid == 0) {
-        unsigned long long pk = 0;
-#pragma unroll
-        for (int v = 0; v < V; ++v) {
-          unsigned long long tsum = 0;
-          for (int w2 = 0; w2 < RVR_NWV; ++w2) tsum += (reinterpret_cast<unsigned long long*>(tot)[w2] >> (7 * v)) & 127ull;
-          pk |= tsum << (10 * v);
-        }
-        rvr_publish(sec_c(par, unit), tag, __longlong_as_double(static_cast<long long>(pk)));
-      }
-      __syncthreads();
-    }
-    stamp(2);
-
-    double gR[2][V], anR[2], bnR[2];
-    unsigned long long cpk = 0;
-#pragma unroll
-    for (int e = 0; e < 2; ++e) {
-      anR[e] = aR[e];
-      bnR[e] = bR[e];
-#pragma unroll
-      for (int v = 0; v < V; ++v) gR[e][v] = 0.0;
-    }
-    {
-      const uint32_t tag32 = static_cast<uint32_t>(epoch & 0xffffffffull);
-      int fail = 0;
-      const long long t_poll = wall_clock64();
-      for (unsigned spins = 0;; ++spins) {
-        bool ok = true;
+    const bool guess = A.window_in_use == 2 ? !redo : window_guess(A.window_in_use, redo, k_, zero_run);
+    const bool narrow = A.window_in_use != 0 && (kind != K_TRIAL || guess);
+    redo = false;
+    auto turn = [&](auto wc) __attribute__((always_inline)) -> int {
+      constexpr int W = decltype(wc)::value;
+      constexpr int NSW = W + 1;
+      fstamp_value(RVR_F_KIND, kind);
+      fstamp_value(RVR_F_WIDTH, W);
+      double y[NSW];
+#pragma unroll
+      for (int v = 0; v < NSW; ++v) y[v] = 0.0;
+      if (kind != K_BUILD) {
 #pragma unroll
         for (int e = 0; e < 2; ++e) {
           const int r = tid + e * RVR_NT;
-          if ((e == 0 || two) && rok[e] && kind != K_BUILD) {
-            rvr_u4 w[V + 2];
-            if (kind == K_TRIAL) {
-#pragma unroll
-              for (int v = 0; v < V; ++v) w[v] = rvr_ld16(sec_g(par, v, r));
+          if (r < nrows) {
+            double al = alpha;
+#pragma unroll
+            for (int l = 0; l < W; ++l) {
+              double t = cl_project(UR[e], al, GR[e]);
+              if (kind == K_PAIR) t = (l == 0) ? UR[e] : 0.0;
+              Xt[r * W + l] = t;
+              al = al * P.beta;
             }
-            w[V] = rvr_ld16(sec_g(par, V, r));
-            w[V + 1] = rvr_ld16(sec_g(par, V + 1, r));
+          }
+        }
+        __syncthreads();
+        fstamp(RVR_F_XT);
+        double acc[NSW];
+        rs_wave_pass<VT, W>(sl, toff, pc, np, 0, Xt, (kind == K_TRIAL) ? d : 0.0, acc, G, lgrp * SL_SUB);
+        if constexpr (FINE) {
+          if (A.stamps && unit == 0 && lane == 0 && trow < RVR_FINE_TURNS)
+            A.stamps[RVR_FINE0 + trow * 32 + RVR_F_WAVE + wave] = wall_clock64() + (acc[0] > 1e300 ? 1 : 0);
+        }
+        if (wave < W) {
+          double z = 0.0, t1 = 0.0;
+          if (kind == K_TRIAL) {
+            for (int r = lane; r < nrows; r += 64) {
+              const double c = Xt[r * W + wave];
+              z += c * c;
+              t1 += c;
+            }
+            z = wave_sum_to_lane63(z);
+            t1 = wave_sum_to_lane63(t1);
+          }
+          if (lane == 63) {
+            const double nl = cl_norm(z, kind == K_TRIAL);
+            nrmL[wave] = nl;
+            sxL[wave] = (kind == K_TRIAL) ? t1 / nl : 0.0;
+          }
+        }
+        __syncthreads();
+        fstamp(RVR_F_NORMS);
+        if (packed) {
+          for (int o = Wd; o < 64; o <<= 1) {
+#pragma unroll
+            for (int v = 0; v < NSW; ++v) acc[v] += __shfl_xor(acc[v], o);
+          }
+        }
+#pragma unroll
+        for (int v = 0; v < NSW; ++v) scr[(wave * NSW + v) * 64 + lane] = acc[v];
+        __syncthreads();
+        if (wave < U.ncgs) {
+          uint32_t mine = 0;
+#pragma unroll
+          for (int w = 0; w < RVR_NWV; ++w) mine |= (static_cast<int>((wcg >> (8 * w)) & 255ull) == wave) ? (1u << w) : 0u;
+#pragma unroll
+          for (int v = 0; v < NSW; ++v) {
+            double sum = 0.0;
+#pragma unroll
+            for (int w = 0; w < RVR_NWV; ++w) {
+              const double t = scr[(w * NSW + v) * 64 + lane];
+              sum += ((mine >> w) & 1u) ? t : 0.0;
+            }
+            y[v] = sum;
+          }
+        }
+        fstamp(RVR_F_SUMS, y[0]);
+      }
+      stamp(1);
+      ++epoch;
+      ++exchanges;
+      const int par = static_cast<int>(epoch & 1ull);
+      const unsigned long long tag = (epoch & 0xffffffffull) << 32;
+      double gn_c[W], an_c = a_c, bn_c = b_c;
+      uint32_t cbits = 0;
+      if (kind == K_TRIAL) {
+        double al = alpha;
+#pragma unroll
+        for (int v = 0; v < W; ++v) {
+          const double t = cl_project(u_c, al, g_c);
+          const double nv = rvr_uni(nrmL + v), sv = rvr_uni(sxL + v);
+          const double xi = t / nv;
+          double gn;
+          if (v == 0) {
+            an_c = y[0] / nv;
+            bn_c = y[W] / nv;
+            gn = cl_grad(d, xi, sv, an_c, bn_c);
+          } else {
+            const double gs = y[v] / nv;
+            gn = cl_grad_fused(d, xi, sv, gs);
+          }
+          gn_c[v] = gn;
+          if (cown && rpos < 0 && (xi > 0.0 || gn > 0.0)) cbits |= 1u << v;
+          if (cown && rpos >= 0) rvr_publish(sec_g(par, v, rpos), tag, gn);
+          al = al * P.beta;
+        }
+      } else {
+#pragma unroll
+        for (int v = 0; v < W; ++v) gn_c[v] = 0.0;
+        if (kind == K_PAIR) {
+          an_c = y[0];
+          bn_c = y[W];
+        } else if (cown) {
+          gn_c[0] = cl_grad(d, u_c, s, a_c, b_c);
+          if (rpos < 0 && (u_c > 0.0 || gn_c[0] > 0.0)) cbits = 1u;
+        }
+      }
+      if (kind != K_BUILD && cown && rpos >= 0) {
+        rvr_publish(sec_g(par, V, rpos), tag, an_c);
+        rvr_publish(sec_g(par, V + 1, rpos), tag, bn_c);
+      }
+      a_c = an_c;
+      b_c = bn_c;
+      fstamp(RVR_F_TAIL, a_c + gn_c[W - 1]);
+      if (U.ncgs == 1) {
+        if (wave == 0) {
+          unsigned long long pk = 0;
+#pragma unroll
+          for (int v = 0; v < W; ++v) pk |= static_cast<unsigned long long>(__popcll(__ballot((cbits >> v) & 1u))) << (10 * v);
+          if (lane == 0) rvr_publish(sec_c(par, unit), tag, __longlong_as_double(static_cast<long long>(pk)));
+        }
+        __syncthreads();
+      } else {
+        unsigned long long w = 0;
+#pragma unroll
+        for (int v = 0; v < W; ++v) w |= static_cast<unsigned long long>(__popcll(__ballot((cbits >> v) & 1u))) << (7 * v);
+        if (lane == 0) reinterpret_cast<unsigned long long*>(tot)[wave] = w;
+        __syncthreads();
+        if (tid == 0) {
+          unsigned long long pk = 0;
+#pragma unroll
+          for (int v = 0; v < W; ++v) {
+            unsigned long long tsum = 0;
+            for (int w2 = 0; w2 < RVR_NWV; ++w2) tsum += (reinterpret_cast<unsigned long long*>(tot)[w2] >> (7 * v)) & 127ull;
+            pk |= tsum << (10 * v);
+          }
+          rvr_publish(sec_c(par, unit), tag, __longlong_as_double(static_cast<long long>(pk)));
+        }
+        __syncthreads();
+      }
+      stamp(2);
+
+      double gR[2][W], anR[2], bnR[2];
+      unsigned long long cpk = 0;
+#pragma unroll
+      for (int e = 0; e < 2; ++e) {
+        anR[e] = aR[e];
+        bnR[e] = bR[e];
+#pragma unroll
+        for (int v = 0; v < W; ++v) gR[e][v] = 0.0;
+      }
+      {
+        const uint32_t tag32 = static_cast<uint32_t>(epoch & 0xffffffffull);
+        int fail = 0;
+        const long long t_poll = wall_clock64();
+        for (unsigned spins = 0;; ++spins) {
+          bool ok = true;
+#pragma unroll
+          for (int e = 0; e < 2; ++e) {
+            const int r = tid + e * RVR_NT;
+            if ((e == 0 || two) && rok[e] && kind != K_BUILD) {
+              rvr_u4 w[W + 2];
+              if (kind == K_TRIAL) {
+#pragma unroll
+                for (int v = 0; v < W; ++v) w[v] = rvr_ld16(sec_g(par, v, r));
+              }
+              w[W] = rvr_ld16(sec_g(par, V, r));
+              w[W + 1] = rvr_ld16(sec_g(par, V + 1, r));
+              rvr_wait_loads();
+              if (kind == K_TRIAL) {
+#pragma unroll
+                for (int v = 0; v < W; ++v) {
+                  rvr_tie(w[v]);
+                  ok = rvr_take(w[v], tag32, gR[e][v]) && ok;
+                }
+              }
+              rvr_tie(w[W]);
+              rvr_tie(w[W + 1]);
+              ok = rvr_take(w[W], tag32, anR[e]) && ok;
+              ok = rvr_take(w[W + 1], tag32, bnR[e]) && ok;
+            }
+          }
+          if (tid < A.nunits) {
+            rvr_u4 w = rvr_ld16(sec_c(par, tid));
             rvr_wait_loads();
-            if (kind == K_TRIAL) {
-#pragma unroll
-              for (int v = 0; v < V; ++v) {
-                rvr_tie(w[v]);
-                ok = rvr_take(w[v], tag32, gR[e][v]) && ok;
+            rvr_tie(w);
+            double cd;
+            ok = rvr_take(w, tag32, cd) && ok;
+            cpk = static_cast<unsigned long long>(__double_as_longlong(cd));
+          }
+          if (__all(ok)) break;
+          if ((spins & 63u) == 63u || A.timeout_ticks < 0) {
+            const bool late = wall_clock64() - t_poll > A.timeout_ticks;
+            const uint32_t e2 = __hip_atomic_load(A.ctl, __ATOMIC_RELAXED, __HIP_MEMORY_SCOPE_AGENT);
+            if (late || e2 != 0) {
+              fail = 1;
+              break;
+            }
+          }
+        }
+        if (__syncthreads_or(fail)) {
+          if (tid == 0) {
+            uint32_t expect = 0;
+            if (__hip_atomic_compare_exchange_strong(A.ctl, &expect, static_cast<uint32_t>(RVR_ERR_TIMEOUT), __ATOMIC_RELAXED,
+                                                     __ATOMIC_RELAXED, __HIP_MEMORY_SCOPE_AGENT) &&
+                A.giveup_host)
+              __hip_atomic_store(A.giveup_host, static_cast<uint32_t>(RVR_ERR_TIMEOUT), __ATOMIC_RELAXED, __HIP_MEMORY_SCOPE_SYSTEM);
+          }
+          return 1;
+        }
+      }
+      stamp(3);
+#pragma unroll
+      for (int e = 0; e < 2; ++e) {
+        aR[e] = anR[e];
+        bR[e] = bnR[e];
+      }
+
+      double* rbuf = red;
+      int* ibuf = reinterpret_cast<int*>(red + V * RVR_NWV * 4);
+      int nrounds = 0;
+      auto round_sums = [&](int rd, double (&dv)[3], int (&iv)[3]) __attribute__((always_inline)) {
+#pragma unroll
+        for (int q = 0; q < 3; ++q) dv[q] = wave_sum_to_lane63(dv[q]);
+        if (wave * 64 < A.nunits) iv[2] = wave_isum_to_lane63(iv[2]);
+        if (lane == 63) {
+#pragma unroll
+          for (int q = 0; q < 3; ++q) rbuf[(rd * RVR_NWV + wave) * 4 + q] = dv[q];
+#pragma unroll
+          for (int q = 0; q < 3; ++q) ibuf[(rd * RVR_NWV + wave) * 4 + q] = iv[q];
+        }
+        __syncthreads();
+#pragma unroll
+        for (int q = 0; q < 3; ++q) {
+          double acc = rbuf[(rd * RVR_NWV) * 4 + q];
+          int iacc = ibuf[(rd * RVR_NWV) * 4 + q];
+#pragma unroll
+          for (int w = 1; w < RVR_NWV; ++w) {
+            acc += rbuf[(rd * RVR_NWV + w) * 4 + q];
+            iacc += ibuf[(rd * RVR_NWV + w) * 4 + q];
+          }
+          dv[q] = __hiloint2double(__builtin_amdgcn_readfirstlane(__double2hiint(acc)),
+                                   __builtin_amdgcn_readfirstlane(__double2loint(acc)));
+          iv[q] = __builtin_amdgcn_readfirstlane(iacc);
+        }
+        fstamp(RVR_F_ROUND + rd);
+        ++nrounds;
+      };
+      auto stamp_decided = [&]() {
+        stamp(4);
+        fstamp(RVR_F_DECIDED);
+        fstamp_value(RVR_F_ROUNDS, nrounds);
+      };
+      ++n_iters;
+      if (kind != K_BUILD) {
+        ++n_passes;
+        ++n_view_passes;
+      }
+      ++stamp_row;
+      bool penalty = false;
+      int pen_cnt = 0;
+      double pen_rs = 0.0;
+      if (kind == K_TRIAL) {
+        int jstar = -1;
+        double Fnew = 0.0, deltaF = 0.0, du2 = 0.0;
+        int lr = 0, no = 0;
+        const double alpha_w = alpha;
+        const int k_w = k_;
+        if constexpr (W < V) ++n_single;
+        double al = alpha_w;
+#pragma unroll
+        for (int v = 0; v < W; ++v) {
+          if (jstar < 0) {
+            double dv[3] = {0.0, 0.0, 0.0};
+            int iv[3] = {0, 0, 0};
+            const double nv = rvr_uni(nrmL + v);
+#pragma unroll
+            for (int e = 0; e < 2; ++e) {
+              if (e == 0 || two) {
+                const double xi = cl_project(UR[e], al, GR[e]) / nv;
+                const double gv = gR[e][v];
+                bool live = false, pen = false;
+                if (rok[e]) {
+                  dv[0] += xi * gv;
+                  const double du = xi - UR[e];
+                  dv[1] += du * du;
+                  live = xi > 0.0 || gv > 0.0;
+                  if (v == 0) {
+                    const double cbu = cl_pen_cbu(rvr_uni(sxL), bnR[e], xi);
+                    if (cl_pen_in(cbu, xi, P.eps)) {
+                      pen = true;
+                      dv[2] += cl_pen_ratio(anR[e], xi, cbu);
+                    }
+                  }
+                }
+                iv[0] += __popcll(__ballot(live));
+                if (v == 0) iv[1] += __popcll(__ballot(pen));
               }
             }
-            rvr_tie(w[V]);
-            rvr_tie(w[V + 1]);
-            ok = rvr_take(w[V], tag32, anR[e]) && ok;
-            ok = rvr_take(w[V + 1], tag32, bnR[e]) && ok;
-          }
-        }
-        if (tid < A.nunits) {
-          rvr_u4 w = rvr_ld16(sec_c(par, tid));
-          rvr_wait_loads();
-          rvr_tie(w);
-          double cd;
-          ok = rvr_take(w, tag32, cd) && ok;
-          cpk = static_cast<unsigned long long>(__double_as_longlong(cd));
-        }
-        if (__all(ok)) break;
-        if ((spins & 63u) == 63u || A.timeout_ticks < 0) {
-          const bool late = wall_clock64() - t_poll > A.timeout_ticks;
-          const uint32_t e2 = __hip_atomic_load(A.ctl, __ATOMIC_RELAXED, __HIP_MEMORY_SCOPE_AGENT);
-          if (late || e2 != 0) {
-            fail = 1;
-            break;
-          }
-        }
-      }
-      if (__syncthreads_or(fail)) {
-        if (tid == 0) {
-          uint32_t expect = 0;
-          if (__hip_atomic_compare_exchange_strong(A.ctl, &expect, static_cast<uint32_t>(RVR_ERR_TIMEOUT), __ATOMIC_RELAXED,
-                                                   __ATOMIC_RELAXED, __HIP_MEMORY_SCOPE_AGENT) &&
-              A.giveup_host)
-            __hip_atomic_store(A.giveup_host, static_cast<uint32_t>(RVR_ERR_TIMEOUT), __ATOMIC_RELAXED, __HIP_MEMORY_SCOPE_SYSTEM);
-        }
-        return;
-      }
-    }
-    stamp(3);
-#pragma unroll
-    for (int e = 0; e < 2; ++e) {
-      aR[e] = anR[e];
-      bR[e] = bnR[e];
-    }
-
-    double* rbuf = red;
-    int* ibuf = reinterpret_cast<int*>(red + V * RVR_NWV * 4);
-    int nrounds = 0;
-    auto round_sums = [&](int rd, double (&dv)[3], int (&iv)[3]) __attribute__((always_inline)) {
-#pragma unroll
-      for (int q = 0; q < 3; ++q) dv[q] = wave_sum_to_lane63(dv[q]);
-      if (wave * 64 < A.nunits) iv[2] = wave_isum_to_lane63(iv[2]);
-      if (lane == 63) {
-#pragma unroll
-        for (int q = 0; q < 3; ++q) rbuf[(rd * RVR_NWV + wave) * 4 + q] = dv[q];
-#pragma unroll
-        for (int q = 0; q < 3; ++q) ibuf[(rd * RVR_NWV + wave) * 4 + q] = iv[q];
-      }
-      __syncthreads();
-#pragma unroll
-      for (int q = 0; q < 3; ++q) {
-        double acc = rbuf[(rd * RVR_NWV) * 4 + q];
-        int iacc = ibuf[(rd * RVR_NWV) * 4 + q];
-#pragma unroll
-        for (int w = 1; w < RVR_NWV; ++w) {
-          acc += rbuf[(rd * RVR_NWV + w) * 4 + q];
-          iacc += ibuf[(rd * RVR_NWV + w) * 4 + q];
-        }
-        dv[q] = __hiloint2double(__builtin_amdgcn_readfirstlane(__double2hiint(acc)),
-                                 __builtin_amdgcn_readfirstlane(__double2loint(acc)));
-        iv[q] = __builtin_amdgcn_readfirstlane(iacc);
-      }
-      fstamp(RVR_F_ROUND + rd);
-      ++nrounds;
-    };
-    auto stamp_decided = [&]() {
-      stamp(4);
-      fstamp(RVR_F_DECIDED);
-      fstamp_value(RVR_F_ROUNDS, nrounds);
-    };
-    ++n_iters;
-    if (kind != K_BUILD) {
-      ++n_passes;
-      ++n_view_passes;
-    }
-    ++stamp_row;
-    bool penalty = false;
-    int pen_cnt = 0;
-    double pen_rs = 0.0;
-    if (kind == K_TRIAL) {
-      int jstar = -1;
-      double Fnew = 0.0, deltaF = 0.0, du2 = 0.0;
-      int lr = 0, no = 0;
-      const double alpha_w = alpha;
-      double al = alpha_w;
-#pragma unroll
-      for (int v = 0; v < V; ++v) {
+            iv[2] = (tid < A.nunits) ? static_cast<int>((cpk >> (10 * v)) & 1023ull) : 0;
+            round_sums(v, dv, iv);
+            if (v == 0) {
+              pen_rs = dv[2];
+              pen_cnt = iv[1];
+            }
+            ++n_trials;
+            Fnew = dv[0];
+            deltaF = Fnew - F;
+            bool accept = true;
+            if (deltaF < -P.eps) {
+              alpha = alpha * P.beta;
+              ++k_;
+              if (k_ < P.maxlsiters) accept = false;
+            }
+            if (accept) {
+              jstar = v;
+              du2 = dv[1];
+              lr = iv[0];
+              no = iv[2];
+              s = rvr_uni(sxL + v);
+              u_c = cl_project(u_c, al, g_c) / nv;
+              g_c = gn_c[v];
+#pragma unroll
+              for (int e = 0; e < 2; ++e) {
+                UR[e] = rok[e] ? cl_project(UR[e], al, GR[e]) / nv : 0.0;
+                GR[e] = rok[e] ? gR[e][v] : 0.0;
+              }
+            }
+          }
+          al = al * P.beta;
+        }
+        stamp_decided();
         if (jstar < 0) {
-          double dv[3] = {0.0, 0.0, 0.0};
-          int iv[3] = {0, 0, 0};
-          const double nv = rvr_uni(nrmL + v);
-#pragma unroll
-          for (int e = 0; e < 2; ++e) {
-            if (e == 0 || two) {
-              const double xi = cl_project(UR[e], al, GR[e]) / nv;
-              const double gv = gR[e][v];
-              bool live = false, pen = false;
-              if (rok[e]) {
-                dv[0] += xi * gv;
-                const double du = xi - UR[e];
-                dv[1] += du * du;
-                live = xi > 0.0 || gv > 0.0;
-                if (v == 0) {
-                  const double cbu = cl_pen_cbu(rvr_uni(sxL), bnR[e], xi);
-                  if (cl_pen_in(cbu, xi, P.eps)) {
-                    pen = true;
-                    dv[2] += cl_pen_ratio(anR[e], xi, cbu);
-                  }
-                }
-              }
-              iv[0] += __popcll(__ballot(live));
-              if (v == 0) iv[1] += __popcll(__ballot(pen));
-            }
-          }
-          iv[2] = (tid < A.nunits) ? static_cast<int>((cpk >> (10 * v)) & 1023ull) : 0;
-          round_sums(v, dv, iv);
-          if (v == 0) {
-            pen_rs = dv[2];
-            pen_cnt = iv[1];
-          }
-          ++n_trials;
-          Fnew = dv[0];
-          deltaF = Fnew - F;
-          bool accept = true;
-          if (deltaF < -P.eps) {
-            alpha = alpha * P.beta;
-            ++k_;
-            if (k_ < P.maxlsiters) accept = false;
-          }
-          if (accept) {
-            jstar = v;
-            du2 = dv[1];
-            lr = iv[0];
-            no = iv[2];
-            s = rvr_uni(sxL + v);
-            u_c = cl_project(u_c, al, g_c) / nv;
-            g_c = gn_c[v];
-#pragma unroll
-            for (int e = 0; e < 2; ++e) {
-              UR[e] = rok[e] ? cl_project(UR[e], al, GR[e]) / nv : 0.0;
-              GR[e] = rok[e] ? gR[e][v] : 0.0;
-            }
-          }
-        }
-        al = al * P.beta;
-      }
-      stamp_decided();
-      if (jstar < 0) continue;
-      const double deltau = sqrt(du2);
-      F = Fnew;
-      ++j_;
-      nout = no;
-      nlive = lr + nout;
-      if (deltau < P.tol_u || fabs(deltaF) < P.tol_F || j_ >= P.maxiniters) {
-        if (jstar == 0) {
-          penalty = true;
+          if constexpr (W < V) {
+            alpha = alpha_w;
+            k_ = k_w;
+            n_trials -= W;
+            zero_run = 0;
+            ++n_redo;
+            ++n_redo_here;
+            redo = true;
+          }
+          return 0;
+        }
+        zero_run = (k_ == 0) ? (zero_run < 1000000 ? zero_run + 1 : zero_run) : 0;
+        const double deltau = sqrt(du2);
+        F = Fnew;
+        ++j_;
+        nout = no;
+        nlive = lr + nout;
+        if (deltau < P.tol_u || fabs(deltaF) < P.tol_F || j_ >= P.maxiniters) {
+          if (jstar == 0) {
+            penalty = true;
+          } else {
+            kind = K_PAIR;
+            return 0;
+          }
         } else {
-          kind = K_PAIR;
-          continue;
-        }
+          alpha = 1.0;
+          k_ = 0;
+          want_out = nout != 0 || view_wanted_v(A.rvp, m, true, A.rv_rows, nlive, nout, n_iters + 1 - n_redo, rv_builds, rv_last, rv_backoff);
+          return 0;
+        }
+      } else if (kind == K_PAIR) {
+        double dv[3] = {0.0, 0.0, 0.0};
+        int iv[3] = {0, 0, 0};
+#pragma unroll
+        for (int e = 0; e < 2; ++e) {
+          const double cbu = s - bR[e] - UR[e];
+          bool pen = false;
+          if (rok[e] && cbu > P.eps && UR[e] > P.eps) {
+            pen = true;
+            dv[2] += fabs((aR[e] + UR[e]) / cbu);
+          }
+          iv[1] += __popcll(__ballot(pen));
+        }
+        round_sums(0, dv, iv);
+        pen_rs = dv[2];
+        pen_cnt = iv[1];
+        penalty = true;
+        stamp_decided();
       } else {
+        double dv[3] = {0.0, 0.0, 0.0};
+        int iv[3] = {0, 0, 0};
+#pragma unroll
+        for (int e = 0; e < 2; ++e) {
+          bool live = false;
+          if (rok[e]) {
+            const double gi = cl_grad(d, UR[e], s, aR[e], bR[e]);
+            GR[e] = gi;
+            dv[0] += UR[e] * gi;
+            live = UR[e] > 0.0 || gi > 0.0;
+          }
+          iv[0] += __popcll(__ballot(live));
+        }
+        iv[2] = (tid < A.nunits) ? static_cast<int>(cpk & 1023ull) : 0;
+        round_sums(0, dv, iv);
+        stamp_decided();
+        if (cown) g_c = gn_c[0];
+        F = dv[0];
+        nout = iv[2];
+        nlive = iv[0] + nout;
+        j_ = 0;
         alpha = 1.0;
         k_ = 0;
+        kind = K_TRIAL;
         want_out = nout != 0 || view_wanted_v(A.rvp, m, true, A.rv_rows, nlive, nout, n_iters + 1 - n_redo, rv_builds, rv_last, rv_backoff);
-        continue;
-      }
-    } else if (kind == K_PAIR) {
-      double dv[3] = {0.0, 0.0, 0.0};
-      int iv[3] = {0, 0, 0};
-#pragma unroll
-      for (int e = 0; e < 2; ++e) {
-        const double cbu = s - bR[e] - UR[e];
-        bool pen = false;
-        if (rok[e] && cbu > P.eps && UR[e] > P.eps) {
-          pen = true;
-          dv[2] += fabs((aR[e] + UR[e]) / cbu);
-        }
-        iv[1] += __popcll(__ballot(pen));
-      }
-      round_sums(0, dv, iv);
-      pen_rs = dv[2];
-      pen_cnt = iv[1];
-      penalty = true;
-      stamp_decided();
-    } else {
-      double dv[3] = {0.0, 0.0, 0.0};
-      int iv[3] = {0, 0, 0};
-#pragma unroll
-      for (int e = 0; e < 2; ++e) {
-        bool live = false;
-        if (rok[e]) {
-          const double gi = cl_grad(d, UR[e], s, aR[e], bR[e]);
-          GR[e] = gi;
-          dv[0] += UR[e] * gi;
-          live = UR[e] > 0.0 || gi > 0.0;
-        }
-        iv[0] += __popcll(__ballot(live));
-      }
-      iv[2] = (tid < A.nunits) ? static_cast<int>(cpk & 1023ull) : 0;
-      round_sums(0, dv, iv);
-      stamp_decided();
-      if (cown) g_c = gn_c[0];
-      F = dv[0];
-      nout = iv[2];
-      nlive = iv[0] + nout;
-      j_ = 0;
-      alpha = 1.0;
-      k_ = 0;
-      kind = K_TRIAL;
-      want_out = nout != 0 || view_wanted_v(A.rvp, m, true, A.rv_rows, nlive, nout, n_iters + 1 - n_redo, rv_builds, rv_last, rv_backoff);
-      continue;
-    }
-    if (penalty) {
-      bool done = true;
-      if (pen_cnt > 0) {
-        d += pen_rs / static_cast<double>(pen_cnt);
-        ++i_;
-        done = i_ >= P.maxoliters;
-      }
-      if (!done) {
-        kind = K_BUILD;
-        continue;
-      }
-      write_point(true);
-      if (blockIdx.x == 0 && A.kind != nullptr && A.marks != nullptr) {
-        const int64_t n = (A.marks_n < KIND_CAP) ? A.marks_n : KIND_CAP;
-        for (int64_t i = tid; i < n; i += RVR_NT)
-          __hip_atomic_store(A.kind + i, A.marks[i], __ATOMIC_RELAXED, __HIP_MEMORY_SCOPE_SYSTEM);
-      }
-      if (arrive_last() && tid == 0) {
-        SolverState* o = A.st;
-        o->ubp = e_ubp ^ 1;
-        o->ubv = 0;
-        SolveShared* sh = A.shared;
-        sh->F = F;
-        sh->d = d;
-        sh->n_passes = n_passes;
-        sh->n_trials = n_trials;
-        sh->ifinal = i_;
-        sh->ubp = e_ubp ^ 1;
-        sh->ubv = 0;
-        sh->done = 1;
-        report_run();
-        if (A.host) {
-          HostMirror* hm = A.host;
-          __hip_atomic_store(&hm->F, F, __ATOMIC_RELAXED, __HIP_MEMORY_SCOPE_SYSTEM);
-          __hip_atomic_store(&hm->d, d, __ATOMIC_RELAXED, __HIP_MEMORY_SCOPE_SYSTEM);
-          __hip_atomic_store(&hm->n_passes, n_passes, __ATOMIC_RELAXED, __HIP_MEMORY_SCOPE_SYSTEM);
-          __hip_atomic_store(&hm->n_trials, n_trials, __ATOMIC_RELAXED, __HIP_MEMORY_SCOPE_SYSTEM);
-          __hip_atomic_store(&hm->n_view_passes, n_view_passes, __ATOMIC_RELAXED, __HIP_MEMORY_SCOPE_SYSTEM);
-          __hip_atomic_store(&hm->nlive, nlive, __ATOMIC_RELAXED, __HIP_MEMORY_SCOPE_SYSTEM);
-          __hip_atomic_store(&hm->nout, nout, __ATOMIC_RELAXED, __HIP_MEMORY_SCOPE_SYSTEM);
-          __hip_atomic_store(&hm->iters, n_iters, __ATOMIC_RELAXED, __HIP_MEMORY_SCOPE_SYSTEM);
-          __hip_atomic_store(&hm->ifinal, i_, __ATOMIC_RELAXED, __HIP_MEMORY_SCOPE_SYSTEM);
-          __hip_atomic_store(&hm->ubp, e_ubp ^ 1, __ATOMIC_RELAXED, __HIP_MEMORY_SCOPE_SYSTEM);
-          __hip_atomic_store(&hm->ubv, 0, __ATOMIC_RELAXED, __HIP_MEMORY_SCOPE_SYSTEM);
-          __hip_atomic_store(&hm->done, 1, __ATOMIC_RELEASE, __HIP_MEMORY_SCOPE_SYSTEM);
-        }
-      }
-      stamp_end();
-      return;
-    }
+        return 0;
+      }
+      if (penalty) {
+        bool done = true;
+        if (pen_cnt > 0) {
+          d += pen_rs / static_cast<double>(pen_cnt);
+          ++i_;
+          done = i_ >= P.maxoliters;
+        }
+        if (!done) {
+          kind = K_BUILD;
+          return 0;
+        }
+        write_point(true);
+        if (blockIdx.x == 0 && A.kind != nullptr && A.marks != nullptr) {
+          const int64_t n = (A.marks_n < KIND_CAP) ? A.marks_n : KIND_CAP;
+          for (int64_t i = tid; i < n; i += RVR_NT)
+            __hip_atomic_store(A.kind + i, A.marks[i], __ATOMIC_RELAXED, __HIP_MEMORY_SCOPE_SYSTEM);
+        }
+        if (arrive_last() && tid == 0) {
+          SolverState* o = A.st;
+          o->ubp = e_ubp ^ 1;
+          o->ubv = 0;
+          o->n_redo = n_redo;
+          SolveShared* sh = A.shared;
+          sh->F = F;
+          sh->d = d;
+          sh->n_passes = n_passes;
+          sh->n_trials = n_trials;
+          sh->ifinal = i_;
+          sh->ubp = e_ubp ^ 1;
+          sh->ubv = 0;
+          sh->done = 1;
+          report_run();
+          if (A.host) {
+            HostMirror* hm = A.host;
+            __hip_atomic_store(&hm->F, F, __ATOMIC_RELAXED, __HIP_MEMORY_SCOPE_SYSTEM);
+            __hip_atomic_store(&hm->d, d, __ATOMIC_RELAXED, __HIP_MEMORY_SCOPE_SYSTEM);
+            __hip_atomic_store(&hm->n_passes, n_passes, __ATOMIC_RELAXED, __HIP_MEMORY_SCOPE_SYSTEM);
+            __hip_atomic_store(&hm->n_trials, n_trials, __ATOMIC_RELAXED, __HIP_MEMORY_SCOPE_SYSTEM);
+            __hip_atomic_store(&hm->n_view_passes, n_view_passes, __ATOMIC_RELAXED, __HIP_MEMORY_SCOPE_SYSTEM);
+            __hip_atomic_store(&hm->nlive, nlive, __ATOMIC_RELAXED, __HIP_MEMORY_SCOPE_SYSTEM);
+            __hip_atomic_store(&hm->nout, nout, __ATOMIC_RELAXED, __HIP_MEMORY_SCOPE_SYSTEM);
+            __hip_atomic_store(&hm->iters, n_iters, __ATOMIC_RELAXED, __HIP_MEMORY_SCOPE_SYSTEM);
+            __hip_atomic_store(&hm->ifinal, i_, __ATOMIC_RELAXED, __HIP_MEMORY_SCOPE_SYSTEM);
+            __hip_atomic_store(&hm->ubp, e_ubp ^ 1, __ATOMIC_RELAXED, __HIP_MEMORY_SCOPE_SYSTEM);
+            __hip_atomic_store(&hm->ubv, 0, __ATOMIC_RELAXED, __HIP_MEMORY_SCOPE_SYSTEM);
+            __hip_atomic_store(&hm->n_redo, n_redo, __ATOMIC_RELAXED, __HIP_MEMORY_SCOPE_SYSTEM);
+            __hip_atomic_store(&hm->done, 1, __ATOMIC_RELEASE, __HIP_MEMORY_SCOPE_SYSTEM);
+          }
+        }
+        stamp_end();
+        return 1;
+      }
+      return 0;
+    };
+    if (narrow ? turn(std::integral_constant<int, 1>{}) : turn(std::integral_constant<int, V>{})) return;
   }
 }
 
diff --git a/clipper_amd/csrc/k_solver.hip.h b/clipper_amd/csrc/k_solver.hip.h
--- a/clipper_amd/csrc/k_solver.hip.h
+++ b/clipper_amd/csrc/k_solver.hip.h
@@ -89,6 +89,8 @@
   int64_t n_view_passes;
   int32_t hold;
   int32_t hold_nlive;
+  int32_t n_redo;
+  int32_t pad_;
 };
 
 enum HoldReason : int32_t { HOLD_ROW_VIEW = 1, HOLD_SUB_ENTER = 2, HOLD_SUB_LEAVE = 3 };
@@ -364,6 +366,10 @@
   L.chain = acc;
 }
 
+__device__ __forceinline__ bool window_guess(int adaptive, bool redo, int k, int zero_run) {
+  return adaptive != 0 && !redo && k == 0 && zero_run >= 2;
+}
+
 template <int V, int NT>
 __device__ __forceinline__ bool decide(const SolveArgs& A, const HeadLoads& L, double* red,
                                        SolverState* stash, PassPlan& plan) {
@@ -688,7 +694,7 @@
     return false;
   }
   const bool sub_leave = A.sub_state == 2 && action == ACT_PASS && !sub_ok;
-  const int wnext = (A.adaptive_window != 0 && !redo && k_ == 0 && zero_run >= 2) ? 1 : V;
+  const int wnext = window_guess(A.adaptive_window, redo, k_, zero_run) ? 1 : V;
   if (writer && tid == 0) {
     auto record = [&](SolverState* o, bool norms_in_place) {
       o->d = d;
@@ -763,6 +769,7 @@
         __hip_atomic_store(&hm->ifinal, i_, __ATOMIC_RELAXED, __HIP_MEMORY_SCOPE_SYSTEM);
         __hip_atomic_store(&hm->ubp, ubp, __ATOMIC_RELAXED, __HIP_MEMORY_SCOPE_SYSTEM);
         __hip_atomic_store(&hm->ubv, ubv, __ATOMIC_RELAXED, __HIP_MEMORY_SCOPE_SYSTEM);
+        __hip_atomic_store(&hm->n_redo, L.n_redo, __ATOMIC_RELAXED, __HIP_MEMORY_SCOPE_SYSTEM);
         __hip_atomic_store(&hm->done, 1, __ATOMIC_RELEASE, __HIP_MEMORY_SCOPE_SYSTEM);
       }
       if (action != ACT_PASS || A.decide_only != 0 || sub_leave) {
diff --git a/include/clipper_hip.h b/include/clipper_hip.h
--- a/include/clipper_hip.h
+++ b/include/clipper_hip.h
@@ -70,6 +70,9 @@
   double sub_pass_avg_us;
   int64_t sub_pass_samples;
   int64_t sub_dense;
+  int64_t resident_single_turns;
+  int64_t resident_redos;
+  int64_t window_redos;
 } clipper_hip_view_stats_t;
 
 
```
